# NethermindEth/latticefold

Hardware: AMD Instinct MI355X
Metric: folding-prover steps/sec (one NIFSProver::prove per step), GoldilocksRingNTT (higher is better)
Workload: dtype u64; 1 GPU; C4: GoldilocksRingNTT R1CS->CCS, m=N=2^20 rows, wit_len=262144, L=4, B=2^16, b=2, K=16, kappa=26, t=3; parallelism=replicas x1

## Files before the change

latticefold_amd/csrc/lf_capi.cpp:

```cpp
#include "lf_ring_host.h"

const char *lf_strerror(int code) {
    switch (code) {
        case LF_OK: return "ok";
        case LF_ERR_INVALID: return "invalid argument / wrong length";
        case LF_ERR_HIP: return "HIP runtime error (no GPU or out of device memory)";
        case LF_ERR_UNSUPPORTED: return "unsupported parameter";
        case LF_ERR_BAD_TABLES: return "ring tables are not a ring isomorphism";
        case LF_ERR_NORM: return "witness coefficient exceeds the decomposition bound";
        case LF_ERR_SIZE_BOUNDS: return "invalid size bounds (m must be >= wit_len*L, power of two)";
        case LF_ERR_STATE: return "call sequence misuse";
        case LF_ERR_REJECT: return "verifier rejected the proof";
    }
    return "unknown error";
}
const char *lf_phase_name(int i) { return (i >= 0 && i < LF_N_PHASES) ? PHASE_NAMES[i] : ""; }

static int install_tables(lf_ctx *c, u64 nonres, const u64 *y) {
    CrtTables T;
    if (build_crt_tables(nonres, y, T) != 0) return LF_ERR_BAD_TABLES;
    c->ring.T = T;
    c->dcrt = make_dev_crt(T);
    return ring_ops<GoldRing>::install_icrt(c, &T.icrt[0][0]);
}

int lf_ctx_create_ring(lf_ctx **out, int device, int ring) {
    if (ring == LF_RING_GOLDILOCKS) return lf_ctx_create(out, device);
    if (!out || ring != LF_RING_BABYBEAR) return LF_ERR_INVALID;
    lf_ctx *c = new lf_ctx();
    c->device = device;
    int rc = lfbb::BbCtx::create(&c->bb, c, device);
    if (rc != LF_OK) { delete c; return rc; }
    *out = c;
    return LF_OK;
}
int lf_ctx_device(const lf_ctx *c) { return c->device; }
int lf_ctx_ring(const lf_ctx *c) { return c && c->bb ? LF_RING_BABYBEAR : LF_RING_GOLDILOCKS; }
int lf_ring_words(int ring) { return ring == LF_RING_BABYBEAR ? 72 : (ring == LF_RING_GOLDILOCKS ? 24 : 0); }
int lf_ring_tau(int ring) { return ring == LF_RING_BABYBEAR ? 9 : (ring == LF_RING_GOLDILOCKS ? 3 : 0); }
uint64_t lf_ring_modulus(int ring) { return ring == LF_RING_BABYBEAR ? (uint64_t)lfbb::BB_P : (ring == LF_RING_GOLDILOCKS ? LF_P : 0); }

int lf_ctx_create(lf_ctx **out, int device) {
    if (!out) return LF_ERR_INVALID;
    int cnt = 0;
    if (hipGetDeviceCount(&cnt) != hipSuccess || cnt <= 0 || device < 0 || device >= cnt) return LF_ERR_HIP;
    HIPCHK(hipSetDevice(device));
    lf_ctx *c = new lf_ctx();
    c->device = device;
    int least = 0, greatest = 0;
    (void)hipDeviceGetStreamPriorityRange(&least, &greatest);
    if (c->create_lane_streams() != LF_OK || hipStreamCreateWithPriority(&c->st_io, hipStreamDefault, least) != hipSuccess) { delete c; return LF_ERR_HIP; }
    (void)hipEventCreateWithFlags(&c->ev_block, hipEventBlockingSync | hipEventDisableTiming);
    u64 nr, y[24];
    default_ring(&nr, y);
    int rc = install_tables(c, nr, y);
    if (rc != LF_OK) { delete c; return rc; }
    *out = c;
    return LF_OK;
}
static void planes_pool_drop(int device);
void lf_ctx_destroy(lf_ctx *c) {
    if (!c) return;
    while (c->io_jobs.load() > 0) std::this_thread::yield();
    (void)hipSetDevice(c->device);
    planes_pool_drop(c->device);
    if (c->bb) { c->bb->destroy(); delete c; return; }
    (void)c->sync_lanes();
    if (c->st_io) (void)hipStreamSynchronize(c->st_io);
    for (int l = 0; l < LF_NLANES; l++)
        if (c->stage[l]) (void)hipHostFree(c->stage[l]);
    if (c->h_pin2) { (void)hipHostFree(c->h_pin2); c->h_pin2 = nullptr; }
    if (c->ev_block) (void)hipEventDestroy(c->ev_block);
    c->comm[0].destroy();
    c->comm[1].destroy();
    if (c->tail_mail) (void)hipHostFree(c->tail_mail);
    if (c->tail_counters) (void)hipFree(c->tail_counters);
    if (c->d_poseidon) (void)hipFree(c->d_poseidon);
    if (c->ev_theta) (void)hipEventDestroy(c->ev_theta);
    if (c->ev_aux) (void)hipEventDestroy(c->ev_aux);
    if (c->st_aux) (void)hipStreamDestroy(c->st_aux);
    if (c->h_aux) (void)hipHostFree(c->h_aux);
    for (int i = 0; i < 2; i++)
        if (c->bits_ev[i]) (void)hipEventDestroy(c->bits_ev[i]);
    c->release_core();
    delete c;
}
int lf_set_ring_tables(lf_ctx *c, uint64_t nonres, const uint64_t *y) {
    if (!c || !y) return LF_ERR_INVALID;
    if (c->bb) return c->bb->set_ring_tables(nonres, y);
    std::lock_guard<std::mutex> g(c->mu);
    HIPCHK(hipSetDevice(c->device));
    return install_tables(c, nonres, y);
}
int lf_get_ring_tables(lf_ctx *c, uint64_t *nonres, uint64_t *y) {
    if (!c || !nonres || !y) return LF_ERR_INVALID;
    if (c->bb) return c->bb->get_ring_tables(nonres, y);
    *nonres = c->ring.T.nu;
    for (int k = 0; k < 8; k++)
        for (int q = 0; q < 3; q++) y[3 * k + q] = c->ring.T.y[k].c[q];
    return LF_OK;
}

int lf_set_digit_mode(lf_ctx *c, int mode) {
    if (!c || (mode != 0 && mode != 1)) return LF_ERR_INVALID;
    std::lock_guard<std::mutex> g(c->mu);
    c->core_any().digit_mode = mode;
    return LF_OK;
}
int lf_set_ext_basis(lf_ctx *c, const uint64_t *T) {
    if (!c || !T) return LF_ERR_INVALID;
    std::lock_guard<std::mutex> g(c->mu);
    const int ring = lf_ctx_ring(c);
    return c->xb.set(T, lf_ring_tau(ring), lf_ring_modulus(ring));
}
int lf_set_sharding(lf_ctx *c, int rank, int world, lf_exchange_fn cb, void *user) {
    if (!c || world < 1 || rank < 0 || rank >= world || (world & (world - 1)) != 0 || (world > 1 && !cb)) return LF_ERR_INVALID;
    if (c->bb) return c->bb->set_sharding(rank, world, cb, user);
    std::lock_guard<std::mutex> g(c->mu);
    if (c->A_loaded) return LF_ERR_STATE;
    for (int l = 0; l < 2; l++) {
        c->comm[l].destroy();
        c->comm[l].rank = rank; c->comm[l].world = world; c->comm[l].cb = cb; c->comm[l].user = user; c->comm[l].poisoned = false; c->comm[l].model = false;
    }
    c->sh_rank = rank; c->sh_world = world;
    c->two_lanes_ok = false;
    c->agreed_two_lanes = -1;
    return LF_OK;
}
int lf_set_sharding_model(lf_ctx *c, int rank, int world) {
    if (!c || world < 1 || rank < 0 || rank >= world || (world & (world - 1)) != 0) return LF_ERR_INVALID;
    if (c->bb) return LF_ERR_UNSUPPORTED;
    std::lock_guard<std::mutex> g(c->mu);
    if (c->A_loaded) return LF_ERR_STATE;
    for (int l = 0; l < 2; l++) {
        c->comm[l].destroy();
        c->comm[l].rank = rank; c->comm[l].world = world; c->comm[l].cb = nullptr; c->comm[l].user = nullptr; c->comm[l].poisoned = false; c->comm[l].model = world > 1;
    }
    c->sh_rank = rank; c->sh_world = world;
    c->two_lanes_ok = world > 1;
    c->agreed_two_lanes = -1;
    return LF_OK;
}
int lf_dist_stats_words(lf_ctx *c, uint64_t *words_sent, int reset) {
    if (!c || !words_sent) return LF_ERR_INVALID;
    if (c->bb) { *words_sent = 0; return LF_OK; }
    *words_sent = c->comm[0].words_sent + c->comm[1].words_sent;
    if (reset) c->comm[0].words_sent = c->comm[1].words_sent = 0;
    return LF_OK;
}
int exchange_modsum_dev(lf_ctx *c, u64 *inout_dev, size_t words) {
    if (c->sh_world <= 1 && !(c->tn.force_exchange && c->cm().nccl)) return LF_OK;
    u64 *g;
    RET(c->tbuf("sh_gather", (size_t)c->sh_world * words, &g));
    RET(c->cm().allgather_dev(inout_dev, g, words, c->stream()));
    launch_modsum(g, (u32)c->sh_world, words, inout_dev, c->stream());
    return LF_OK;
}
int lf_dist_unique_id(uint8_t *id128) { return lfdist::rccl_unique_id(id128); }
static int dist_handshake(lf_ctx *c) {
    c->two_lanes_ok = false;
    if (getenv("LF_DIST_NO_HANDSHAKE")) return LF_OK;
    const int W = c->sh_world, R = c->sh_rank, ITER = 4;
    const size_t words = 64, per_it = words * (size_t)(W + 1);
    const long limit_ms = 20000;
    u64 *dbuf[2] = {nullptr, nullptr}, *hbuf[2] = {nullptr, nullptr};
    for (int l = 0; l < 2; l++) {
        if (lf_dev_malloc(&dbuf[l], per_it * ITER * 8) != hipSuccess || hipHostMalloc((void **)&hbuf[l], per_it * ITER * 8) != hipSuccess) {
            for (int q = 0; q < 2; q++) { if (dbuf[q]) (void)hipFree(dbuf[q]); if (hbuf[q]) (void)hipHostFree(hbuf[q]); }
            return LF_ERR_HIP;
        }
    }
    auto word = [](int g, int lane, int it, size_t w) { return ((u64)(g + 1) * 0x9E3779B97F4A7C15ull) ^ ((u64)lane << 40) ^ ((u64)it << 32) ^ (u64)w; };
    auto run = [&](int lane) -> int {
        const int keep = t_lane;
        t_lane = lane;
        int rc = hipSetDevice(c->device) == hipSuccess ? LF_OK : LF_ERR_HIP;
        for (int it = 0; it < ITER && rc == LF_OK; it++) {
            u64 *hs = hbuf[lane] + per_it * it, *ds = dbuf[lane] + per_it * it;
            for (size_t w = 0; w < words; w++) hs[w] = word(R, lane, it, w);
            if (hipMemcpyAsync(ds, hs, words * 8, hipMemcpyHostToDevice, c->stream()) != hipSuccess) { rc = LF_ERR_HIP; break; }
            rc = c->cm().allgather_dev(ds, ds + words, words, c->stream());
            if (rc == LF_OK && hipMemcpyAsync(hs + words, ds + words, words * W * 8, hipMemcpyDeviceToHost, c->stream()) != hipSuccess) rc = LF_ERR_HIP;
        }
        t_lane = keep;
        return rc;
    };
    c->lane1.submit([&]() -> int { return run(1); });
    int rc = run(0);
    const int rc1 = c->lane1.wait();
    if (rc == LF_OK) rc = rc1;
    bool timed_out = false;
    const auto deadline = std::chrono::steady_clock::now() + std::chrono::milliseconds(limit_ms);
    for (int l = 0; l < 2 && rc == LF_OK && !timed_out; l++)
        for (;;) {
            const hipError_t q = hipStreamQuery(c->st_lane[l]);
            if (q == hipSuccess) break;
            if (q != hipErrorNotReady) { rc = LF_ERR_HIP; break; }
            if (std::chrono::steady_clock::now() > deadline) { timed_out = true; break; }
            std::this_thread::sleep_for(std::chrono::microseconds(200));
        }
    if (timed_out || rc != LF_OK) {
        c->comm[0].abort_peers(); c->comm[1].abort_peers();
        return LF_ERR_STATE;
    }
    bool ok = true;
    for (int l = 0; l < 2 && ok; l++)
        for (int it = 0; it < ITER && ok; it++)
            for (int g2 = 0; g2 < W && ok; g2++)
                for (size_t w = 0; w < words && ok; w++) ok = hbuf[l][per_it * it + words + (size_t)g2 * words + w] == word(g2, l, it, w);
    {
        const char *e = getenv("LF_SHARD_TWO_LANES");
        const u64 mine = e ? (atoi(e) != 0 ? 2 : 0) : (ok ? 1 : 0);
        u64 *hs = hbuf[0], *ds = dbuf[0];
        hs[0] = mine;
        const int keep = t_lane;
        t_lane = 0;
        int rc2 = hipMemcpyAsync(ds, hs, 8, hipMemcpyHostToDevice, c->stream()) == hipSuccess ? LF_OK : LF_ERR_HIP;
        if (rc2 == LF_OK) rc2 = c->cm().allgather_dev(ds, ds + 1, 1, c->stream());
        if (rc2 == LF_OK && hipMemcpyAsync(hs + 1, ds + 1, (size_t)W * 8, hipMemcpyDeviceToHost, c->stream()) != hipSuccess) rc2 = LF_ERR_HIP;
        bool late = false;
        for (; rc2 == LF_OK;) {
            const hipError_t q = hipStreamQuery(c->stream());
            if (q == hipSuccess) break;
            if (q != hipErrorNotReady) { rc2 = LF_ERR_HIP; break; }
            if (std::chrono::steady_clock::now() > deadline) { late = true; break; }
            std::this_thread::sleep_for(std::chrono::microseconds(200));
        }
        t_lane = keep;
        if (late || rc2 != LF_OK) { c->comm[0].abort_peers(); c->comm[1].abort_peers(); return LF_ERR_STATE; }
        u64 mn = 2;
        for (int g2 = 0; g2 < W; g2++) mn = hs[1 + g2] < mn ? hs[1 + g2] : mn;
        ok = mn >= 1;
        c->agreed_two_lanes = ok ? 1 : 0;
    }
    for (int l = 0; l < 2; l++) { (void)hipFree(dbuf[l]); (void)hipHostFree(hbuf[l]); c->comm[l].n_exchanges = 0; c->comm[l].us_total = 0; c->comm[l].us_max = 0; }
    c->two_lanes_ok = ok;
// ... 380 lines not shown
    return c->bb ? ring_ops<BbRing>::witness_from_f(c->bb->p, f_ntt, out) : ring_ops<GoldRing>::witness_from_f(c, f_ntt, out);
}
int lf_witness_get_f_coeff(lf_ctx *c, const lf_witness *w, uint64_t *out) {
    if (!c || !w || !out || w->ctx != c) return LF_ERR_INVALID;
    return c->bb ? ring_ops<BbRing>::witness_get_f_coeff(c->bb->p, w, out) : ring_ops<GoldRing>::witness_get_f_coeff(c, w, out);
}
int lf_witness_get_f(lf_ctx *c, const lf_witness *w, uint64_t *out) {
    if (LF_XB(c) && w && out) { XB x(c); int rc = lf_witness_get_f(c, w, out); if (rc == LF_OK) x.ring_out(out, w->N); return rc; }
    if (!c || !w || !out || w->ctx != c) return LF_ERR_INVALID;
    return c->bb ? ring_ops<BbRing>::witness_get_f(c->bb->p, w, out) : ring_ops<GoldRing>::witness_get_f(c, w, out);
}
int lf_witness_get_w_ccs(lf_ctx *c, const lf_witness *w, uint64_t *out) {
    if (LF_XB(c) && w && out && c->have_ccs_any()) { XB x(c); int rc = lf_witness_get_w_ccs(c, w, out); if (rc == LF_OK) x.ring_out(out, c->params_any().wit_len); return rc; }
    if (!c || !w || !out || w->ctx != c) return LF_ERR_INVALID;
    return c->bb ? ring_ops<BbRing>::witness_get_w_ccs(c->bb->p, w, out) : ring_ops<GoldRing>::witness_get_w_ccs(c, w, out);
}
int lf_witness_commit(lf_ctx *c, const lf_witness *w, uint64_t *cm_out) {
    if (LF_XB(c) && w && cm_out) { XB x(c); int rc = lf_witness_commit(c, w, cm_out); if (rc == LF_OK) x.ring_out(cm_out, c->core_any().kappa); return rc; }
    if (!c || !w || !cm_out || w->ctx != c) return LF_ERR_INVALID;
    return c->bb ? ring_ops<BbRing>::witness_commit(c->bb->p, w, cm_out) : ring_ops<GoldRing>::witness_commit(c, w, cm_out);
}
namespace {
struct PoolEnt { int device; size_t bytes; int32_t *p; };
std::mutex g_pool_mu;
std::vector<PoolEnt> g_pool;
}
int lf_planes_alloc(lf_ctx *c, size_t bytes, int32_t **out) {
    {
        std::lock_guard<std::mutex> g(g_pool_mu);
        for (size_t i = 0; i < g_pool.size(); i++)
            if (g_pool[i].device == c->device && g_pool[i].bytes == bytes) {
                *out = g_pool[i].p;
                g_pool.erase(g_pool.begin() + (long)i);
                return LF_OK;
            }
    }
    return lf_dev_malloc(out, bytes) == hipSuccess ? LF_OK : LF_ERR_HIP;
}
static void planes_release_dev(int device, size_t bytes, int32_t *p) {
    if (!p) return;
    {
        std::lock_guard<std::mutex> g(g_pool_mu);
        if (g_pool.size() < 9) { g_pool.push_back({device, bytes, p}); return; }
    }
    (void)hipFree(p);
}
void lf_planes_release(lf_ctx *c, size_t bytes, int32_t *p) { planes_release_dev(c->device, bytes, p); }
static void planes_pool_drop(int device) {
    std::lock_guard<std::mutex> g(g_pool_mu);
    for (size_t i = 0; i < g_pool.size();)
        if (g_pool[i].device == device) { (void)hipFree(g_pool[i].p); g_pool.erase(g_pool.begin() + (long)i); }
        else i++;
}
void lf_witness_free(lf_witness *w) {
    if (!w) return;
    (void)hipSetDevice(w->device);
    planes_release_dev(w->device, w->plane_bytes, w->planes);
    planes_release_dev(w->device, w->f_bytes, (int32_t *)w->f_ntt);
    planes_release_dev(w->device, w->w_bytes, (int32_t *)w->w_ccs);
    delete w;
}

lf_transcript *lf_transcript_new(void) { return new lf_transcript(); }
lf_transcript *lf_transcript_new_ring(int ring) {
    if (ring == LF_RING_GOLDILOCKS) return new lf_transcript();
    if (ring != LF_RING_BABYBEAR) return nullptr;
    lf_transcript *t = new lf_transcript();
    t->bb = new lfbb::BbTranscript();
    return t;
}
lf_transcript *lf_transcript_clone(const lf_transcript *t) { return t ? new lf_transcript(*t) : nullptr; }
void lf_transcript_free(lf_transcript *t) { delete t; }
void lf_transcript_absorb_fq(lf_transcript *t, const uint64_t *x, size_t n) {
    if (t->bb) t->bb->absorb_fq(x, n);
    else t->t.absorb_fq(x, n);
}
void lf_transcript_absorb_ring(lf_transcript *t, const uint64_t *e, size_t n) {
    if (t->bb) t->bb->absorb_ring(e, n);
    else t->t.absorb_ring(e, n);
}
void lf_transcript_get_challenge(lf_transcript *t, uint64_t *o) {
    if (t->bb) {
        lfbb::H9 c = t->bb->get_challenge();
        memcpy(o, c.c, sizeof(c.c));
        return;
    }
    Fq3 c = t->t.get_challenge();
    o[0] = c.c[0]; o[1] = c.c[1]; o[2] = c.c[2];
}
void lf_transcript_get_short_challenge(lf_transcript *t, uint64_t *o) {
    if (t->bb) t->bb->get_short_challenge(o);
    else t->t.get_short_challenge(o);
}
void lf_transcript_squeeze_bytes(lf_transcript *t, uint8_t *out, size_t n) {
    if (!t || !out || !n) return;
    const size_t usable = t->bb ? 3 : 7, ne = (n + usable - 1) / usable;
    std::vector<u64> e(ne);
    if (t->bb) t->bb->squeeze(e.data(), ne);
    else t->t.squeeze(e.data(), ne);
    for (size_t i = 0, o = 0; i < ne && o < n; i++)
        for (size_t j = 0; j < usable && o < n; j++) out[o++] = (uint8_t)(e[i] >> (8 * j));
}
void lf_poseidon_permute(uint64_t *state, int plain) {
    if (plain == 2) Transcript::permute_scalar(state);
    else if (plain) Transcript::permute_plain(state);
    else Transcript::permute(state);
}
void lf_poseidon_permute_ring(uint64_t *state, int plain, int ring) {
    if (ring == LF_RING_BABYBEAR) {
        if (plain == 2) lfbb::BbTranscript::permute_scalar(state);
        else if (plain) lfbb::BbTranscript::permute_plain(state);
        else lfbb::BbTranscript::permute(state);
    } else lf_poseidon_permute(state, plain);
}
void lf_poseidon_params(uint64_t *ark, uint64_t *mds) {
    const u64 *a, *m;
    Transcript::params(&a, &m);
    memcpy(ark, a, 720 * 8);
    memcpy(mds, m, 576 * 8);
}
void lf_poseidon_params_ring(uint64_t *ark, uint64_t *mds, int ring) {
    const u64 *a, *m;
    if (ring == LF_RING_BABYBEAR) lfbb::BbTranscript::params(&a, &m);
    else Transcript::params(&a, &m);
    memcpy(ark, a, 720 * 8);
    memcpy(mds, m, 576 * 8);
}

int lf_last_phase_ms(lf_ctx *c, float *out) {
    if (!c || !out) return LF_ERR_INVALID;
    for (int i = 0; i < LF_N_PHASES; i++) out[i] = c->core_any().phase_ms[i];
    return LF_OK;
}
int lf_last_timeline(lf_ctx *c, char *names, double *ms, int max_marks) {
    if (!c || !names || !ms || max_marks < 0) return LF_ERR_INVALID;
    if (c->bb) return 0;
    int n = 0;
    for (auto &m : c->tl_marks) {
        if (n >= max_marks) break;
        const char *w = m.first;
        while (*w == ' ') w++;
        snprintf(names + 32 * n, 32, "%s", w);
        ms[n++] = m.second;
    }
    return n;
}
int lf_abi_version(void) { return LFHIP_ABI_VERSION; }
int lf_debug_i8_prof(uint64_t *out64) {
    if (!out64) return LF_ERR_INVALID;
    return getenv("LF_I8G_PROF") ? ajtai_i8g_read_prof((unsigned long long *)out64) : ajtai_i8_read_prof((unsigned long long *)out64);
}
extern "C" int lfdbg_i8g_wg(unsigned int *out512) { return out512 ? ajtai_i8g_read_wg(out512) : -1; }
extern "C" unsigned lfdbg_i8g_planes_base(int ring, uint64_t base) { return ajtai_i8g_planes_base(ring == LF_RING_BABYBEAR ? ajtai_i8_babybear() : ajtai_i8_goldilocks(), base); }
int lf_last_fold_paths(lf_ctx *c, unsigned *sv_round_mask) {
    if (!c || !sv_round_mask) return LF_ERR_INVALID;
    *sv_round_mask = c->core_any().sv_round_mask;
    return LF_OK;
}
int lf_last_fold_split_rounds(lf_ctx *c, unsigned *round_mask) {
    if (!c || !round_mask) return LF_ERR_INVALID;
    *round_mask = c->core_any().fold_split_mask;
    return LF_OK;
}
int lf_last_lin_split_rounds(lf_ctx *c, unsigned *rounds) {
    if (!c || !rounds) return LF_ERR_INVALID;
    *rounds = c->bb ? 0u : c->lin_split_rounds;
    return LF_OK;
}
int lf_last_kernel_stats(lf_ctx *c, float *fold_ms, int *fold_n, float *aj_ms, int *aj_n) {
    if (!c) return LF_ERR_INVALID;
    const CtxCoreBase &k = c->core_any();
    if (fold_ms) *fold_ms = k.k_fold_ms;
    if (fold_n) *fold_n = k.k_fold_n;
    if (aj_ms) *aj_ms = k.k_ajtai_ms;
    if (aj_n) *aj_n = k.k_ajtai_n;
    return LF_OK;
}

namespace {
struct GoldV {
    static constexpr int RE = 24, TAU = 3;
    static u64 modulus() { return LF_P; }
    typedef Fq3 Ext;
    typedef Transcript Tr;
    HostRing ring;
    void mul(const u64 *a, const u64 *b, u64 *o) const { ring.mul_ntt(a, b, o); }
    void mul_ext(const u64 *a, Ext s, u64 *o) const { ring.mul_fq3(a, s, o); }
    static void add(const u64 *a, const u64 *b, u64 *o) { HostRing::add(a, b, o); }
    static void sub(const u64 *a, const u64 *b, u64 *o) { HostRing::sub(a, b, o); }
    static void from_u64(u64 v, u64 *o) { HostRing::from_u64(v, o); }
    static void from_ext(Ext e, u64 *o) { HostRing::from_fq3(e, o); }
    static Ext ext_of(const u64 *e) { return fq3_make(e[0], e[1], e[2]); }
    static Ext ext_from_u64(u64 v) { return fq3_make(v % LF_P, 0, 0); }
    Ext ext_mul(Ext a, Ext b) const { return ring.mul3(a, b); }
    static Ext ext_add(Ext a, Ext b) { return fq3_add(a, b); }
    static Ext ext_sub(Ext a, Ext b) { return fq3_sub(a, b); }
    Ext ext_inv(Ext a) const { return ring.inv3(a); }
    static void absorb_ext(Tr &tr, Ext e) { tr.absorb_fq3_as_ring(e); }
    void crt(const u64 *c, u64 *o) const { ring.crt(c, o); }
    static u64 fmul(u64 a, u64 b) { return fq_mul(a % LF_P, b % LF_P); }
    static u64 fadd(u64 a, u64 b) { return fq_add(a, b); }
    static void rot_x(u64 *a) {
        u64 top = a[23];
        for (int j = 23; j > 0; j--) a[j] = a[j - 1];
        a[0] = fq_neg(top);
        a[12] = fq_add(a[12], top);
    }
};
}

int lf_verify_host(int ring, const lf_params *p, const uint32_t *S_off, const uint32_t *S_idx, const uint64_t *c, lf_transcript *t,
                   const uint64_t *acc, const uint64_t *cm_i, const uint64_t *proof, uint64_t *lcccs_out, int *failed_stage) {
    if (!p || !S_off || !S_idx || !c || !t || !acc || !cm_i || !proof || !lcccs_out) return LF_ERR_INVALID;
    if (p->s == 0 || p->s > 40 || p->K == 0 || p->K > 32 || p->q == 0 || p->q > 8 || p->t == 0 || p->t > 16) return LF_ERR_UNSUPPORTED;
    if (((size_t)1 << p->s) < (size_t)p->wit_len * p->L) return LF_ERR_SIZE_BOUNDS;
    if (failed_stage) *failed_stage = 0;
    if (ring == LF_RING_BABYBEAR) return t->bb ? lfbb::bb_verify_host(p, S_off, S_idx, c, *t->bb, acc, cm_i, proof, lcccs_out, failed_stage) : LF_ERR_INVALID;
    if (ring != LF_RING_GOLDILOCKS || t->bb) return LF_ERR_INVALID;
    static const GoldV *gv = [] {
        GoldV *g = new GoldV();
        u64 nr, y[24];
        default_ring(&nr, y);
        build_crt_tables(nr, y, g->ring.T);
        return g;
    }();
    lfv::Verifier<GoldV> V(*gv, *p, S_off, S_idx, c);
    int rc = V.verify(t->t, acc, cm_i, proof, lcccs_out);
    if (failed_stage) *failed_stage = V.stage;
    return rc;
}
```

latticefold_amd/csrc/lf_ctx.h:

```cpp
#pragma once
#include <hip/hip_runtime.h>
#include <assert.h>
#include <string.h>

#include <atomic>
#include <chrono>
#include <condition_variable>
#include <functional>
#include <future>
#include <thread>
#include <map>
#include <memory>
#include <mutex>
#include <string>
#include <vector>

#include "../../include/lfhip.h"
#include "bb_capi.h"
#include "lf_ctx_core.h"
#include "lf_common.h"
#include "lf_dist.h"
#include "lf_kernels.h"
#include "lf_sb.h"
#include "lf_verify.h"

using namespace lf;

namespace lf {
void launch_fix_many(const DevCrt &t, const u64 *in, size_t ld_in, u64 *out, size_t ld_out, size_t n_in, u32 rows3, Fq3Const r, hipStream_t s);
}

#include <stdio.h>
#include <stdlib.h>
static bool lf_trace_on() { static int v = -1; if (v < 0) v = getenv("LF_TRACE") ? 1 : 0; return v == 1; }
#define LF_TRACE(c, msg)                                                              \
    do {                                                                              \
        if (lf_trace_on()) {                                                          \
            hipError_t e_ = hipStreamSynchronize((c)->stream());                            \
            fprintf(stderr, "[lf] %s:%d %s -> %s\n", __func__, __LINE__, msg, hipGetErrorString(e_)); \
            fflush(stderr);                                                           \
        }                                                                             \
    } while (0)

inline thread_local int t_lane = 0;

struct lf_transcript {
    Transcript t;
    lfbb::BbTranscript *bb = nullptr;
    lf_transcript() {}
    lf_transcript(const lf_transcript &o) : t(o.t), bb(o.bb ? new lfbb::BbTranscript(*o.bb) : nullptr) {}
    ~lf_transcript() { delete bb; }
};

struct Timeline {
    bool on;
    std::chrono::steady_clock::time_point t0;
    std::vector<std::pair<const char *, double>> marks, marks1;
    Timeline() : on(getenv("LF_TIMELINE") != nullptr), t0(std::chrono::steady_clock::now()) { marks1.reserve(32); }
    void mark(const char *what) {
        marks.push_back({what, std::chrono::duration<double, std::milli>(std::chrono::steady_clock::now() - t0).count()});
    }
    void mark1(const char *what) { marks1.push_back({what, std::chrono::duration<double, std::milli>(std::chrono::steady_clock::now() - t0).count()}); }
    void merge() {
        marks.insert(marks.end(), marks1.begin(), marks1.end());
        marks1.clear();
        std::stable_sort(marks.begin(), marks.end(), [](const std::pair<const char *, double> &a, const std::pair<const char *, double> &b) { return a.second < b.second; });
    }
    void dump() {
        if (!on) return;
        double prev = 0;
        for (auto &m : marks) { fprintf(stderr, "[timeline] %-28s at %8.3f ms  (+%7.3f)\n", m.first, m.second, m.second - prev); prev = m.second; }
    }
};
inline thread_local Timeline *t_tl = nullptr;
#define TL_MARK(x) do { if (t_tl) t_tl->mark(x); } while (0)

static const char *PHASE_NAMES[LF_N_PHASES] = {"linearization", "decomp_crt_commit", "decomp_evals", "fold_prepare",
                                                "fold_sumcheck", "fold_finish", "host_transcript", "total"};

struct LaneWorker {
    std::thread th;
    std::mutex m;
    std::condition_variable cv;
    std::function<int()> job;
    bool has_job = false, done = false, stop = false;
    int rc = 0;
    void loop() {
        std::unique_lock<std::mutex> lk(m);
        for (;;) {
            cv.wait(lk, [&] { return has_job || stop; });
            if (stop) return;
            std::function<int()> j = std::move(job);
            has_job = false;
            lk.unlock();
            int r = j();
            lk.lock();
            rc = r;
            done = true;
            cv.notify_all();
        }
    }
    void submit(std::function<int()> j) {
        std::unique_lock<std::mutex> lk(m);
        if (!th.joinable()) th = std::thread([this] { loop(); });
        job = std::move(j);
        has_job = true;
        done = false;
        cv.notify_all();
    }
    int wait() {
        std::unique_lock<std::mutex> lk(m);
        cv.wait(lk, [&] { return done; });
        return rc;
    }
    ~LaneWorker() {
        {
            std::unique_lock<std::mutex> lk(m);
            stop = true;
            cv.notify_all();
        }
        if (th.joinable()) th.join();
    }
};

struct lf_ctx : CtxCore<u64> {
    lf_ctx() : CtxCore<u64>(8192, 2 * 9 * 24 * sizeof(u64)) {}
    int lane() const override { return t_lane; }
    lfbb::BbCtx *bb = nullptr;
    ExtBasis xb;
    hipStream_t &st_io = st_lane[2];
    std::mutex io_mu;
    std::atomic<int> io_jobs{0};
    inline CtxCoreBase &core_any();
    bool have_ccs_any() { return core_any().have_ccs; }
    const lf_params &params_any() { return core_any().P; }
    size_t n_any() { return core_any().n; }
    size_t m_any() { return core_any().m; }
    size_t N_any() { return core_any().N; }
    HostRing ring;
    DevCrt dcrt;
    LaneWorker lane1;
    int agreed_two_lanes = -1;
    bool two_lanes_ok = false;
    lfdist::Comm comm[2];
    lfdist::Comm &cm() { assert(t_lane < 2); return comm[t_lane]; }
    bool ccs_general = false;
    size_t shc_r0 = (size_t)-1, shc_rcnt = 0, shc_lo = 0, shc_hi = 0;
    LinCombDesc desc{};
    std::vector<std::pair<const char *, double>> tl_marks;
    const lf_witness *bits_wit[2] = {nullptr, nullptr};
    u32 *bits_ptr[2] = {nullptr, nullptr};
    hipEvent_t bits_ev[2] = {nullptr, nullptr};
    hipEvent_t ev_yR = nullptr, ev_yL = nullptr;
    u64 *h_pin2 = nullptr;
    size_t h_pin2_words = 0;
    int pin2(size_t words) {
        if (words <= h_pin2_words) return LF_OK;
        if (h_pin2) (void)hipHostFree(h_pin2);
        h_pin2 = nullptr; h_pin2_words = 0;
        if (hipHostMalloc((void **)&h_pin2, words * 8) != hipSuccess) return LF_ERR_HIP;
        h_pin2_words = words;
        return LF_OK;
    }
    hipStream_t st_aux = nullptr;
    hipEvent_t ev_aux = nullptr;
    u64 *h_aux = nullptr;
    unsigned lin_split_rounds = 0;

    unsigned char *stage[LF_NLANES] = {nullptr, nullptr, nullptr};
    size_t stage_off[LF_NLANES] = {0, 0, 0};
    static constexpr size_t STAGE_BYTES = (size_t)1 << 20;
    int h2d_small(void *dst, const void *src, size_t bytes) {
        unsigned char *&ring = stage[t_lane];
        if (!ring && hipHostMalloc((void **)&ring, STAGE_BYTES, hipHostMallocDefault) != hipSuccess) { ring = nullptr; return LF_ERR_HIP; }
        const size_t need = (bytes + 63) & ~(size_t)63;
        if (need > STAGE_BYTES) {
            HIPCHK(hipMemcpyAsync(dst, src, bytes, hipMemcpyHostToDevice, stream()));
            HIPCHK(hipStreamSynchronize(stream()));
            return LF_OK;
        }
        if (stage_off[t_lane] + need > STAGE_BYTES) {
            HIPCHK(hipStreamSynchronize(stream()));
            stage_off[t_lane] = 0;
        }
        unsigned char *slot = ring + stage_off[t_lane];
        stage_off[t_lane] += need;
        memcpy(slot, src, bytes);
        HIPCHK(hipMemcpyAsync(dst, slot, bytes, hipMemcpyHostToDevice, stream()));
        return LF_OK;
    }
    TailMail *tail_mail = nullptr;
    u32 *tail_counters = nullptr;
    u64 *tail_dev_chal = nullptr;
    u32 tail_epoch = 0;
    int num_cus = 0;
    int tail_setup() {
        if (tail_mail) return LF_OK;
        hipDeviceProp_t pr;
        HIPCHK(hipGetDeviceProperties(&pr, device));
        num_cus = pr.multiProcessorCount;
        void *d = nullptr;
        HIPCHK(lf_dev_malloc(&d, 4096));
        HIPCHK(hipMemset(d, 0, 4096));
        tail_counters = (u32 *)d;
        tail_dev_chal = (u64 *)((char *)d + 1024);
        HIPCHK(hipHostMalloc((void **)&tail_mail, sizeof(TailMail), hipHostMallocMapped | hipHostMallocCoherent));
        memset(tail_mail, 0, sizeof(TailMail));
        return LF_OK;
    }
    u64 *d_poseidon = nullptr;
    int poseidon_setup() {
        if (d_poseidon) return LF_OK;
        const u64 *a, *m;
        Transcript::params(&a, &m);
        HIPCHK(lf_dev_malloc(&d_poseidon, (720 + 576) * 8));
        HIPCHK(hipMemcpy(d_poseidon, a, 720 * 8, hipMemcpyHostToDevice));
        HIPCHK(hipMemcpy(d_poseidon + 720, m, 576 * 8, hipMemcpyHostToDevice));
        return LF_OK;
    }
    hipEvent_t ev_theta = nullptr;
    hipEvent_t ev_block = nullptr;
    int lane_sync() {
        if (t_lane == 1 && ev_block) {
            HIPCHK(hipEventRecord(ev_block, st_lane[1]));
            HIPCHK(hipEventSynchronize(ev_block));
            return LF_OK;
        }
        HIPCHK(hipStreamSynchronize(stream()));
        return LF_OK;
    }
};
inline CtxCoreBase &lf_ctx::core_any() { return bb ? bb->core() : *this; }


#pragma GCC visibility push(hidden)
Fq3Const f3c(Fq3 a);
bool shard_keep(const lf_ctx *c, int kind, size_t n);
int build_eq_dev(lf_ctx *c, const Fq3 *pt, u32 nv, u64 *eq_dev);
int exchange_modsum_dev(lf_ctx *c, u64 *inout_dev, size_t words);
int down_small(lf_ctx *c, const u64 *dsrc, size_t words, u64 *host);
void shard_slice(const lf_ctx *c, size_t n, size_t *i0, size_t *cnt);
struct GatherPart { const u64 *src; size_t src_ld; u64 *dst; size_t planes; };
int shard_col_range(lf_ctx *c, size_t r0, size_t rcnt, size_t *lo, size_t *hi);
Fq3 sc_round_transcript(Transcript &tr, const u64 *evals, u32 npts);
void sc_prologue(Transcript &tr, u32 nv, u32 deg);
int gather_slices(lf_ctx *c, u64 *buf, size_t planes, size_t n);
struct SideState {
    const int32_t *planes = nullptr;
    u64 *z = nullptr;
    u64 *eq_r = nullptr;
    std::vector<u64> lcccs;
    std::atomic<int> z_state{0};
    hipEvent_t z_ev = nullptr;
    const unsigned char *D = nullptr;
    u32 *sv_bits = nullptr;
    ~SideState() { if (z_ev) (void)hipEventDestroy(z_ev); }
};
int gather_parts(lf_ctx *c, const GatherPart *parts, int np, size_t lcl);
inline thread_local bool t_xb_active = false;
struct XB {
    lf_ctx *c;
    size_t RE, TAU;
    std::vector<std::unique_ptr<std::vector<u64>>> keep;
    lf_transcript *tr = nullptr;
    explicit XB(lf_ctx *cc) : c(cc), RE((size_t)lf_ring_words(lf_ctx_ring(cc))), TAU((size_t)lf_ring_tau(lf_ctx_ring(cc))) { t_xb_active = true; }
    ~XB() {
        t_xb_active = false;
        if (tr) { tr->t.set_basis(nullptr, nullptr); if (tr->bb) tr->bb->set_basis(nullptr, nullptr); }
    }
    const u64 *ring_in(const u64 *p, size_t elems) {
        if (!p) return p;
        keep.emplace_back(new std::vector<u64>(p, p + elems * RE));
        c->xb.to_int(keep.back()->data(), elems * 8);
        return keep.back()->data();
    }
    const u64 *ext_in(const u64 *p, size_t n) {
        if (!p) return p;
        keep.emplace_back(new std::vector<u64>(p, p + n * TAU));
        c->xb.to_int(keep.back()->data(), n);
        return keep.back()->data();
    }
    void ring_out(u64 *p, size_t elems) { if (p) c->xb.to_ext(p, elems * 8); }
    void ext_out(u64 *p, size_t n) { if (p) c->xb.to_ext(p, n); }
    void transcript(lf_transcript *t) {
        tr = t;
        if (t->bb) t->bb->set_basis(c->xb.T, c->xb.Ti);
        else t->t.set_basis(c->xb.T, c->xb.Ti);
    }
};
#define LF_XB(c) ((c) && (c)->xb.on && !t_xb_active)
int fold_impl(lf_ctx *c, Transcript &tr, SideState *S , u64 *lcccs_out, lf_witness **w_out, u64 *proof);
int commit_download(lf_ctx *c, const u64 *dev, size_t words, u64 *host);
int commit_parts_i8g(lf_ctx *c, const unsigned char *D, size_t ldn, u32 NP, u64 *out_dev);
int sb_cut_parts(lf_ctx *c, const lf_witness *wit, const char *name, const unsigned char **D);
void fold_draw_rho(lf_ctx *c, Transcript &tr, const u64 *eta, std::vector<u64> &rho_c, std::vector<u64> &rho, std::vector<int8_t> &rho8);
void fold_instance_host(lf_ctx *c, const std::vector<Fq3> &pt, const u64 *theta, const u64 *eta, const std::vector<u64> &rho_c, const std::vector<u64> &rho, SideState *S,
                        u64 *lcccs_out);
int fold_impl_sb(lf_ctx *c, Transcript &tr, SideState *S , u64 *lcccs_out, lf_witness **w_out, u64 *proof);
int sb_fold_round_abi(lf_ctx *c, const u64 *t5, const u64 *F, size_t n, const Fq3Const *d_mu, u64 *evals_out);
int dot_batch_dev(lf_ctx *c, const u64 *X, size_t ldx, u32 na, const u64 *Y, size_t ldy, u32 nb, size_t n, u64 *dpart, u64 *od, hipStream_t st = nullptr,
                         const char *tag = "", unsigned char *yb_pre = nullptr);
int coef_eval_dev(lf_ctx *c, const int32_t *planes, size_t n, const u64 *eq, size_t ldeq, u32 K, int mode_bits, u64 *partial, u64 *od, size_t ldp,
                         const lf_witness *wit = nullptr);
int lin_tail_rounds(lf_ctx *c, Transcript &tr, const u64 *cur, const u64 *cure, size_t n, u64 *tout, u64 *partial, u32 round, Fq3 *point,
                           u64 *msgs, u32 deg, const std::function<void(u32)> *after_round);
int build_z(lf_ctx *c, const int32_t *planes, u32 K, int mode_bits, const u64 *heads, u64 *z, size_t w0 = 0, size_t wcnt = (size_t)-1,
            const unsigned char *D = nullptr );
bool lcccs_point(const lf_params &P, const u64 *lcccs, std::vector<Fq3> &pt);
#pragma GCC visibility pop
```

latticefold_amd/csrc/lf_ctx_core.h:

```cpp
#pragma once
#include <hip/hip_runtime.h>

#include <chrono>
#include <map>
#include <mutex>
#include <string>
#include <vector>

#include "../../include/lfhip.h"
#include "lf_common.h"

struct lf_witness;

constexpr int LF_NLANES = 3;

struct EvPair { hipEvent_t a, b; };

struct CtxCoreBase {
    int device = 0;
    hipStream_t st_lane[LF_NLANES] = {nullptr, nullptr, nullptr};
    std::mutex mu, buf_mu, ev_mu;
    int digit_mode = 0;
    Tunables tn;
    uint32_t lin_blocks = 0;
    bool A_loaded = false;
    unsigned char *dAb = nullptr;
    uint32_t i8_nch = 0, i8_kc = 0;
    uint32_t kappa = 0;
    size_t nA = 0, nA_total = 0, A_col0 = 0;
    int sh_rank = 0, sh_world = 1;
    bool have_ccs = false;
    lf_params P{};
    size_t N = 0, m = 0, n = 0;
    std::vector<uint32_t *> d_rowptr, d_col, d_colptr, d_rowidx;
    int sc_round = -1, sc_cur = 0;
    size_t sc_n = 0;
    int sf_round = -1, sf_cur = 0;
    size_t sf_n = 0;
    const lf_witness *vs_wit = nullptr;
    bool vs_keep = false;
    uint64_t *vs_dev = nullptr;
    hipEvent_t ev_prep[2] = {nullptr, nullptr};
    unsigned sv_round_mask = 0;
    unsigned fold_split_mask = 0;
    float phase_ms[LF_N_PHASES] = {0};
    float k_fold_ms = 0, k_ajtai_ms = 0;
    int k_fold_n = 0, k_ajtai_n = 0;
    double host_tr_ms = 0;

    virtual int lane() const = 0;
    hipStream_t stream() const { return st_lane[lane()]; }

    std::map<std::string, DevBuf> bufs;
    std::string lane_name(const std::string &name) const {
        const int l = lane();
        return l ? (l == 1 ? "lane1:" : "lane2:") + name : name;
    }
    int buf(const std::string &name, size_t bytes, void **out) {
        DevBuf *b;
        {
            std::lock_guard<std::mutex> g(buf_mu);
            b = &bufs[lane_name(name)];
        }
        int rc = b->ensure(bytes);
        *out = b->p;
        return rc;
    }
    void drop_buf(const std::string &name) {
        std::lock_guard<std::mutex> g(buf_mu);
        auto it = bufs.find(lane_name(name));
        if (it != bufs.end()) { it->second.release(); bufs.erase(it); }
    }
    template <class T>
    int tbuf(const std::string &name, size_t count, T **out) {
        void *p;
        int rc = buf(name, count * sizeof(T), &p);
        *out = (T *)p;
        return rc;
    }
    uint64_t *h_pin_lane[LF_NLANES] = {nullptr, nullptr, nullptr};
    size_t h_pin_words_lane[LF_NLANES] = {0, 0, 0};
    uint64_t *h_round[LF_NLANES] = {nullptr, nullptr, nullptr};
    uint64_t *&h_pin_ref() { return h_pin_lane[lane()]; }
    int pin(size_t words) {
        uint64_t *&hp = h_pin_lane[lane()];
        size_t &hw = h_pin_words_lane[lane()];
        if (words <= hw) return LF_OK;
        if (hp) (void)hipHostFree(hp);
        hp = nullptr; hw = 0;
        if (words < pin_min_words) words = pin_min_words;
        if (hipHostMalloc((void **)&hp, words * 8) != hipSuccess) return LF_ERR_HIP;
        hw = words;
        return LF_OK;
    }
    uint64_t *round_out() {
        uint64_t *&p = h_round[lane()];
        if (!p && hipHostMalloc((void **)&p, round_out_bytes, hipHostMallocMapped) != hipSuccess) p = nullptr;
        return p;
    }
    std::vector<EvPair> ev_pool;
    size_t ev_used = 0;
    std::vector<std::pair<int, size_t>> ev_tags;
    size_t ev_begin(int tag) {
        std::lock_guard<std::mutex> g(ev_mu);
        if (ev_used == ev_pool.size()) {
            EvPair e;
            (void)hipEventCreate(&e.a);
            (void)hipEventCreate(&e.b);
            ev_pool.push_back(e);
        }
        size_t i = ev_used++;
        (void)hipEventRecord(ev_pool[i].a, stream());
        ev_tags.push_back({tag, i});
        return i;
    }
    void ev_end(size_t i) {
        if (i == (size_t)-1) return;
        std::lock_guard<std::mutex> g(ev_mu);
        (void)hipEventRecord(ev_pool[i].b, stream());
    }
    void ev_reset() {
        ev_used = 0;
        ev_tags.clear();
    }
    void ev_collect() {
        (void)hipStreamSynchronize(st_lane[0]);
        (void)hipStreamSynchronize(st_lane[1]);
        k_fold_ms = k_ajtai_ms = 0;
        k_fold_n = k_ajtai_n = 0;
        for (int i = 0; i < LF_N_PHASES; i++) phase_ms[i] = 0;
        for (auto &tg : ev_tags) {
            float ms = 0;
            (void)hipEventElapsedTime(&ms, ev_pool[tg.second].a, ev_pool[tg.second].b);
            if (tg.first == 0) { k_fold_ms += ms; k_fold_n++; }
            else if (tg.first == 1) { k_ajtai_ms += ms; k_ajtai_n++; }
            else if (tg.first >= 10 && tg.first < 10 + LF_N_PHASES) phase_ms[tg.first - 10] += ms;
        }
        phase_ms[6] = (float)host_tr_ms;
    }
    int shard_columns(size_t n_cols, size_t *col0, size_t *cnt) const {
        if (n_cols % (size_t)sh_world) return LF_ERR_UNSUPPORTED;
        *cnt = n_cols / sh_world;
        *col0 = *cnt * sh_rank;
        return LF_OK;
    }
    int create_lane_streams() {
        int least = 0, greatest = 0;
        (void)hipDeviceGetStreamPriorityRange(&least, &greatest);
        if (hipStreamCreateWithPriority(&st_lane[0], hipStreamDefault, least) != hipSuccess ||
            hipStreamCreateWithPriority(&st_lane[1], hipStreamDefault, greatest) != hipSuccess) return LF_ERR_HIP;
        return LF_OK;
    }
    int sync_lanes() {
        HIPCHK(hipStreamSynchronize(st_lane[0]));
        HIPCHK(hipStreamSynchronize(st_lane[1]));
        return LF_OK;
    }
    void drop_matrix() {
        if (dAb) (void)hipFree(dAb);
        dAb = nullptr;
        A_loaded = false;
        kappa = i8_nch = i8_kc = 0;
        nA = nA_total = A_col0 = 0;
    }
    virtual ~CtxCoreBase() {}

protected:
    CtxCoreBase(size_t pin_min, size_t round_bytes) : pin_min_words(pin_min), round_out_bytes(round_bytes) {}
    const size_t pin_min_words, round_out_bytes;
    void release_base() {
        for (auto &kv : bufs) kv.second.release();
        drop_matrix();
        for (int l = 0; l < LF_NLANES; l++) {
            if (h_pin_lane[l]) (void)hipHostFree(h_pin_lane[l]);
            if (h_round[l]) (void)hipHostFree(h_round[l]);
            h_pin_lane[l] = h_round[l] = nullptr;
        }
        for (auto &e : ev_pool) { (void)hipEventDestroy(e.a); (void)hipEventDestroy(e.b); }
        ev_pool.clear();
        for (int l = 0; l < 2; l++)
            if (ev_prep[l]) (void)hipEventDestroy(ev_prep[l]);
        for (int l = 0; l < LF_NLANES; l++)
            if (st_lane[l]) (void)hipStreamDestroy(st_lane[l]);
    }
};

template <class W>
struct CtxCore : CtxCoreBase {
    W *d_icrt = nullptr;
    W *d_icrt_sp_val = nullptr;
    uint32_t *d_icrt_sp_col = nullptr;
    std::vector<W *> d_val, d_valT;
    const W *vs_eq = nullptr;
    void free_ccs() {
        for (auto q : d_rowptr) (void)hipFree(q);
        for (auto q : d_col) (void)hipFree(q);
        for (auto q : d_val) (void)hipFree(q);
// ... 26 lines not shown
```

latticefold_amd/csrc/lf_fold.cpp:

```cpp
#include "lf_ring_host.h"

static int tail_host_rounds(lf_ctx *c, Transcript &tr, u32 epoch, u32 nr, u32 npts, bool dev_transcript, u64 *msgs, Fq3 *pt,
                            const std::function<void(u32)> *after_round = nullptr, u32 round0 = 0) {
    TailMail *mail = c->tail_mail;
    const auto t_start = std::chrono::steady_clock::now();
    double host_us = 0, wait_us = 0;
    auto t_mark = t_start;
    const bool tl_on = t_tl && t_tl->on;
    for (u32 i = 0; i < nr; i++) {
        u32 spins = 0;
        while (__atomic_load_n(&mail->msg_seq[i], __ATOMIC_ACQUIRE) != epoch) {
            __builtin_ia32_pause();
            if ((++spins & 0xfff) == 0) {
                if (__atomic_load_n(&mail->err, __ATOMIC_RELAXED) == epoch ||
                    std::chrono::duration<double>(std::chrono::steady_clock::now() - t_start).count() > 10.0) {
                    __atomic_store_n(&mail->abort_seq, epoch, __ATOMIC_RELEASE);
                    (void)hipStreamSynchronize(c->stream());
                    return LF_ERR_HIP;
                }
            }
        }
        if (tl_on) { auto nw = std::chrono::steady_clock::now(); wait_us += std::chrono::duration<double, std::micro>(nw - t_mark).count(); t_mark = nw; }
        u64 *evs = msgs + (size_t)i * npts * 24;
        memcpy(evs, (const void *)mail->msg[i], (size_t)npts * 24 * 8);
// ... 28 lines not shown
    RET(c->tail_setup());
    LinTailArgs A;
    A.T = cur; A.E = cure; A.Tout = tout; A.n0 = n; A.rounds = P.s - round + 1; A.deg = deg; A.partial = partial;
    RET(c->tbuf("lin_tail_priv", lin_tail_priv_words(n, P.t), &A.priv));
    A.counters = c->tail_counters; A.dev_chal = c->tail_dev_chal;
    HIPCHK(hipHostGetDevicePointer((void **)&A.mail, c->tail_mail, 0));
    if (++c->tail_epoch >= (1u << 30)) c->tail_epoch = 1;
    A.epoch = c->tail_epoch;
    A.r_first = f3c(point[round - 2]);
    A.dev_transcript = (c->tn.device_transcript && !c->xb.on) ? 1u : 0u;
    A.pos_ark = A.pos_mds = nullptr; A.sponge_state = nullptr;
    if (A.dev_transcript) {
        RET(tail_sponge_to_device(c, tr, &A.sponge_state));
        A.pos_ark = c->d_poseidon; A.pos_mds = c->d_poseidon + 720;
    }
    if (launch_lin_tail(c->dcrt, c->desc, A, c->stream()) == 0) return LF_ERR_UNSUPPORTED;
    if (hipGetLastError() != hipSuccess) return LF_ERR_HIP;
    return tail_host_rounds(c, tr, A.epoch, A.rounds, deg + 1, A.dev_transcript != 0, msgs + (size_t)(round - 1) * (deg + 1) * 24, &point[round - 1], after_round, round);
}
static int fold_tail_rounds(lf_ctx *c, Transcript &tr, const FoldRoundArgs &a, u64 *curF, u64 *const Fbuf[2], u64 *T_other, const Fq3Const *d_mu,
                            u64 *partial, u32 round, std::vector<Fq3> &pt, u64 *msgs, u32 deg) {
    const lf_params &P = c->P;
    RET(c->tail_setup());
    const u32 nr = P.s - round + 1;
    FoldTailArgs A;
    A.T[0] = (u64 *)a.eqL; A.T[1] = T_other;
    A.F[0] = curF; A.F[1] = curF == Fbuf[0] ? Fbuf[1] : Fbuf[0];
    A.n0 = a.n; A.rounds = nr; A.K = P.K; A.mu_pow = d_mu; A.partial = partial;
    A.counters = c->tail_counters; A.dev_chal = c->tail_dev_chal;
    RET(c->tbuf("tail_eqpriv", fold_tail_eqpriv_words(a.n, P.K), &A.eqpriv));
    HIPCHK(hipHostGetDevicePointer((void **)&A.mail, c->tail_mail, 0));
    if (++c->tail_epoch >= (1u << 30)) c->tail_epoch = 1;
    A.epoch = c->tail_epoch;
    A.r_first = f3c(pt[round - 2]);
    A.dev_transcript = (c->tn.device_transcript && !c->xb.on) ? 1u : 0u;
    A.pos_ark = A.pos_mds = nullptr; A.sponge_state = nullptr;
    if (A.dev_transcript) {
        RET(tail_sponge_to_device(c, tr, &A.sponge_state));
        A.pos_ark = c->d_poseidon; A.pos_mds = c->d_poseidon + 720;
    }
    if (launch_fold_tail(c->dcrt, A, c->num_cus, c->stream()) == 0) return LF_ERR_UNSUPPORTED;
    if (hipGetLastError() != hipSuccess) return LF_ERR_HIP;
    return tail_host_rounds(c, tr, A.epoch, nr, deg + 1, A.dev_transcript != 0, msgs + (size_t)(round - 1) * (deg + 1) * 24, &pt[round - 1]);
}

static void sv_build_coef(lf_ctx *c, int V, const Fq3 *W, std::vector<u64> &out) {
    const int NX = 2 * V, NPR = sv_num_pairs(V);
    std::vector<Fq3> C((size_t)NPR * 4, fq3_zero());
    std::vector<SvPair> prs(NPR);
    for (int i = 0; i < NPR; i++) prs[i] = sv_pair(V, i);
    auto find = [&](unsigned s, unsigned b) {
        for (int i = 0; i < NPR; i++)
            if (prs[i].s == s && prs[i].b == b) return i;
        return -1;
    };
    std::vector<Fq3> wa(NX), wb(NX);
    for (int x = 0; x < NX; x++) {
        if (x < V) { wa[x] = W[x]; wb[x] = fq3_neg(W[x]); }
        else { wa[x] = fq3_zero(); wb[x] = W[x - V]; }
    }
    for (int x = 0; x < NX; x++)
        for (int y = x; y < NX; y++) {
            const Fq3 p2[3] = {c->ring.mul3(wa[x], wa[y]), fq3_add(c->ring.mul3(wa[x], wb[y]), c->ring.mul3(wb[x], wa[y])), c->ring.mul3(wb[x], wb[y])};
            for (int z = y; z < NX; z++) {
                Fq3 p3[4];
                p3[0] = c->ring.mul3(p2[0], wa[z]);
                p3[1] = fq3_add(c->ring.mul3(p2[0], wb[z]), c->ring.mul3(p2[1], wa[z]));
                p3[2] = fq3_add(c->ring.mul3(p2[1], wb[z]), c->ring.mul3(p2[2], wa[z]));
                p3[3] = c->ring.mul3(p2[2], wb[z]);
                int mult, idx;
                if (x == y && y == z) { mult = 1; idx = find(1u << x, 1u << x); }
                else if (x == y) { mult = 3; idx = find(1u << z, (1u << x) | (1u << z)); }
                else if (y == z) { mult = 3; idx = find(1u << x, (1u << x) | (1u << y)); }
                else { mult = 6; const unsigned mk = (1u << x) | (1u << y) | (1u << z); idx = find(mk, mk); }
                for (int e = 0; e < 4; e++) {
                    Fq3 t = p3[e], acc = fq3_zero();
                    for (int i = 0; i < mult; i++) acc = fq3_add(acc, t);
                    C[(size_t)idx * 4 + e] = fq3_add(C[(size_t)idx * 4 + e], acc);
                }
            }
        }
    for (int x = 0; x < NX; x++) {
        const int idx = find(1u << x, 1u << x);
        C[(size_t)idx * 4] = fq3_sub(C[(size_t)idx * 4], wa[x]);
        C[(size_t)idx * 4 + 1] = fq3_sub(C[(size_t)idx * 4 + 1], wb[x]);
    }
    out.resize((size_t)NPR * 12);
    for (size_t i = 0; i < (size_t)NPR * 4; i++)
        for (int q = 0; q < 3; q++) out[i * 3 + q] = C[i].c[q];
}

void fold_draw_rho(lf_ctx *c, Transcript &tr, const u64 *eta, std::vector<u64> &rho_c, std::vector<u64> &rho, std::vector<int8_t> &rho8) {
    const lf_params &P = c->P;
    const u32 K2 = 2 * P.K;
    rho_c.assign((size_t)K2 * 24, 0); rho.assign((size_t)K2 * 24, 0); rho8.assign((size_t)K2 * 24, 0);
    {
        HostTimer ht(c);
        tr.absorb_ring(eta, (size_t)K2 * P.t);
        tr.absorb_label("rho_s");
        for (u32 i = 0; i + 1 < K2; i++) tr.get_short_challenge(&rho_c[(size_t)i * 24]);
        rho_c[(size_t)(K2 - 1) * 24] = 1;
        for (u32 i = 0; i < K2; i++) {
            c->ring.crt(&rho_c[(size_t)i * 24], &rho[(size_t)i * 24]);
            for (int q2 = 0; q2 < 24; q2++) {
                u64 v = rho_c[(size_t)i * 24 + q2];
                rho8[(size_t)i * 24 + q2] = (int8_t)(v > LF_P / 2 ? -(int64_t)(LF_P - v) : (int64_t)v);
            }
        }
    }
}
void fold_instance_host(lf_ctx *c, const std::vector<Fq3> &pt, const u64 *theta, const u64 *eta, const std::vector<u64> &rho_c, const std::vector<u64> &rho, SideState *S,
                        u64 *lcccs_out) {
    const lf_params &P = c->P;
    const u32 K = P.K, K2 = 2 * K;
    const size_t ll = lf_lcccs_len(&P);
    HostTimer ht(c);
    u64 *o = lcccs_out;
    for (u32 i = 0; i < P.s; i++, o += 24) HostRing::from_fq3(pt[i], o);
    {
        Fq3 res[24];
        for (int j = 0; j < 24; j++) res[j] = fq3_zero();
        for (u32 i = 0; i < K2; i++) {
            u64 rot[24];
            memcpy(rot, &rho_c[(size_t)i * 24], sizeof(rot));
            const u64 *th = theta + (size_t)i * 72;
            for (int bi = 0; bi < 24; bi++) {
                Fq3 b = fq3_make(th[3 * bi], th[3 * bi + 1], th[3 * bi + 2]);
                for (int j = 0; j < 24; j++)
                    if (rot[j]) res[j] = fq3_add(res[j], fq3_mul_fq(b, rot[j]));
                u64 top = rot[23];
                for (int j = 23; j > 0; j--) rot[j] = rot[j - 1];
                rot[0] = fq_neg(top);
                rot[12] = fq_add(rot[12], top);
            }
        }
        for (int j = 0; j < 24; j++) { o[3 * j] = res[j].c[0]; o[3 * j + 1] = res[j].c[1]; o[3 * j + 2] = res[j].c[2]; }
        o += 72;
    }
    u64 tmp[24];
    auto part = [&](u32 i) { return &S[i < K ? 0 : 1].lcccs[(size_t)(i % K) * ll * 24]; };
    for (u32 q2 = 0; q2 < P.kappa; q2++, o += 24) {
        memset(o, 0, 24 * 8);
        for (u32 i = 0; i < K2; i++) { c->ring.mul_ntt(part(i) + ((size_t)P.s + 3 + q2) * 24, &rho[(size_t)i * 24], tmp); HostRing::add(o, tmp, o); }
    }
    for (u32 j = 0; j < P.t; j++, o += 24) {
        memset(o, 0, 24 * 8);
        for (u32 i = 0; i < K2; i++) { c->ring.mul_ntt(&rho[(size_t)i * 24], eta + ((size_t)i * P.t + j) * 24, tmp); HostRing::add(o, tmp, o); }
    }
    for (u32 q2 = 0; q2 < P.l + 1; q2++, o += 24) {
        memset(o, 0, 24 * 8);
        for (u32 i = 0; i < K2; i++) { c->ring.mul_ntt(&rho[(size_t)i * 24], part(i) + ((size_t)P.s + 3 + P.kappa + P.t + q2) * 24, tmp); HostRing::add(o, tmp, o); }
    }
}
int fold_impl(lf_ctx *c, Transcript &tr, SideState *S , u64 *lcccs_out, lf_witness **w_out, u64 *proof) {
    if (c->P.b != 2) return fold_impl_sb(c, tr, S, lcccs_out, w_out, proof);
    const lf_params &P = c->P;
    size_t m = c->m, n = c->n, N = c->N;
    u32 K = P.K, K2 = 2 * K, deg = 2 * P.b;
    std::vector<Fq3> alpha(K2), zeta(K2), mu(K2), beta(P.s);
    {
        HostTimer ht(c);
        tr.absorb_label("alpha_s");
        for (u32 i = 0; i < K2; i++) alpha[i] = tr.get_challenge();
        tr.absorb_label("zeta_s");
        for (u32 i = 0; i < K2; i++) zeta[i] = tr.get_challenge();
    }
    size_t ph = c->ev_begin(13);
    std::vector<Fq3Const> mu_pow((size_t)K2 * 3), a_pow((size_t)K2 * 3), z_pow((size_t)K2 * P.t);
    for (u32 i = 0; i < K2; i++) {
        Fq3 pa = alpha[i], pz = zeta[i];
        for (u32 d = 0; d < 3; d++) { a_pow[(size_t)i * 3 + d] = f3c(pa); pa = c->ring.mul3(pa, alpha[i]); }
        for (u32 j = 0; j < P.t; j++) { z_pow[(size_t)i * P.t + j] = f3c(pz); pz = c->ring.mul3(pz, zeta[i]); }
    }
    Fq3Const *d_mu, *d_ap, *d_zp;
    RET(upload_consts(c, "c_ap", a_pow, &d_ap));
    RET(upload_consts(c, "c_zp", z_pow, &d_zp));
    u64 *G[2], *eqb, *zz, *partial, *od;
    RET(c->tbuf("fold_G1", 24 * m, &G[0]));
    RET(c->tbuf("fold_G2", 24 * m, &G[1]));
    RET(c->tbuf("fold_eqb", 3 * m, &eqb));
    RET(c->tbuf("fold_zz", (size_t)P.t * 24 * n, &zz));
    RET(c->tbuf("round_partial", round_partial_words(), &partial));
    od = c->round_out();
    if (!od) return LF_ERR_HIP;
    u64 *const od_host = od, *od_shard = nullptr;
    if (c->sh_world > 1) {
        RET(c->tbuf("fold_round_out", 5 * 24 + 8, &od_shard));
        od = od_shard;
    }
    const bool shard_tabs = shard_keep(c, 1, m);
    const size_t g_r0 = shard_tabs ? (size_t)c->sh_rank * (m / (size_t)c->sh_world) : 0, g_rcnt = shard_tabs ? m / (size_t)c->sh_world : (size_t)-1;
    size_t zc_lo = 0, zc_hi = n;
    if (shard_tabs) RET(shard_col_range(c, g_r0, g_rcnt, &zc_lo, &zc_hi));
    {
        hipStream_t s0 = c->stream(), s1 = (t_lane == 0) ? c->st_lane[1] : s0;
        u64 *zz1 = zz;
        if (s1 != s0) {
            RET(c->tbuf("fold_zz1", (size_t)P.t * 24 * n, &zz1));
            if (!c->ev_prep[0]) { HIPCHK(hipEventCreateWithFlags(&c->ev_prep[0], hipEventDisableTiming)); HIPCHK(hipEventCreateWithFlags(&c->ev_prep[1], hipEventDisableTiming)); }
            HIPCHK(hipEventRecord(c->ev_prep[0], s0));
            HIPCHK(hipStreamWaitEvent(s1, c->ev_prep[0], 0));
        }
        for (int sd = 0; sd < 2; sd++) {
            hipStream_t st = sd ? s1 : s0;
            u64 *zb = sd ? zz1 : zz;
            launch_lincomb_z(c->dcrt, S[sd].z + zc_lo, n, K, d_zp + (size_t)sd * K * P.t, P.t, zc_hi - zc_lo, zb + zc_lo, st);
            if (c->ccs_general) {
                u64 *zaos;
                RET(c->tbuf(sd ? "spmv_zaos_R" : "spmv_zaos_L", (size_t)P.t * n * 24, &zaos));
                launch_spmv_rows(c->dcrt, P.t, c->d_rowptr.data(), c->d_col.data(), c->d_val.data(), zb, (size_t)24 * n, n, zaos, G[sd], m, 0, st, g_r0, g_rcnt);
            } else
            launch_spmv_sum(c->dcrt, P.t, c->d_rowptr.data(), c->d_col.data(), c->d_val.data(), zb, (size_t)24 * n, n, G[sd], m, st, g_r0, g_rcnt);
            launch_add_fhat_comb(c->dcrt, S[sd].planes, N, K, d_ap + (size_t)sd * K * 3, G[sd], m, st, g_r0, g_rcnt);
        }
        if (s1 != s0) {
            HIPCHK(hipEventRecord(c->ev_prep[1], s1));
            HIPCHK(hipStreamWaitEvent(s0, c->ev_prep[1], 0));
        }
    }
    {
        HostTimer ht(c);
        tr.absorb_label("mu_s");
        for (u32 i = 0; i + 1 < K2; i++) mu[i] = tr.get_challenge();
        mu[K2 - 1] = fq3_one();
        tr.absorb_label("beta_s");
        for (u32 i = 0; i < P.s; i++) beta[i] = tr.get_challenge();
    }
    TL_MARK(" fold challenges");
    for (u32 i = 0; i < K2; i++) {
        Fq3 pm = mu[i];
        for (u32 d = 0; d < 3; d++) { mu_pow[(size_t)i * 3 + d] = f3c(pm); pm = c->ring.mul3(pm, mu[i]); }
    }
    RET(upload_consts(c, "c_mu", mu_pow, &d_mu));
    RET(build_eq_dev(c, beta.data(), P.s, eqb));
    u64 *svE[3] = {nullptr, nullptr, nullptr};
    const bool sv_split = !c->tn.fold_sv_no_split && P.s >= 4 && m >= 256;
    if (sv_split) {
        RET(c->tbuf("fold_svE1", 3 * (m / 2), &svE[0]));
        RET(c->tbuf("fold_svE2", 3 * (m / 4), &svE[1]));
        RET(c->tbuf("fold_svE3", 3 * (m / 8), &svE[2]));
        RET(build_eq_dev(c, beta.data() + 1, P.s - 1, svE[0]));
    }
    Fq3 sv_c = fq3_one();
    u32 svE_level = 1;
    const bool fr_split = sv_split && c->sh_world == 1 && c->dcrt.nu2p40 && !c->tn.fold_rounds_no_split;
    u64 *svE_rest = nullptr;
    if (fr_split) RET(c->tbuf("fold_svE_rest", 3 * (m / 8) + 64, &svE_rest));
    auto svE_ptr = [&](u32 l) -> u64 * {
        if (l <= 3) return svE[l - 1];
        size_t off = 0;
        for (u32 q = 4; q < l; q++) off += 3 * (m >> q);
        return svE_rest + off;
    };
    auto svE_ensure = [&](u32 l) {
        for (; svE_level < l; svE_level++)
            launch_eq_pairsum(svE_ptr(svE_level), m >> svE_level, m >> (svE_level + 1), svE_ptr(svE_level + 1), m >> (svE_level + 1), c->stream());
    };
    auto sv_c_at = [&](u32 round, const std::vector<Fq3> &ptv) {
        Fq3 cc = fq3_one();
        for (u32 k = 1; k < round; k++) {
            const Fq3 b = beta[k - 1], r = ptv[k - 1];
            cc = c->ring.mul3(cc, fq3_add(c->ring.mul3(fq3_sub(fq3_one(), b), fq3_sub(fq3_one(), r)), c->ring.mul3(b, r)));
        }
        return cc;
    };
    LF_TRACE(c, "fold prepare");
    c->ev_end(ph);
    if (t_tl && t_tl->on) { (void)hipStreamSynchronize(c->stream()); TL_MARK(" fold prepare (synced)"); }

    ph = c->ev_begin(14);
    u64 *msgs = proof;
    std::vector<Fq3> pt(P.s);
    { HostTimer ht(c); sc_prologue(tr, P.s, deg); }
    const size_t Gw = (size_t)c->sh_world, gr = (size_t)c->sh_rank;
    bool sharded = Gw > 1;
    const bool fused = !c->tn.fold_unfused && (Gw == 1 || !c->tn.shard_plain_rounds);
    const size_t fuse_min = c->tn.fuse_min;
    int fmode = 0;
    const u64 *prevF = nullptr;
    size_t prevld = 0;
    const size_t lut_min = c->tn.lut_min;
    const size_t tab_min = c->tn.tab_min;
    const bool use_lut = fused && P.s >= 4 && m / 4 >= lut_min && m / 4 >= 4 && !c->tn.fold_no_lut;
    const bool use_r4tab = use_lut && c->dcrt.nu2p40 && !c->tn.fold_no_r4tab;
    const bool use_r5 = use_r4tab && !c->tn.fold_no_r5tab && Gw == 1 && P.s >= 5 && (N & 3) == 0 && (c->tn.no_tail || m / 8 > c->tn.tail_n) && m / 32 >= c->tn.r5_min;
    u64 *F[2], *T5[2];
    size_t half = m / 2;
    const size_t f0_ent = use_lut ? m / 16 : m / 4, f1_ent = use_r5 ? m / 32 : m / 8;
    RET(c->tbuf("fold_F0", (size_t)K2 * 3 * 24 * (f0_ent ? f0_ent : 1), &F[0]));
    RET(c->tbuf("fold_F1", (size_t)K2 * 3 * 24 * (f1_ent ? f1_ent : 1), &F[1]));
    RET(c->tbuf("fold_T0", 57 * (half ? half : 1), &T5[0]));
    RET(c->tbuf("fold_T1", 57 * (half / 2 ? half / 2 : 1), &T5[1]));
    FoldRoundArgs a;
    a.eqL = S[0].eq_r; a.eqR = S[1].eq_r; a.eqB = eqb; a.G1 = G[0]; a.G2 = G[1]; a.ld = m; a.n = m;
    a.p0 = 0; a.pcnt = m / 2; a.pF0 = 0;
    const u64 *curF = nullptr;
    size_t ldF = 0;
    int flip = 0;
    u64 *d_lut = nullptr;
    c->sv_round_mask = 0;
    c->fold_split_mask = 0;
    u32 *sv_bits[2] = {nullptr, nullptr};
    const bool sv_two_streams = t_lane == 0 && Gw == 1;
    hipStream_t sv_g_stream = c->stream();
    const bool use_sv = !c->tn.force_exchange && !c->tn.fold_no_sv && (Gw == 1 || !c->tn.shard_plain_rounds) && N <= m && (N & 3) == 0 && !c->tn.fold_tab_r1;
    for (u32 round = 1; round <= P.s; round++) {
        fmode = 0;
        if (!sharded && !c->tn.no_tail && round >= 5 && fmode == 0 && curF && ldF == a.n && a.n <= c->tn.tail_n && a.n >= 4 &&
            P.s - round + 1 <= TAIL_MAX_ROUNDS) {
            int trc = fold_tail_rounds(c, tr, a, (u64 *)curF, F, T5[flip], d_mu, partial, round, pt, msgs, deg);
            if (trc == LF_OK) {
                curF = (u64 *)curF == F[0] ? F[1] : F[0];
                ldF = 2;
                break;
            }
            if (trc != LF_ERR_UNSUPPORTED) return trc;
        }
        if (round > 1) {
            Fq3Const r = f3c(pt[round - 2]);
            size_t nn = a.n / 2;
            u64 *dst = T5[flip];
            const bool handover = sharded && !shard_keep(c, 1, nn);
            hipStream_t sg = c->stream();
            if (use_sv && sv_two_streams && !sharded && (int)round <= c->tn.sv_rounds && round <= 3 && nn / 2 >= c->tn.sv_min && sv_shape_ok(1 << (round - 1), nn / 2, K))
                sg = c->st_lane[1];
            sv_g_stream = sg;
            if (sharded) {
                const size_t j0 = gr * (nn / Gw), jc = nn / Gw;
                if (round == 2) {
                    launch_fix_many(c->dcrt, a.eqL + 2 * j0, a.ld, dst + j0, nn, 2 * jc, 1, r, sg);
                    launch_fix_many(c->dcrt, a.eqR + 2 * j0, a.ld, dst + 3 * nn + j0, nn, 2 * jc, 1, r, sg);
                    launch_fix_many(c->dcrt, a.eqB + 2 * j0, a.ld, dst + 6 * nn + j0, nn, 2 * jc, 1, r, sg);
                    launch_fix_many(c->dcrt, a.G1 + 2 * j0, a.ld, dst + 9 * nn + j0, nn, 2 * jc, 8, r, sg);
                    launch_fix_many(c->dcrt, a.G2 + 2 * j0, a.ld, dst + 33 * nn + j0, nn, 2 * jc, 8, r, sg);
                } else {
                    launch_fix_many(c->dcrt, a.eqL + 2 * j0, a.ld, dst + j0, nn, 2 * jc, 19, r, sg);
                }
                if (handover && round <= 3) RET(gather_slices(c, dst, 57, nn));
            } else if (round == 2) {
                launch_fix_many(c->dcrt, a.eqL, a.ld, dst, nn, a.n, 1, r, sg);
                launch_fix_many(c->dcrt, a.eqR, a.ld, dst + 3 * nn, nn, a.n, 1, r, sg);
                launch_fix_many(c->dcrt, a.eqB, a.ld, dst + 6 * nn, nn, a.n, 1, r, c->stream());
                launch_fix_many(c->dcrt, a.G1, a.ld, dst + 9 * nn, nn, a.n, 8, r, sg);
                launch_fix_many(c->dcrt, a.G2, a.ld, dst + 33 * nn, nn, a.n, 8, r, sg);
            } else if (sg != c->stream()) {
                launch_fix_many(c->dcrt, a.eqL, a.ld, dst, nn, a.n, 2, r, sg);
                launch_fix_many(c->dcrt, a.eqB, a.ld, dst + 6 * nn, nn, a.n, 1, r, c->stream());
                launch_fix_many(c->dcrt, a.G1, a.ld, dst + 9 * nn, nn, a.n, 16, r, sg);
            } else {
                launch_fix_many(c->dcrt, a.eqL, a.ld, dst, nn, a.n, 19, r, c->stream());
            }
            if (handover) {
                if (round > 3) {
                    u64 *fd = F[(round & 1) ? 0 : 1];
                    size_t lcl = ldF / 2;
                    launch_fix_many(c->dcrt, curF, ldF, fd, lcl, ldF, K2 * 3 * 8, r, c->stream());
                    const GatherPart gp[2] = {{dst + gr * lcl, nn, dst, 57}, {fd, lcl, fd, (size_t)K2 * 3 * 24}};
                    RET(gather_parts(c, gp, 2, lcl));
                    curF = fd; ldF = nn;
                    sharded = false;
                    a.eqL = dst; a.eqR = dst + 3 * nn; a.eqB = dst + 6 * nn; a.G1 = dst + 9 * nn; a.G2 = dst + 33 * nn;
                    a.ld = nn; a.n = nn; a.p0 = 0; a.pcnt = nn / 2; a.pF0 = 0;
                    flip ^= 1;
                    goto tables_ready;
                }
                sharded = false;
            }
            if (round == 3) {
                Fq3 r1 = pt[0], r2 = pt[1], o1 = fq3_sub(fq3_one(), r1), o2 = fq3_sub(fq3_one(), r2);
                Fq3Const W[4] = {f3c(c->ring.mul3(o1, o2)), f3c(c->ring.mul3(r1, o2)), f3c(c->ring.mul3(o1, r2)), f3c(c->ring.mul3(r1, r2))};
                size_t q = sharded ? nn / Gw : nn, j0 = sharded ? gr * q : 0;
                if (use_lut) {
                    std::vector<u64> lut(2 * 81 * 3);
                    for (int code = 0; code < 81; code++) {
                        Fq3 v = fq3_zero();
                        int cc = code;
                        for (int b = 0; b < 4; b++, cc /= 3) {
                            Fq3 wb = fq3_make(W[b].c[0], W[b].c[1], W[b].c[2]);
                            if (cc % 3 == 2) v = fq3_add(v, wb);
                            else if (cc % 3 == 0) v = fq3_sub(v, wb);
                        }
                        lut[3 * code] = v.c[0]; lut[3 * code + 1] = v.c[1]; lut[3 * code + 2] = v.c[2];
                        Fq3 sq = c->ring.mul3(v, v);
                        lut[3 * (81 + code)] = sq.c[0]; lut[3 * (81 + code) + 1] = sq.c[1]; lut[3 * (81 + code) + 2] = sq.c[2];
                    }
                    RET(c->tbuf("fold_lut", 2 * 81 * 3 + 8, &d_lut));
                    RET(c->h2d_small(d_lut, lut.data(), lut.size() * 8));
                    fmode = 3;
                    curF = nullptr; ldF = q;
                } else {
                    launch_fold_materialize2(c->dcrt, S[0].planes, S[1].planes, N, j0, q, K, W, F[0], c->stream());
                    curF = F[0]; ldF = q;
                }
            } else if (round > 3) {
                u64 *fd = F[(round & 1) ? 0 : 1];
                if (use_lut && round == 4) fmode = 4;
                else if (use_r5 && round == 5) fmode = 7;
                else if (fused && ldF >= fuse_min && ldF >= 4) { prevF = curF; prevld = ldF; fmode = 1; }
                else launch_fix_many(c->dcrt, curF, ldF, fd, ldF / 2, ldF, K2 * 3 * 8, r, c->stream());
                curF = fd; ldF = ldF / 2;
            }
            a.eqL = dst; a.eqR = dst + 3 * nn; a.eqB = dst + 6 * nn; a.G1 = dst + 9 * nn; a.G2 = dst + 33 * nn;
            a.ld = nn; a.n = nn;
            flip ^= 1;
        }
        if (sharded && !shard_keep(c, 1, a.n)) sharded = false;
        if (sharded) { a.pcnt = a.n / 2 / Gw; a.p0 = gr * a.pcnt; a.pF0 = a.p0; }
        else { a.p0 = 0; a.pcnt = a.n / 2; a.pF0 = 0; }
    tables_ready:
        const u64 *Er = nullptr;
        size_t ldEr = 0;
        bool split_now = false;
        if (fr_split && round >= 2 && !sharded && (fmode == 7 || (fmode == 4 && use_r4tab)) && a.pcnt >= c->tn.fold_split_min) {
            sv_c = sv_c_at(round, pt);
            const Fq3 bi = beta[round - 1];
            if ((sv_c.c[0] | sv_c.c[1] | sv_c.c[2]) && (bi.c[0] | bi.c[1] | bi.c[2])) {
                svE_ensure(round);
                Er = svE_ptr(round); ldEr = m >> round;
                split_now = true;
                c->fold_split_mask |= 1u << (round - 1);
            }
        }
        size_t ev = c->ev_begin(0);
        const int svV = 1 << (round - 1);
        if (use_sv && (int)round <= c->tn.sv_rounds && round <= 3 && a.pcnt >= c->tn.sv_min && sv_shape_ok(svV, a.pcnt, K) && (a.p0 * (size_t)svV) % 256 == 0) {
            std::vector<Fq3> W((size_t)svV, fq3_one());
            for (int b = 0; b < svV; b++)
                for (u32 j = 0; j + 1 < round; j++) W[b] = c->ring.mul3(W[b], ((b >> j) & 1) ? pt[j] : fq3_sub(fq3_one(), pt[j]));
            std::vector<u64> coef;
            sv_build_coef(c, svV, W.data(), coef);
            u64 *d_coef, *gtmp, *svtp;
            unsigned char *sveb;
            int32_t *svpart, *svtot;
            RET(c->tbuf("sv_coef", coef.size() + 8, &d_coef));
            RET(c->tbuf("sv_gtmp", 128, &gtmp));
            RET(c->tbuf("sv_tp", sv_tp_words(K), &svtp));
            RET(c->tbuf("sv_eb", sv_eb_bytes(a.pcnt), &sveb));
            RET(c->tbuf("sv_part", sv_part_words(svV, a.pcnt, K), &svpart));
            RET(c->tbuf("sv_tot", sv_tot_words(svV, K), &svtot));
            RET(c->h2d_small(d_coef, coef.data(), coef.size() * 8));
            if (!sv_bits[0])
                for (int sd = 0; sd < 2; sd++) {
                    if (S[sd].sv_bits) { sv_bits[sd] = S[sd].sv_bits; continue; }
                    RET(c->tbuf(sd ? "sv_bits_R" : "sv_bits_L", sv_bits_words(N, K), &sv_bits[sd]));
                    launch_sv_bits(S[sd].planes, N, N, K, sv_bits[sd], c->stream());
                }
            hipStream_t sg = round == 1 ? (sv_two_streams && !sharded ? c->st_lane[1] : c->stream()) : sv_g_stream;
            hipEvent_t g_ready = nullptr;
            if (sg != c->stream()) {
                if (!c->ev_prep[0]) { HIPCHK(hipEventCreateWithFlags(&c->ev_prep[0], hipEventDisableTiming)); HIPCHK(hipEventCreateWithFlags(&c->ev_prep[1], hipEventDisableTiming)); }
                if (round == 1) {
                    HIPCHK(hipEventRecord(c->ev_prep[0], c->stream()));
                    HIPCHK(hipStreamWaitEvent(sg, c->ev_prep[0], 0));
                }
            }
            launch_fold_round_g(c->dcrt, a, partial, gtmp, sg);
            if (sg != c->stream()) {
                HIPCHK(hipEventRecord(c->ev_prep[1], sg));
                g_ready = c->ev_prep[1];
            }
            const u64 *Ei = nullptr;
            size_t ldE = 0;
            Fq3Const w01[2] = {};
            if (sv_split) {
                sv_c = sv_c_at(round, pt);
                const Fq3 bi = beta[round - 1];
                w01[0] = f3c(c->ring.mul3(sv_c, fq3_sub(fq3_one(), bi)));
                w01[1] = f3c(c->ring.mul3(sv_c, bi));
                svE_ensure(round);
                const size_t ne = m >> round;
                Ei = svE[round - 1]; ldE = ne;
            }
            if (launch_sv_round(c->dcrt, svV, sv_bits[0], sv_bits[1], N, a.eqB, a.ld, a.p0, a.pcnt, K, d_mu, d_coef, sveb, svpart, svtot, svtp, gtmp, od, c->stream(), g_ready,
                                Ei, ldE, w01) != 0)
                return LF_ERR_UNSUPPORTED;
            c->sv_round_mask |= 1u << (round - 1);
        } else
        if ((round == 2 || (round == 1 && c->tn.fold_tab_r1)) && a.pcnt >= tab_min) {
            const int nd = round == 1 ? 2 : 4, ncode = round == 1 ? 9 : 81;
            std::vector<u64> poly((size_t)ncode * 12);
            const Fq3 one = fq3_one(), r1v = round == 2 ? pt[0] : fq3_zero();
            auto small = [&](int v) { return v == 0 ? fq3_zero() : (v > 0 ? (v == 1 ? one : fq3_add(one, one)) : (v == -1 ? fq3_neg(one) : fq3_neg(fq3_add(one, one)))); };
            for (int code = 0; code < ncode; code++) {
                int dg[4] = {0, 0, 0, 0}, cc = code;
                for (int b = 0; b < nd; b++, cc /= 3) dg[b] = cc % 3 - 1;
                Fq3 f0, f1;
                if (round == 1) { f0 = small(dg[0]); f1 = small(dg[1]); }
                else {
                    f0 = fq3_add(small(dg[0]), c->ring.mul3(small(dg[1] - dg[0]), r1v));
                    f1 = fq3_add(small(dg[2]), c->ring.mul3(small(dg[3] - dg[2]), r1v));
                }
                Fq3 df = fq3_sub(f1, f0), f0s = c->ring.mul3(f0, f0), dfs = c->ring.mul3(df, df);
                Fq3 t1 = c->ring.mul3(f0s, df), t2 = c->ring.mul3(f0, dfs);
                Fq3 q[4] = {fq3_sub(c->ring.mul3(f0s, f0), f0), fq3_sub(fq3_add(fq3_add(t1, t1), t1), df), fq3_add(fq3_add(t2, t2), t2), c->ring.mul3(dfs, df)};
                for (int e = 0; e < 4; e++)
                    for (int w = 0; w < 3; w++) poly[(size_t)code * 12 + 3 * e + w] = q[e].c[w];
            }
            u64 *d_poly, *d_tp;
            RET(c->tbuf("fold_poly", 81 * 12 + 8, &d_poly));
            RET(c->tbuf("fold_tp", (size_t)K2 * 3 * 81 * 12, &d_tp));
            RET(c->h2d_small(d_poly, poly.data(), poly.size() * 8));
            launch_fold_round_tab(c->dcrt, (int)round, a, S[0].planes, S[1].planes, N, K, d_mu, d_poly, d_tp, partial, od, c->stream());
        } else if (round == 1) launch_fold_round1(c->dcrt, a, S[0].planes, S[1].planes, N, K, d_mu, partial, od, c->stream());
        else if (round == 2) launch_fold_round2(c->dcrt, a, S[0].planes, S[1].planes, N, K, d_mu, f3c(pt[0]), partial, od, c->stream());
        else if (fmode == 3 && c->dcrt.nu2p40) {
            u64 *mutab;
            RET(c->tbuf("fold_mutab", (size_t)3 * K2 * 3 * 81 * 4, &mutab));
            launch_fold_round_lut_mu(c->dcrt, a, S[0].planes, S[1].planes, N, d_lut, mutab, K, d_mu, partial, od, c->stream());
        } else if (fmode == 3) launch_fold_round_lut(c->dcrt, a, S[0].planes, S[1].planes, N, d_lut, K, d_mu, partial, od, c->stream());
        else if (fmode == 4 && use_r4tab) {
            u64 *r4sq, *r4mt;
            RET(c->tbuf("fold_r4sq", (size_t)6561 * 4, &r4sq));
            RET(c->tbuf("fold_r4mt", (size_t)K2 * 3 * 162 * 4, &r4mt));
            launch_fold_round_lut_fix_tab(c->dcrt, a, S[0].planes, S[1].planes, N, d_lut, f3c(pt[round - 2]), r4sq, r4mt, use_r5 ? nullptr : (u64 *)curF, ldF, K, d_mu, partial, od,
                                          c->stream(), Er, ldEr);
        } else if (fmode == 7) {
            u64 *r5xx, *r5yy, *r5mt;
            RET(c->tbuf("fold_r5xx", (size_t)6561 * 4, &r5xx));
            RET(c->tbuf("fold_r5yy", (size_t)6561 * 4, &r5yy));
            RET(c->tbuf("fold_r5mt", (size_t)K2 * 3 * 324 * 4, &r5mt));
            launch_fold_round_lut_fix5(c->dcrt, a, S[0].planes, S[1].planes, N, d_lut, f3c(pt[round - 3]), f3c(pt[round - 2]), r5xx, r5yy, r5mt, (u64 *)curF, ldF, K, d_mu, partial, od,
                                       c->stream(), Er, ldEr);
        } else if (fmode == 4) launch_fold_round_lut_fix(c->dcrt, a, S[0].planes, S[1].planes, N, d_lut, f3c(pt[round - 2]), (u64 *)curF, ldF, K, d_mu, partial, od, c->stream());
        else if (fmode == 1) launch_fold_round_fix(c->dcrt, a, prevF, prevld, f3c(pt[round - 2]), (u64 *)curF, ldF, K, d_mu, partial, od, c->stream(), Er, ldEr);
        else launch_fold_round(c->dcrt, a, curF, ldF, K, d_mu, partial, od, c->stream());
        if (split_now) {
            u64 *partial_g;
            RET(c->tbuf("round_partial_g", round_partial_words(), &partial_g));
            launch_fold_round_g(c->dcrt, a, partial_g, od + 120, c->stream());
        }
        c->ev_end(ev);
        LF_TRACE(c, "fold round");
        u64 *evs = msgs + (size_t)(round - 1) * (deg + 1) * 24;
        if (od == od_shard) {
            if (sharded) RET(exchange_modsum_dev(c, od, (size_t)(deg + 1) * 24));
            HIPCHK(hipMemcpyAsync(od_host, od, (size_t)(deg + 1) * 24 * 8, hipMemcpyDeviceToHost, c->stream()));
        }
        RET(c->lane_sync());
        if (split_now) {
            HostTimer ht2(c);
            const Fq3 bi = beta[round - 1], obi = fq3_sub(fq3_one(), bi), cinv = c->ring.inv3(sv_c), binv = c->ring.inv3(bi);
            const Fq3 x = pt[round - 2];
            Fq3 wS[5];
            for (u32 j = 0; j <= deg; j++) {
                Fq3 num = fq3_one();
                u64 den = 1;
                for (u32 k = 0; k <= deg; k++) {
                    if (k == j) continue;
                    num = c->ring.mul3(num, fq3_sub(x, fq3_make(k, 0, 0)));
                    den = fq_mul(den, j > k ? (u64)(j - k) : LF_P - (u64)(k - j));
                }
                const u64 di = fq_inv(den);
                wS[j] = fq3_make(fq_mul(num.c[0], di), fq_mul(num.c[1], di), fq_mul(num.c[2], di));
            }
            const u64 *pe = msgs + (size_t)(round - 2) * (deg + 1) * 24;
            auto ld = [&](const u64 *b, u32 e, u32 slot) { return fq3_make(b[e * 24 + 3 * slot], b[e * 24 + 3 * slot + 1], b[e * 24 + 3 * slot + 2]); };
            for (u32 slot = 0; slot < 8; slot++) {
                Fq3 S = fq3_zero();
                for (u32 j = 0; j <= deg; j++) S = fq3_add(S, c->ring.mul3(wS[j], ld(pe, j, slot)));
                const Fq3 A0 = ld(od_host, 0, slot), A1 = ld(od_host, 1, slot), A2 = ld(od_host, 2, slot);
                const u64 *gev = od_host + 120;
                const Fq3 Gsum = fq3_add(ld(gev, 0, slot), ld(gev, 1, slot));
                const Fq3 T1 = c->ring.mul3(fq3_sub(c->ring.mul3(fq3_sub(S, Gsum), cinv), c->ring.mul3(obi, A0)), binv);
                const Fq3 A3 = fq3_sub(fq3_sub(fq3_sub(T1, A0), A1), A2);
                Fq3 l = obi;
                const Fq3 dl = fq3_sub(bi, obi);
                for (u32 X = 0; X <= deg; X++) {
                    const Fq3 xs = fq3_make(X, 0, 0);
                    const Fq3 T = fq3_add(A0, c->ring.mul3(xs, fq3_add(A1, c->ring.mul3(xs, fq3_add(A2, c->ring.mul3(xs, A3))))));
                    const Fq3 g = fq3_add(c->ring.mul3(c->ring.mul3(sv_c, l), T), ld(gev, X, slot));
                    evs[X * 24 + 3 * slot] = g.c[0]; evs[X * 24 + 3 * slot + 1] = g.c[1]; evs[X * 24 + 3 * slot + 2] = g.c[2];
                    l = fq3_add(l, dl);
                }
            }
        } else
        memcpy(evs, od_host, (size_t)(deg + 1) * 24 * 8);
        HostTimer ht(c);
        pt[round - 1] = sc_round_transcript(tr, evs, deg + 1);
        if (round == 1) TL_MARK("  round 1");
        if (round == 2) TL_MARK("  round 2");
        if (round == 3) TL_MARK("  round 3");
        if (round == 6) TL_MARK("  round 6");
        if (round == 10) TL_MARK("  round 10");
    }
    TL_MARK(" fold sumcheck");
    c->ev_end(ph);

    ph = c->ev_begin(15);
    u64 *theta = proof + (size_t)P.s * (deg + 1) * 24, *eta = theta + (size_t)K2 * 72;
    u64 *eq0, *q, *red, *sm, *dpart;
    RET(c->tbuf("fold_eq0", 3 * m, &eq0));
    RET(c->tbuf("dec_q", (size_t)P.t * 24 * n, &q));
    RET(c->tbuf("red_partial", 256 * 4096, &red));
    RET(c->tbuf("dec_small", 32 * 72 + 32 * 8 * 24 + 64, &sm));
    RET(c->tbuf("dot_partial", dot_partial_words(K, P.t), &dpart));
    RET(build_eq_dev(c, pt.data(), P.s, eq0));
    hipStream_t s1f = (t_lane == 0 && c->sh_world == 1 && c->st_lane[1]) ? c->st_lane[1] : c->stream();
    if (s1f != c->stream() && !c->ev_prep[0]) { HIPCHK(hipEventCreateWithFlags(&c->ev_prep[0], hipEventDisableTiming)); HIPCHK(hipEventCreateWithFlags(&c->ev_prep[1], hipEventDisableTiming)); }
    {
        size_t c0, cnt;
        shard_slice(c, n, &c0, &cnt);
        if (s1f != c->stream() && P.t > 1) {
            HIPCHK(hipEventRecord(c->ev_prep[0], c->stream()));
            HIPCHK(hipStreamWaitEvent(s1f, c->ev_prep[0], 0));
        }
        for (u32 j = 0; j < P.t; j++)
            launch_spmv_t_eq(c->dcrt, c->d_colptr[j], c->d_rowidx[j], c->d_valT[j], eq0, m, q + (size_t)j * 24 * n, n, (j & 1) ? s1f : c->stream(), c0, cnt);
        if (s1f != c->stream() && P.t > 1) {
            HIPCHK(hipEventRecord(c->ev_prep[1], s1f));
            HIPCHK(hipStreamWaitEvent(c->stream(), c->ev_prep[1], 0));
        }
    }
    u64 *fsm;
    RET(c->tbuf("fold_small", (size_t)K2 * 72 + (size_t)K2 * P.t * 24 + 64, &fsm));
    RET(c->pin((size_t)K2 * 72 + (size_t)K2 * P.t * 24));
    u64 *hp = c->h_pin_ref();
    u64 *d_theta = fsm, *d_eta = fsm + (size_t)K2 * 72;
    if (P.s >= 4 && curF && ldF == 2 && !c->tn.theta_eval) launch_fix_final(c->dcrt, curF, K2 * 3 * 8, f3c(pt[P.s - 1]), d_theta, c->stream());
    else
    {
        size_t i0, cnt;
        shard_slice(c, N, &i0, &cnt);
        for (int sd = 0; sd < 2; sd++) RET(coef_eval_dev(c, S[sd].planes + i0, cnt, eq0 + i0, m, K, 1, red, d_theta + (size_t)sd * K * 72, N));
        RET(exchange_modsum_dev(c, d_theta, (size_t)K2 * 72));
    }
    HIPCHK(hipMemcpyAsync(hp, d_theta, (size_t)K2 * 72 * 8, hipMemcpyDeviceToHost, c->stream()));
    if (!c->ev_theta) HIPCHK(hipEventCreateWithFlags(&c->ev_theta, hipEventDisableTiming));
    HIPCHK(hipEventRecord(c->ev_theta, c->stream()));
    {
        size_t c0, cnt;
        shard_slice(c, n, &c0, &cnt);
        hipStream_t s1 = (t_lane == 0 && c->sh_world == 1 && c->st_lane[1]) ? c->st_lane[1] : c->stream();
        if (s1 != c->stream()) {
            if (!c->ev_prep[0]) { HIPCHK(hipEventCreateWithFlags(&c->ev_prep[0], hipEventDisableTiming)); HIPCHK(hipEventCreateWithFlags(&c->ev_prep[1], hipEventDisableTiming)); }
            unsigned char *ybq = nullptr;
            if (!c->tn.dot_valu && cnt >= c->tn.dot_min && P.t <= 3 && K <= 16 && ((((size_t)(S[0].z + c0)) ^ ((size_t)(S[1].z + c0))) & 15) == 0) {
                RET(c->tbuf("dot_yb", dot_i8_yb_bytes(n + 1), &ybq));
                if (launch_dot_pack_y(S[0].z + c0, q + c0, n, P.t, cnt, ybq, c->stream()) != 0) ybq = nullptr;
            }
            HIPCHK(hipEventRecord(c->ev_prep[0], c->stream()));
            HIPCHK(hipStreamWaitEvent(s1, c->ev_prep[0], 0));
            u64 *dpart1;
            RET(c->tbuf("dot_partial1", dot_partial_words(K, P.t), &dpart1));
            RET(dot_batch_dev(c, S[1].z + c0, n, K, q + c0, n, P.t, cnt, dpart1, d_eta + (size_t)K * P.t * 24, s1, "_1", ybq));
            HIPCHK(hipEventRecord(c->ev_prep[1], s1));
            RET(dot_batch_dev(c, S[0].z + c0, n, K, q + c0, n, P.t, cnt, dpart, d_eta, nullptr, "", ybq));
            HIPCHK(hipStreamWaitEvent(c->stream(), c->ev_prep[1], 0));
        } else
            for (int sd = 0; sd < 2; sd++) RET(dot_batch_dev(c, S[sd].z + c0, n, K, q + c0, n, P.t, cnt, dpart, d_eta + (size_t)sd * K * P.t * 24));
        RET(exchange_modsum_dev(c, d_eta, (size_t)K2 * P.t * 24));
    }
    HIPCHK(hipMemcpyAsync(hp + (size_t)K2 * 72, d_eta, (size_t)K2 * P.t * 24 * 8, hipMemcpyDeviceToHost, c->stream()));
    HIPCHK(hipEventSynchronize(c->ev_theta));
    memcpy(theta, hp, (size_t)K2 * 72 * 8);
    {
        HostTimer ht(c);
        tr.absorb_ring(theta, (size_t)K2 * 3);
    }
    HIPCHK(hipStreamSynchronize(c->stream()));
    memcpy(eta, hp + (size_t)K2 * 72, (size_t)K2 * P.t * 24 * 8);
    TL_MARK(" theta/eta");
    std::vector<u64> rho_c, rho;
    std::vector<int8_t> rho8;
    fold_draw_rho(c, tr, eta, rho_c, rho, rho8);
    int8_t *d_rho;
    RET(c->tbuf("c_rho", (size_t)K2 * 24 + 64, &d_rho));
    HIPCHK(hipMemcpyAsync(d_rho, rho8.data(), rho8.size(), hipMemcpyHostToDevice, c->stream()));
    int32_t *npl;
    RET(lf_planes_alloc(c, N * 24 * 4, &npl));
    LF_TRACE(c, "theta/eta");
    launch_fold_witness(S[0].planes, S[1].planes, N, K, d_rho, npl, c->stream());
    u64 *nf = nullptr, *nw = nullptr;
    const size_t nf_bytes = N * 24 * 8, nw_bytes = (size_t)P.wit_len * 24 * 8;
    RET(lf_planes_alloc(c, nf_bytes, (int32_t **)&nf));
    RET(lf_planes_alloc(c, nw_bytes, (int32_t **)&nw));
// ... 89 lines not shown
```

latticefold_amd/csrc/lf_kernels.h:

```cpp
#pragma once
#include "lf_ajtai_i8.h"
#include "lf_sv_rounds.h"
#include <hip/hip_runtime.h>

#include "lf_host.h"

namespace lf {

struct DevCrt {
    u64 nu;
    int nu2p40;
    u64 w4, w2, w10, w1, w7, w5, w11;
    int slot_of_pos[8], pos1[8], pos2[8];
    u64 tw1[8], tw2[8];
};
DevCrt make_dev_crt(const CrtTables &T);

struct Fq3Const { u64 c[3]; };

void launch_aos_to_soa(const u64 *aos, u64 *soa, size_t n, hipStream_t s);
void launch_soa_to_aos(const u64 *soa, u64 *aos, size_t n, hipStream_t s);
void launch_fill_uniform(u64 *dst, size_t words, u64 seed, size_t start, hipStream_t s);
void launch_fill_ajtai(u64 *A, u32 kappa, size_t n, size_t n_total, size_t col0, u64 seed, hipStream_t s, u32 row0 = 0);

void launch_modsum(const u64 *parts, u32 nparts, size_t words, u64 *out, hipStream_t s);
void launch_gather_relayout(const u64 *all, u32 nranks, size_t planes, size_t lcl, u64 *full, hipStream_t s);
void launch_gather_relayout_part(const u64 *all, u32 nranks, size_t planes_tot, size_t p0, size_t planes, size_t lcl, u64 *full, hipStream_t s);

void launch_selftest_field(u64 seed, u32 n, u64 *mism_dev, hipStream_t s);

void launch_crt_fwd(const DevCrt &t, const u64 *coef, u64 *ntt, size_t n, hipStream_t s);
void launch_icrt_dense(const u64 *icrt_mat , const u64 *ntt, u64 *coef, size_t n, hipStream_t s);


void launch_decompose(const u64 *coef, size_t n, u64 base, u32 digits, int layout, u64 *out, hipStream_t s, int mode = 0);
void launch_recompose(const u64 *in, size_t n_out, u64 base, u32 digits, u64 *out, hipStream_t s);
void launch_coef_to_i32(const u64 *coef, int32_t *planes, size_t n, u32 bound, int *viol, hipStream_t s);
void launch_i32_to_coef(const int32_t *planes, u64 *coef, size_t n, hipStream_t s);
void launch_recompose_crt(const DevCrt &t, const int32_t *planes, size_t n_planes, u32 wit_len, u32 L, u64 B, u32 K,
                          int mode_bits, u64 *out, size_t ldz, size_t off, hipStream_t s);
void launch_linf(const u64 *coef, size_t n, u64 *out_max, hipStream_t s);


void launch_build_eq(const DevCrt &t, const Fq3Const *r_dev , u32 nv, u64 *eq , hipStream_t s);
size_t build_eq_scratch_words(u32 nv);
void launch_build_eq2(const DevCrt &t, const Fq3Const *r_dev, u32 nv, u64 *scratch, u64 *eq, hipStream_t s);
void launch_spmv(const DevCrt &t, const u32 *rowptr, const u32 *col, const u64 *val , const u64 *z,
                 size_t ldz, u64 *out, size_t m, int accumulate, hipStream_t s, size_t r0 = 0, size_t rcnt = (size_t)-1 );
void launch_spmv_sum(const DevCrt &t, u32 nm, const u32 *const *rowptr, const u32 *const *col, const u64 *const *val, const u64 *z,
                     size_t z_stride, size_t ldz, u64 *out, size_t m, hipStream_t s, size_t r0 = 0, size_t rcnt = (size_t)-1 );
void launch_spmv_rows(const DevCrt &t, u32 nm, const u32 *const *rowptr, const u32 *const *col, const u64 *const *val, const u64 *z, size_t z_stride, size_t n,
                      u64 *zaos, u64 *out, size_t m, int accumulate, hipStream_t s, size_t r0 = 0, size_t rcnt = (size_t)-1);
void launch_spmv_t_eq(const DevCrt &t, const u32 *colptr, const u32 *rowidx, const u64 *val, const u64 *eq, size_t m,
                      u64 *q, size_t n, hipStream_t s, size_t c0 = 0, size_t ccnt = (size_t)-1 );
void launch_dot_batch(const DevCrt &t, const u64 *X, size_t ldx, u32 na, const u64 *Y, size_t ldy, u32 nb, size_t n,
                      u64 *partial, u64 *out, hipStream_t s);
size_t dot_partial_words(u32 na, u32 nb);
void launch_dot_eq(const DevCrt &t, const u64 *X, size_t ldx, u32 na, const u64 *eq, size_t ldeq, size_t n, u64 *partial,
                   u64 *out, hipStream_t s);
void launch_coef_eval(const DevCrt &t, const int32_t *planes, size_t n, const u64 *eq, size_t ldeq, u32 K, int mode_bits,
                      u64 *partial, u64 *out, hipStream_t s, size_t ldp = 0);
size_t coef_eval_partial_words(u32 K);
void launch_lincomb_z(const DevCrt &t, const u64 *z, size_t ldz, u32 K, const Fq3Const *coef_dev , u32 tt, size_t n,
                      u64 *out, hipStream_t s, u32 per_slot = 0);
void launch_add_fhat_comb(const DevCrt &t, const int32_t *planes, size_t n_planes, u32 K, const Fq3Const *apow_dev ,
                          u64 *G, size_t m, hipStream_t s, size_t r0 = 0, size_t rcnt = (size_t)-1 );

void launch_fix_ring(const DevCrt &t, const u64 *in, u64 *out, size_t n_in, Fq3Const r, hipStream_t s);
void launch_fix_fq3(const DevCrt &t, const u64 *in, u64 *out, size_t n_in, Fq3Const r, hipStream_t s);
size_t dot_i8_yb_bytes(size_t n);
size_t dot_i8_part_words(size_t n);
size_t dot_i8_tot_words();
int launch_dot_batch_i8(const DevCrt &t, const u64 *X, size_t ldx, u32 na, const u64 *Y, size_t ldy, u32 nb, size_t n, unsigned char *YB, int32_t *part,
                        long long *tot, u64 *out, hipStream_t s, bool y_packed = false, u32 nb_out = 0, u32 b0 = 0);
int launch_dot_pack_y(const u64 *X, const u64 *Y, size_t ldy, u32 nb, size_t n, unsigned char *YB, hipStream_t s);
void launch_vs_combine(const u64 *vs , u32 K, u64 *v , hipStream_t s);
void launch_fix_final(const DevCrt &t, const u64 *in , u32 rows3, Fq3Const r, u64 *out , hipStream_t s);

struct LinCombDesc {
    u32 t, q;
    u32 S_off[9];
    u32 S_idx[16];
    u64 c[8][24];
    int c_unit[8];
    u32 first[8];
    u32 ms[8];
};
void launch_lin_round(const DevCrt &t, const LinCombDesc &desc, const u64 *mz, size_t ld, const u64 *eq, size_t ldeq, size_t n,
                      u32 deg, u64 *partial, u64 *out, hipStream_t s, u32 max_blocks = 0, u32 split_xmask = 0 );
void launch_lin_round_fused(const DevCrt &t, const LinCombDesc &desc, const u64 *mz_prev, size_t ld_prev, const u64 *eq_prev, size_t ldeq_prev, Fq3Const r, u64 *mz_out,
                            size_t ld_out, u64 *eq_out, size_t ldeq_out, size_t n, u32 deg, u64 *partial, u64 *out, hipStream_t s, u32 max_blocks = 0,
                            u32 split_xmask = 0 );
struct LinFix;
void launch_lin_round_wide(const DevCrt &t, const LinCombDesc &desc, const u64 *mz, size_t ld, const u64 *eq, size_t ldeq, size_t n, u32 deg, u64 *partial, u64 *out,
                           hipStream_t s, u32 max_blocks, u32 split_xmask, const LinFix *fx);
void launch_eq_pairsum(const u64 *in, size_t ld_in, size_t n_out, u64 *out, size_t ld_out, hipStream_t s);
void launch_eq_expand(const DevCrt &t, const u64 *E, size_t lde, size_t pairs, Fq3Const w0, Fq3Const w1, u64 *out, size_t ldo, hipStream_t s);

struct FoldRoundArgs {
    const u64 *eqL, *eqR, *eqB;
    const u64 *G1, *G2;
    size_t ld;
    size_t n;
    size_t p0, pcnt;
    size_t pF0;
};
void launch_fold_round1(const DevCrt &t, const FoldRoundArgs &a, const int32_t *planesL, const int32_t *planesR, size_t n_planes,
                        u32 K, const Fq3Const *mu_pow_dev , u64 *partial, u64 *out, hipStream_t s);
void launch_fold_round_g(const DevCrt &t, const FoldRoundArgs &a, u64 *partial, u64 *out, hipStream_t s);
void launch_fold_materialize(const DevCrt &t, const int32_t *planesL, const int32_t *planesR, size_t n_planes, size_t m, u32 K,
                             Fq3Const r1, u64 *F, hipStream_t s);
void launch_fold_round2(const DevCrt &t, const FoldRoundArgs &a, const int32_t *planesL, const int32_t *planesR, size_t n_planes, u32 K,
                        const Fq3Const *mu_pow_dev, Fq3Const r1, u64 *partial, u64 *out, hipStream_t s);
void launch_fold_round_tab(const DevCrt &t, int round, const FoldRoundArgs &a, const int32_t *planesL, const int32_t *planesR, size_t n_planes, u32 K,
                           const Fq3Const *mu_pow_dev, const u64 *poly_dev, u64 *tp_dev, u64 *partial, u64 *out, hipStream_t s);
void launch_fold_materialize2(const DevCrt &t, const int32_t *planesL, const int32_t *planesR, size_t n_planes, size_t j0, size_t q, u32 K,
                              const Fq3Const W[4], u64 *F, hipStream_t s);
void launch_fold_round(const DevCrt &t, const FoldRoundArgs &a, const u64 *F, size_t ldF, u32 K, const Fq3Const *mu_pow_dev,
                       u64 *partial, u64 *out, hipStream_t s);
void launch_fold_round_lut_fix_tab(const DevCrt &t, const FoldRoundArgs &a, const int32_t *planesL, const int32_t *planesR, size_t n_planes,
                                   const u64 *lut_dev, Fq3Const r, u64 *sq_dev, u64 *mt_dev, u64 *Fout, size_t ldout, u32 K, const Fq3Const *mu_pow_dev,
                                   u64 *partial, u64 *out, hipStream_t s, const u64 *E = nullptr, size_t ldE = 0 );
void launch_fold_round_lut_fix5(const DevCrt &t, const FoldRoundArgs &a, const int32_t *planesL, const int32_t *planesR, size_t n_planes,
                                const u64 *lut_dev, Fq3Const r3, Fq3Const r4, u64 *xx_dev, u64 *yy_dev, u64 *mt_dev, u64 *Fout, size_t ldout, u32 K,
                                const Fq3Const *mu_pow_dev, u64 *partial, u64 *out, hipStream_t s, const u64 *E = nullptr, size_t ldE = 0 );
void launch_fold_round_fix(const DevCrt &t, const FoldRoundArgs &a, const u64 *Fprev, size_t ldprev, Fq3Const r, u64 *Fout, size_t ldout, u32 K,
                           const Fq3Const *mu_pow_dev, u64 *partial, u64 *out, hipStream_t s, const u64 *E = nullptr, size_t ldE = 0 );
void launch_fold_round_lut(const DevCrt &t, const FoldRoundArgs &a, const int32_t *planesL, const int32_t *planesR, size_t n_planes,
                           const u64 *lut_dev, u32 K, const Fq3Const *mu_pow_dev, u64 *partial, u64 *out, hipStream_t s);
void launch_fold_round_lut_mu(const DevCrt &t, const FoldRoundArgs &a, const int32_t *planesL, const int32_t *planesR, size_t n_planes,
                              const u64 *lut_dev, u64 *mutab_dev, u32 K, const Fq3Const *mu_pow_dev, u64 *partial, u64 *out, hipStream_t s);
void launch_fold_round_lut_fix(const DevCrt &t, const FoldRoundArgs &a, const int32_t *planesL, const int32_t *planesR, size_t n_planes,
                               const u64 *lut_dev, Fq3Const r, u64 *Fout, size_t ldout, u32 K, const Fq3Const *mu_pow_dev, u64 *partial,
                               u64 *out, hipStream_t s);
size_t round_partial_words();

void launch_sponge_script(const u64 *ark, const u64 *mds, const u32 *ops, u32 nops, const u64 *words, u64 *out, u64 *state_out, hipStream_t s);

constexpr u32 TAIL_MAX_ROUNDS = 32;
struct TailMail {
    u64 msg[TAIL_MAX_ROUNDS][128];
    u32 msg_seq[TAIL_MAX_ROUNDS];
    u64 chal[TAIL_MAX_ROUNDS][4];
    u32 chal_seq[TAIL_MAX_ROUNDS];
    u32 abort_seq;
    u32 err;
    u64 chal_out[TAIL_MAX_ROUNDS][4];
    u64 sponge[32];
    u64 dbg[TAIL_MAX_ROUNDS][8];
};
struct FoldTailArgs {
    u64 *T[2];
    u64 *F[2];
    size_t n0;
    u32 rounds, K;
    const Fq3Const *mu_pow;
    u64 *partial;
    u64 *eqpriv;
    u32 *counters;
    u64 *dev_chal;
    TailMail *mail;
    u32 epoch;
    Fq3Const r_first;
    u32 dev_transcript;
    const u64 *pos_ark, *pos_mds;
    u64 *sponge_state;
};
struct LinTailArgs {
    const u64 *T;
    const u64 *E;
    u64 *Tout;
    size_t n0;
    u32 rounds, deg;
    u64 *partial;
    u64 *priv;
    u32 *counters;
    u64 *dev_chal;
    TailMail *mail;
    u32 epoch;
    Fq3Const r_first;
    u32 dev_transcript;
    const u64 *pos_ark, *pos_mds;
    u64 *sponge_state;
};
size_t lin_tail_priv_words(size_t n0, u32 t);
u32 launch_lin_tail(const DevCrt &t, const LinCombDesc &desc, const LinTailArgs &A, hipStream_t s);
constexpr u32 FOLD_TAIL_MAX_BLOCKS = 256;
size_t fold_tail_eqpriv_words(size_t n0, u32 K);
u32 launch_fold_tail(const DevCrt &t, const FoldTailArgs &A, int num_cus, hipStream_t s);

void launch_fold_witness(const int32_t *planesL, const int32_t *planesR, size_t n, u32 K, const int8_t *rho_dev, int32_t *out,
                         hipStream_t s);

}
```

latticefold_amd/csrc/lf_prove.cpp:

```cpp
#include "lf_ring_host.h"


void sc_prologue(Transcript &tr, u32 nv, u32 deg) {
    tr.absorb_u64_as_ring(nv);
    tr.absorb_u64_as_ring(deg);
}
Fq3 sc_round_transcript(Transcript &tr, const u64 *evals, u32 npts) {
    tr.absorb_ring(evals, npts);
    Fq3 r = tr.get_challenge();
    tr.absorb_fq3_as_ring(r);
    return r;
}

static int run_lin_sumcheck(lf_ctx *c, Transcript &tr, const u64 *mz, const u64 *eqb, u64 *msgs , Fq3 *point, u64 *u_dev = nullptr,
                            const std::function<void(u32)> *after_round = nullptr, const Fq3 *beta = nullptr) {
    const lf_params &P = c->P;
    u32 deg = P.d + 1;
    size_t m = c->m;
    u64 *fx[2], *fe[2], *partial, *od;
    RET(c->tbuf("lin_fix0", (size_t)P.t * 24 * (m / 2), &fx[0]));
    RET(c->tbuf("lin_fix1", (size_t)P.t * 24 * (m / 4 ? m / 4 : 1), &fx[1]));
    RET(c->tbuf("lin_efix0", 3 * (m / 2), &fe[0]));
    RET(c->tbuf("lin_efix1", 3 * (m / 4 ? m / 4 : 1), &fe[1]));
    RET(c->tbuf("round_partial", round_partial_words(), &partial));
// ... 619 lines not shown
    HIPCHK(hipSetDevice(c->device));
    std::vector<Fq3> rL;
    if (!lcccs_point(P, acc, rL)) return LF_ERR_UNSUPPORTED;
    c->tn = Tunables::read((size_t)1 << 14);
    Timeline tl;
    t_tl = &tl;
    c->ev_reset();
    c->host_tr_ms = 0;
    size_t tot = c->ev_begin(17);
    Transcript &tr = t->t;
    size_t ll = lf_lcccs_len(&P);
    u64 *lin_proof = proof, *decl = lin_proof + lin_proof_len(&P, 3) * 24, *decr = decl + dec_proof_len(&P, 3) * 24, *foldp = decr + dec_proof_len(&P, 3) * 24;
    std::vector<u64> lin(ll * 24);
    u64 *eq_r_R = nullptr;
    SideState S[2];
    std::promise<int> lin_done_p;
    std::shared_future<int> lin_done = lin_done_p.get_future().share();
    c->lin_blocks = 0;
    int rc;
    std::vector<Fq3> rR;
    const bool shard_threads = c->agreed_two_lanes >= 0 ? c->agreed_two_lanes == 1 : (c->tn.shard_two_lanes == 1 || (c->tn.shard_two_lanes < 0 && c->two_lanes_ok));
    if (P.b != 2) {
        u64 *ydL = nullptr, *ydR = nullptr;
        size_t evL = 0, evR = 0;
        rc = sb_cut_parts(c, w_acc, "sb_D_L", &S[0].D);
        if (rc == LF_OK) rc = sb_cut_parts(c, w_i, "sb_D_R", &S[1].D);
        if (rc == LF_OK) rc = decompose_commit_enqueue(c, w_acc, &ydL, &evL, "dec_y", S[0].D);
        if (rc == LF_OK) rc = decompose_commit_finish(c, acc + ((size_t)P.s + 3) * 24, ydL, evL, decl);
        if (rc == LF_OK) rc = decompose_evals(c, acc, rL, w_acc, "L", nullptr, S[0], decl);
        if (rc == LF_OK) rc = decompose_commit_enqueue(c, w_i, &ydR, &evR, "dec_y2", S[1].D);
        if (rc == LF_OK) {
            HostTimer ht(c);
            tr.absorb_label("acc");
            tr.absorb_ring(acc, ll);
            tr.absorb_label("cm_i");
            tr.absorb_ring(cm_i, lf_cccs_len(&P));
        }
        if (rc == LF_OK) rc = linearize_impl(c, tr, cm_i, w_i, lin.data(), lin_proof, &eq_r_R);
        if (rc == LF_OK) {
            lcccs_point(P, lin.data(), rR);
            rc = decompose_evals(c, lin.data(), rR, w_i, "R", eq_r_R, S[1], decr);
        }
        if (rc == LF_OK) c->host_tr_ms += absorb_decomposition(P, tr, acc, decl, S[0]);
        if (rc == LF_OK) rc = decompose_commit_finish(c, cm_i, ydR, evR, decr);
        if (rc == LF_OK) c->host_tr_ms += absorb_decomposition(P, tr, lin.data(), decr, S[1]);
    } else
    if (c->sh_world > 1 && !shard_threads) {
        auto on_lane1 = [&](auto &&fn) -> int { t_lane = 1; int r = fn(); t_lane = 0; return r; };
        u64 *ydL = nullptr, *ydR = nullptr;
        size_t evL = 0, evR = 0;
        rc = on_lane1([&]() -> int {
            RET(decompose_commit_enqueue(c, w_acc, &ydL, &evL));
            RET(decompose_commit_finish(c, acc + ((size_t)P.s + 3) * 24, ydL, evL, decl));
            RET(decompose_evals(c, acc, rL, w_acc, "L", nullptr, S[0], decl));
            return decompose_commit_enqueue(c, w_i, &ydR, &evR);
        });
        {
            HostTimer ht(c);
            tr.absorb_label("acc");
            tr.absorb_ring(acc, ll);
            tr.absorb_label("cm_i");
            tr.absorb_ring(cm_i, lf_cccs_len(&P));
        }
        if (rc == LF_OK) rc = linearize_impl(c, tr, cm_i, w_i, lin.data(), lin_proof, &eq_r_R);
        if (rc == LF_OK) {
            lcccs_point(P, lin.data(), rR);
            rc = decompose_evals(c, lin.data(), rR, w_i, "R", eq_r_R, S[1], decr);
        }
        if (rc == LF_OK) c->host_tr_ms += absorb_decomposition(P, tr, acc, decl, S[0]);
        if (rc == LF_OK) rc = on_lane1([&]() -> int { return decompose_commit_finish(c, cm_i, ydR, evR, decr); });
        c->lin_blocks = 0;
        if (rc == LF_OK) c->host_tr_ms += absorb_decomposition(P, tr, lin.data(), decr, S[1]);
    } else {
    c->bits_wit[0] = c->bits_wit[1] = nullptr;
    if (!c->tn.fold_no_sv && !c->tn.force_exchange && c->N <= c->m && (c->N & 3) == 0 && !c->tn.fold_tab_r1 && (c->m >> 1) >= c->tn.sv_min) {
        const lf_witness *ws[2] = {w_acc, w_i};
        for (int sd = 0; sd < 2; sd++) {
            u32 *bits;
            if (c->tbuf(sd ? "sv_bits_R" : "sv_bits_L", sv_bits_words(c->N, P.K), &bits) != LF_OK) break;
            if (!c->bits_ev[sd] && hipEventCreateWithFlags(&c->bits_ev[sd], hipEventDisableTiming) != hipSuccess) break;
            launch_sv_bits(ws[sd]->planes, c->N, c->N, P.K, bits, c->st_lane[1]);
            if (hipEventRecord(c->bits_ev[sd], c->st_lane[1]) != hipSuccess) break;
            c->bits_wit[sd] = ws[sd]; c->bits_ptr[sd] = bits;
            S[sd].sv_bits = bits;
        }
    }
    c->lane1.submit([&]() -> int {
        t_lane = 1;
        struct Publish {
            SideState &s;
            ~Publish() { int e = 0; s.z_state.compare_exchange_strong(e, -1, std::memory_order_release); }
        } publish{S[1]};
        if (hipSetDevice(c->device) != hipSuccess) return LF_ERR_HIP;
        Timeline *const tl1 = &tl;
        u64 *yd = nullptr, *ydL = nullptr;
        size_t ev = 0;
        bool yR_early = false;
        const u64 *yR_host = nullptr;
        size_t evL = 0;
        RET(decompose_evals(c, acc, rL, w_acc, "L", nullptr, S[0], decl));
        tl1->mark1("L1: left evals down");
        {
            std::vector<u64> xh((size_t)(P.l + 1) * 24);
            memcpy(xh.data(), cm_i + (size_t)P.kappa * 24, (size_t)P.l * 24 * 8);
            HostRing::from_u64(1, xh.data() + (size_t)P.l * 24);
            (void)decompose_prepare_z(c, xh.data(), w_i, "R", S[1], decr);
        }
        RET(decompose_commit_enqueue(c, w_acc, &ydL, &evL));
        const size_t ywords = (size_t)(P.K - 1) * P.kappa * 24;
        const bool early = c->sh_world == 1 && !c->tn.force_exchange && c->pin2(2 * ywords) == LF_OK &&
                           (c->ev_yL || hipEventCreateWithFlags(&c->ev_yL, hipEventDisableTiming) == hipSuccess) &&
                           (c->ev_yR || hipEventCreateWithFlags(&c->ev_yR, hipEventDisableTiming) == hipSuccess);
        bool yL_early = false;
        if (early && hipMemcpyAsync(c->h_pin2, ydL, ywords * 8, hipMemcpyDeviceToHost, c->stream()) == hipSuccess && hipEventRecord(c->ev_yL, c->stream()) == hipSuccess)
            yL_early = true;
        RET(decompose_commit_enqueue(c, w_i, &yd, &ev, "dec_y2"));
        if (early && hipMemcpyAsync(c->h_pin2 + ywords, yd, ywords * 8, hipMemcpyDeviceToHost, c->stream()) == hipSuccess && hipEventRecord(c->ev_yR, c->stream()) == hipSuccess) {
            yR_early = true;
            yR_host = c->h_pin2 + ywords;
        }
        tl1->mark1("L1: commits + z_R enqueued");
        RET(decompose_commit_finish(c, acc + ((size_t)P.s + 3) * 24, ydL, evL, decl, yL_early ? c->h_pin2 : nullptr, yL_early ? c->ev_yL : nullptr));
        tl1->mark1("L1: y_L down");
        if (lin_done.get() != LF_OK) return LF_OK;
        tl1->mark1("L1: left absorb starts");
        absorb_decomposition(P, tr, acc, decl, S[0]);
        tl1->mark1("L1: left absorb done");
        return decompose_commit_finish(c, cm_i, yd, ev, decr, yR_early ? yR_host : nullptr, yR_early ? c->ev_yR : nullptr);
    });
    {
        HostTimer ht(c);
        tr.absorb_label("acc");
        tr.absorb_ring(acc, ll);
        tr.absorb_label("cm_i");
        tr.absorb_ring(cm_i, lf_cccs_len(&P));
    }
    TL_MARK("public input absorbed");
    c->vs_keep = true;
    rc = linearize_impl(c, tr, cm_i, w_i, lin.data(), lin_proof, &eq_r_R);
    c->vs_keep = false;
    TL_MARK("linearization done");
    lin_done_p.set_value(rc);
    if (rc == LF_OK) {
        lcccs_point(P, lin.data(), rR);
        while (S[1].z_state.load(std::memory_order_acquire) == 0) std::this_thread::yield();
        rc = decompose_evals(c, lin.data(), rR, w_i, "R", eq_r_R, S[1], decr);
    }
    c->vs_wit = nullptr;
    TL_MARK("right evals done");
    int rc1 = c->lane1.wait();
    c->lin_blocks = 0;
    TL_MARK("lane 1 joined");
    if (rc == LF_OK) rc = rc1;
    if (rc == LF_OK) c->host_tr_ms += absorb_decomposition(P, tr, lin.data(), decr, S[1]);
    }
    TL_MARK("right absorb done");
    if (rc == LF_OK) rc = fold_impl(c, tr, S, lcccs_out, w_out, foldp);
    c->bits_wit[0] = c->bits_wit[1] = nullptr;
    TL_MARK("fold done");
    tl.merge();
    tl.dump();
    c->tl_marks = tl.marks;
    t_tl = nullptr;
    c->ev_end(tot);
    c->ev_collect();
    if (rc != LF_OK && c->sh_world > 1) { c->comm[0].abort_peers(); c->comm[1].abort_peers(); }
    return rc;
}

int lf_decomposition_prove(lf_ctx *c, lf_transcript *t, const uint64_t *lcccs, const lf_witness *wit, uint64_t *lcccs_s_out, uint64_t *dec_proof_out) {
    if (LF_XB(c) && t && lcccs && dec_proof_out && c->have_ccs_any()) {
        XB x(c);
        const lf_params &P = c->params_any();
        const int ring = lf_ctx_ring(c);
        const size_t ll = lf_lcccs_len_ring(&P, ring);
        x.transcript(t);
        int rc = lf_decomposition_prove(c, t, x.ring_in(lcccs, ll), wit, lcccs_s_out, dec_proof_out);
        if (rc == LF_OK) { x.ring_out(lcccs_s_out, (size_t)P.K * ll); x.ring_out(dec_proof_out, (size_t)P.K * (P.t + x.TAU + P.l + 1 + P.kappa)); }
        return rc;
    }
    if (!c || !t || !lcccs || !wit || !dec_proof_out || wit->ctx != c) return LF_ERR_INVALID;
    if (c->bb) return t->bb ? c->bb->decomposition_prove(*t->bb, lcccs, wit, lcccs_s_out, dec_proof_out) : LF_ERR_INVALID;
    if (t->bb) return LF_ERR_INVALID;
    std::lock_guard<std::mutex> g(c->mu);
    if (!c->have_ccs || !c->A_loaded) return LF_ERR_STATE;
    const lf_params &P = c->P;
    if (c->kappa != P.kappa || c->nA_total != c->N || wit->N != c->N) return LF_ERR_INVALID;
    HIPCHK(hipSetDevice(c->device));
    std::vector<Fq3> r;
    if (!lcccs_point(P, lcccs, r)) return LF_ERR_UNSUPPORTED;
    c->tn = Tunables::read((size_t)1 << 14);
    c->ev_reset();
    c->host_tr_ms = 0;
    u64 *yd = nullptr;
    size_t ev = 0;
    SideState S;
    if (P.b != 2) RET(sb_cut_parts(c, wit, "sb_D_L", &S.D));
    RET(decompose_commit_enqueue(c, wit, &yd, &ev, "dec_y", S.D));
    RET(decompose_commit_finish(c, lcccs + ((size_t)P.s + 3) * 24, yd, ev, dec_proof_out));
    RET(decompose_evals(c, lcccs, r, wit, "L", nullptr, S, dec_proof_out));
    c->host_tr_ms += absorb_decomposition(P, t->t, lcccs, dec_proof_out, S);
    if (lcccs_s_out) memcpy(lcccs_s_out, S.lcccs.data(), S.lcccs.size() * 8);
    c->ev_collect();
    return LF_OK;
}

int lf_folding_prove(lf_ctx *c, lf_transcript *t, const uint64_t *lcccs_s, const lf_witness *w_left, const lf_witness *w_right,
                     uint64_t *lcccs_out, lf_witness **w_out, uint64_t *fold_proof_out) {
    if (LF_XB(c) && t && lcccs_s && lcccs_out && fold_proof_out && c->have_ccs_any()) {
        XB x(c);
        const lf_params &P = c->params_any();
        const int ring = lf_ctx_ring(c);
        const size_t ll = lf_lcccs_len_ring(&P, ring);
        x.transcript(t);
        int rc = lf_folding_prove(c, t, x.ring_in(lcccs_s, 2 * (size_t)P.K * ll), w_left, w_right, lcccs_out, w_out, fold_proof_out);
        if (rc == LF_OK) { x.ring_out(lcccs_out, ll); x.ring_out(fold_proof_out, (size_t)P.s * (2 * P.b + 1) + 2 * (size_t)P.K * (x.TAU + P.t)); }
        return rc;
    }
    if (!c || !t || !lcccs_s || !w_left || !w_right || !lcccs_out || !w_out || !fold_proof_out) return LF_ERR_INVALID;
    if (w_left->ctx != c || w_right->ctx != c) return LF_ERR_INVALID;
    if (c->bb) return t->bb ? c->bb->folding_prove(*t->bb, lcccs_s, w_left, w_right, lcccs_out, w_out, fold_proof_out) : LF_ERR_INVALID;
    if (t->bb) return LF_ERR_INVALID;
    std::lock_guard<std::mutex> g(c->mu);
    if (!c->have_ccs) return LF_ERR_STATE;
    const lf_params &P = c->P;
    if (w_left->N != c->N || w_right->N != c->N) return LF_ERR_INVALID;
    HIPCHK(hipSetDevice(c->device));
    c->tn = Tunables::read((size_t)1 << 14);
    c->ev_reset();
    c->host_tr_ms = 0;
    const size_t ll = lf_lcccs_len(&P);
    const u32 K = P.K, hl = P.l + 1;
    SideState S[2];
    for (int sd = 0; sd < 2; sd++) {
        const u64 *base = lcccs_s + (size_t)sd * K * ll * 24;
        std::vector<Fq3> r;
        if (!lcccs_point(P, base, r)) return LF_ERR_UNSUPPORTED;
        for (u32 k = 1; k < K; k++)
            if (memcmp(base, base + (size_t)k * ll * 24, (size_t)P.s * 24 * 8) != 0) return LF_ERR_INVALID;
        const lf_witness *w = sd ? w_right : w_left;
        u64 *z, *eq_r;
        RET(c->tbuf(sd ? "z_R" : "z_L", (size_t)K * 24 * c->n, &z));
        RET(c->tbuf(sd ? "eq_r_R" : "eq_r_L", 3 * c->m, &eq_r));
        std::vector<u64> heads((size_t)K * hl * 24);
        for (u32 k = 0; k < K; k++)
            memcpy(&heads[(size_t)k * hl * 24], base + ((size_t)k * ll + P.s + 3 + P.kappa + P.t) * 24, (size_t)hl * 24 * 8);
        if (P.b != 2) RET(sb_cut_parts(c, w, sd ? "sb_D_R" : "sb_D_L", &S[sd].D));
        RET(build_z(c, w->planes, K, 1, heads.data(), z, 0, (size_t)-1, S[sd].D));
        RET(build_eq_dev(c, r.data(), P.s, eq_r));
        S[sd].planes = w->planes; S[sd].z = z; S[sd].eq_r = eq_r;
        S[sd].lcccs.assign(base, base + (size_t)K * ll * 24);
    }
    int rc = fold_impl(c, t->t, S, lcccs_out, w_out, fold_proof_out);
    c->ev_collect();
    return rc;
}
```

latticefold_amd/csrc/lf_rounds.hip:

```cpp
#include "lf_kernels.h"

#include <stdlib.h>

#include "lf_kernels_dev.cuh"

namespace lf {

template <int NP>
__device__ __forceinline__ void add_poly_evals(Fq3 (&acc)[NP], const Fq3 *co, int ncoef) {
#pragma unroll
    for (int X = 0; X < NP; X++) {
        Fq3 v = co[ncoef - 1];
        for (int e = ncoef - 2; e >= 0; e--) v = fq3_add(fq3_mul_small(v, X), co[e]);
        acc[X] = fq3_add(acc[X], v);
    }
}

template <bool NU, bool FUSED, bool SPLIT>
__global__ void __launch_bounds__(256) k_lin_round(DevCrt t, LinCombDesc desc, const u64 *mz, size_t ld, const u64 *eq, size_t ldeq, size_t n,
                                                   u32 deg, u64 *partial, LinFix fx, u32 xmask) {
    u32 slot = blockIdx.y;
    size_t pairs = n / 2;
    Fq3 acc[5];
#pragma unroll
// ... 404 lines not shown
#pragma unroll 1
            for (int pass = 0; pass < 2; pass++) {
                int64_t lo[2][4][3], hi[2][4][3];
                int32_t cs[2][4];
#pragma unroll
                for (int e = 0; e < 2; e++)
#pragma unroll
                    for (int j = 0; j < 4; j++) {
                        cs[e][j] = 0;
#pragma unroll
                        for (int c = 0; c < 3; c++) { lo[e][j][c] = 0; hi[e][j][c] = 0; }
                    }
                for (int side = 0; side < 2; side++) {
                    const int32_t *pl = side ? planesR : planesL;
                    for (int d = 0; d < 3; d++) {
                        const int32_t *src = pl + (size_t)(8 * d + slot) * n_planes + 4 * p;
                        int32_t w0 = src[0];
                        int32_t w1 = 4 * p + 1 < n_planes ? src[1] : 0, w2 = 4 * p + 2 < n_planes ? src[2] : 0, w3 = 4 * p + 3 < n_planes ? src[3] : 0;
                        for (u32 k = 0; k < K; k++) {
                            int d0 = digit2(w0, k), d1 = digit2(w1, k), d2 = digit2(w2, k), d3 = digit2(w3, k);
                            int u0 = d0, u1 = d2 - d0, v0 = d1 - d0, v1 = (d3 - d2) - v0;
                            int cf[2][4];
                            if (pass == 0) {
                                int u0s = u0 * u0;
                                cf[0][0] = u0s * u0 - u0; cf[0][1] = 3 * u0s * u1 - u1; cf[0][2] = 3 * u0 * u1 * u1; cf[0][3] = u1 * u1 * u1;
                                cf[1][0] = 3 * u0s * v0 - v0; cf[1][1] = 3 * (u0s * v1 + 2 * u0 * u1 * v0) - v1;
                                cf[1][2] = 3 * (2 * u0 * u1 * v1 + u1 * u1 * v0); cf[1][3] = 3 * u1 * u1 * v1;
                            } else {
                                int v0s = v0 * v0, v1s = v1 * v1;
                                cf[0][0] = 3 * u0 * v0s; cf[0][1] = 3 * (2 * u0 * v0 * v1 + u1 * v0s); cf[0][2] = 3 * (u0 * v1s + 2 * u1 * v0 * v1);
                                cf[0][3] = 3 * u1 * v1s;
                                cf[1][0] = v0s * v0; cf[1][1] = 3 * v0s * v1; cf[1][2] = 3 * v0 * v1s; cf[1][3] = v1s * v1;
                            }
                            Fq3Const m = mu_pow[(side * K + k) * 3 + d];
#pragma unroll
                            for (int e = 0; e < 2; e++)
#pragma unroll
                                for (int j = 0; j < 4; j++) cs[e][j] += cf[e][j];
#pragma unroll
                            for (int c = 0; c < 3; c++) {
                                int32_t ml = (int32_t)((u32)m.c[c] ^ 0x80000000u), mh = (int32_t)((u32)(m.c[c] >> 32) ^ 0x80000000u);
#pragma unroll
                                for (int e = 0; e < 2; e++)
#pragma unroll
                                    for (int j = 0; j < 4; j++) { lo[e][j][c] += (int64_t)ml * cf[e][j]; hi[e][j][c] += (int64_t)mh * cf[e][j]; }
                            }
                        }
                    }
                }
#pragma unroll
                for (int e = 0; e < 2; e++)
#pragma unroll
                    for (int j = 0; j < 4; j++) {
                        Fq3 T;
#pragma unroll
                        for (int c = 0; c < 3; c++) {
                            int64_t off = (int64_t)cs[e][j] << 31;
                            T.c[c] = fq_add(fq_from_i64(lo[e][j][c] + off), fq_mul(fq_from_i64(hi[e][j][c] + off), 1ULL << 32));
                        }
                        if (pass == 0 && e == 0) Q[j] = fq3_add(Q[j], T);
                        else Q[j] = fq3_add(Q[j], M3<NU>(T, pass == 0 ? r1 : (e == 0 ? r1s : r1c3), nu));
                    }
            }
        }
        fold_g2_finish<NU>(acc, Q, a, p, nu);
    }
    add_poly_evals<5>(acc, gco, 3);
    store_round_partial(acc, slot, partial);
}
void launch_fold_round2(const DevCrt &t, const FoldRoundArgs &a, const int32_t *planesL, const int32_t *planesR, size_t n_planes, u32 K,
                        const Fq3Const *mu_pow_dev, Fq3Const r1, u64 *partial, u64 *out, hipStream_t s) {
    u32 gb = (u32)((a.pcnt + 255) / 256);
    if (gb > RED_BLOCKS) gb = RED_BLOCKS;
    if (gb < 1) gb = 1;
    LF_LAUNCH(k_fold_round2, t.nu2p40, dim3(gb, 8), dim3(256), s, t, a, planesL, planesR, n_planes, K, mu_pow_dev, r1, partial);
    hipLaunchKernelGGL(k_reduce_rows, dim3(5 * 24), dim3(256), 0, s, partial, gb, 120, out);
}

__global__ void __launch_bounds__(256) k_fold_materialize2(const int32_t *planesL, const int32_t *planesR, size_t n_planes, size_t j0, size_t q, u32 K,
                                                           Fq3Const W0, Fq3Const W1, Fq3Const W2, Fq3Const W3, u64 *F) {
    size_t jl = (size_t)blockIdx.x * 256 + threadIdx.x;
    u32 cidx = blockIdx.y;
    if (jl >= q) return;
    size_t j = j0 + jl;
    u32 d = cidx / 8, slot = cidx % 8;
    const Fq3Const W[4] = {W0, W1, W2, W3};
    for (int side = 0; side < 2; side++) {
        const int32_t *pl = (side ? planesR : planesL) + (size_t)cidx * n_planes;
        int32_t v[4];
#pragma unroll
        for (int b = 0; b < 4; b++) v[b] = 4 * j + b < n_planes ? pl[4 * j + b] : 0;
        for (u32 k = 0; k < K; k++) {
            u64 acc[3] = {0, 0, 0};
#pragma unroll
            for (int b = 0; b < 4; b++) {
                int dg = digit2(v[b], k);
#pragma unroll
                for (int c = 0; c < 3; c++) {
                    u64 w = W[b].c[c];
                    acc[c] = dg > 0 ? fq_add(acc[c], w) : (dg < 0 ? fq_sub(acc[c], w) : acc[c]);
                }
            }
            u64 *dst = F + (((size_t)(side * K + k) * 3 + d) * 24 + 3 * slot) * q + jl;
            dst[0] = acc[0]; dst[q] = acc[1]; dst[2 * q] = acc[2];
        }
    }
}
void launch_fold_materialize2(const DevCrt &t, const int32_t *planesL, const int32_t *planesR, size_t n_planes, size_t j0, size_t q, u32 K,
                              const Fq3Const W[4], u64 *F, hipStream_t s) {
    hipLaunchKernelGGL(k_fold_materialize2, dim3(cdiv(q, 256), 24), dim3(256), 0, s, planesL, planesR, n_planes, j0, q, K, W[0], W[1], W[2], W[3], F);
}

__global__ void __launch_bounds__(256) k_fold_materialize(const int32_t *planesL, const int32_t *planesR, size_t n_planes, size_t m, u32 K,
                                                          Fq3Const r1, u64 *F) {
    size_t j = (size_t)blockIdx.x * 256 + threadIdx.x;
    u32 cidx = blockIdx.y;
    size_t half = m / 2;
    if (j >= half) return;
    u32 d = cidx / 8, slot = cidx % 8;
    u64 mul[5][3];
#pragma unroll
    for (int c = 0; c < 3; c++) {
        u64 r = r1.c[c], r2 = fq_add(r, r);
        mul[0][c] = fq_neg(r2); mul[1][c] = fq_neg(r); mul[2][c] = 0; mul[3][c] = r; mul[4][c] = r2;
    }
    for (int side = 0; side < 2; side++) {
        const int32_t *pl = (side ? planesR : planesL) + (size_t)cidx * n_planes;
        int32_t v0 = 2 * j < n_planes ? pl[2 * j] : 0, v1 = 2 * j + 1 < n_planes ? pl[2 * j + 1] : 0;
        for (u32 k = 0; k < K; k++) {
            int f0 = digit2(v0, k), df = digit2(v1, k) - f0;
            u64 *dst = F + (((size_t)(side * K + k) * 3 + d) * 24 + 3 * slot) * half + j;
            dst[0] = fq_add(fq_from_digit(f0), mul[df + 2][0]);
            dst[half] = mul[df + 2][1];
            dst[2 * half] = mul[df + 2][2];
        }
    }
}
void launch_fold_materialize(const DevCrt &t, const int32_t *planesL, const int32_t *planesR, size_t n_planes, size_t m, u32 K, Fq3Const r1,
                             u64 *F, hipStream_t s) {
    hipLaunchKernelGGL(k_fold_materialize, dim3(cdiv(m / 2, 256), 24), dim3(256), 0, s, planesL, planesR, n_planes, m, K, r1, F);
}

struct FoldSrc {
    u64 *out; size_t ldo;
    Fq3Const r;
    const int32_t *planesL, *planesR;
    size_t n_planes;
    const u64 *lut;
    const u64 *mutab;
    Fq3Const r_prev;
    const u64 *xx5, *yy5, *mt5;
    const u64 *sq4, *mt4;
    const u64 *E; size_t ldE;
};
template <bool NU>
__global__ void __launch_bounds__(128) k_fold_mutab(DevCrt t, const u64 *lut, const Fq3Const *mu_pow, u32 nkd, u64 *mutab) {
    u32 kd = blockIdx.x, code = threadIdx.x;
    if (code >= 81) return;
    Fq3 L = fq3_make(lut[3 * code], lut[3 * code + 1], lut[3 * code + 2]);
    Fq3Const mc = mu_pow[kd];
    Fq3 m1 = M3<NU>(fq3_make(mc.c[0], mc.c[1], mc.c[2]), L, t.nu), m2 = M3<NU>(m1, L, t.nu), m3 = M3<NU>(m2, L, t.nu);
    const Fq3 v[3] = {m1, m2, m3};
#pragma unroll
    for (int q = 0; q < 3; q++) {
        u64 *o = mutab + (((size_t)q * nkd + kd) * 81 + code) * 4;
        o[0] = v[q].c[0]; o[1] = v[q].c[1]; o[2] = v[q].c[2]; o[3] = 0;
    }
}
template <bool NU>
__global__ void __launch_bounds__(256) k_fold_r4tab(DevCrt t, const u64 *lut, Fq3Const r, const Fq3Const *mu_pow, u32 nkd, u64 *sq, u64 *mt) {
    const u32 i = blockIdx.x * 256 + threadIdx.x;
    const Fq3 rr = fq3_make(r.c[0], r.c[1], r.c[2]);
    auto L = [&](u32 c) { return fq3_make(lut[3 * c], lut[3 * c + 1], lut[3 * c + 2]); };
    if (i < 6561) {
        const u32 c0 = i / 81, c1 = i % 81;
        const Fq3 l0 = L(c0), f = fq3_add(l0, M3<NU>(fq3_sub(L(c1), l0), rr, t.nu)), sv = M3<NU>(f, f, t.nu);
        u64 *o = sq + (size_t)i * 4;
        o[0] = sv.c[0]; o[1] = sv.c[1]; o[2] = sv.c[2]; o[3] = 0;
    } else if (i < 6561 + nkd * 162) {
        const u32 j = i - 6561, kd = j / 162, w = (j % 162) / 81, c = j % 81;
        const Fq3 l = L(c), rl = M3<NU>(l, rr, t.nu);
        const Fq3Const mc = mu_pow[kd];
        const Fq3 m = M3<NU>(fq3_make(mc.c[0], mc.c[1], mc.c[2]), w ? rl : fq3_sub(l, rl), t.nu);
        u64 *o = mt + (((size_t)kd * 2 + w) * 81 + c) * 4;
        o[0] = m.c[0]; o[1] = m.c[1]; o[2] = m.c[2]; o[3] = 0;
    }
}
template <bool NU>
__device__ __forceinline__ Fq3 r5_entry(const u64 *lut, u32 w, u32 c, Fq3 r3, Fq3 r4, u64 nu) {
    const Fq3 l = fq3_make(lut[3 * c], lut[3 * c + 1], lut[3 * c + 2]), rl = M3<NU>(l, r3, nu), a = (w & 1) ? rl : fq3_sub(l, rl), ra = M3<NU>(a, r4, nu);
    return (w & 2) ? ra : fq3_sub(a, ra);
}
template <bool NU>
__global__ void __launch_bounds__(256) k_fold_r5tab(DevCrt t, const u64 *lut, Fq3Const r3c, Fq3Const r4c, const Fq3Const *mu_pow, u32 nkd, u64 *xx, u64 *yy, u64 *mt) {
    const u32 i = blockIdx.x * 256 + threadIdx.x;
    const Fq3 r3 = fq3_make(r3c.c[0], r3c.c[1], r3c.c[2]), r4 = fq3_make(r4c.c[0], r4c.c[1], r4c.c[2]);
    if (i < 2 * 6561) {
        const u32 hi = i / 6561, j = i % 6561, c0 = j / 81, c1 = j % 81;
        const Fq3 f = fq3_add(r5_entry<NU>(lut, 2 * hi, c0, r3, r4, t.nu), r5_entry<NU>(lut, 2 * hi + 1, c1, r3, r4, t.nu)), sv = M3<NU>(f, f, t.nu);
        u64 *o = (hi ? yy : xx) + (size_t)j * 4;
        o[0] = sv.c[0]; o[1] = sv.c[1]; o[2] = sv.c[2]; o[3] = 0;
    } else if (i < 2 * 6561 + nkd * 324) {
        const u32 j = i - 2 * 6561, kd = j / 324, w = (j % 324) / 81, c = j % 81;
        const Fq3Const mc = mu_pow[kd];
        const Fq3 m = M3<NU>(fq3_make(mc.c[0], mc.c[1], mc.c[2]), r5_entry<NU>(lut, w, c, r3, r4, t.nu), t.nu);
        u64 *o = mt + (((size_t)kd * 4 + w) * 81 + c) * 4;
        o[0] = m.c[0]; o[1] = m.c[1]; o[2] = m.c[2]; o[3] = 0;
    }
}
__device__ __forceinline__ u32 digit_code4(const int32_t *v, u32 k) {
    int code = 40;
    const int w[4] = {1, 3, 9, 27};
#pragma unroll
    for (int b = 0; b < 4; b++) {
        int32_t x = v[b], mg = x < 0 ? -x : x;
        int bit = (mg >> k) & 1;
        code += x < 0 ? -bit * w[b] : bit * w[b];
    }
    return (u32)code;
}
template <bool NU, int MODE, bool SPLIT = false>
__global__ void __launch_bounds__(256) k_fold_round(DevCrt t, FoldRoundArgs a, const u64 *F, size_t ldF, u32 K, const Fq3Const *mu_pow,
                                                    FoldSrc src, u64 *partial) {
    static_assert(!SPLIT || (NU && (MODE == 1 || MODE == 6 || MODE == 7)), "split form: the large-round modes of the 2^40 non-residue path");
    constexpr int NA = SPLIT ? 3 : 5;
    u32 slot = blockIdx.y;
    const size_t pend = a.p0 + a.pcnt;
    const u64 nu = t.nu;
    const u32 nkd = 2 * K * 3, per = (nkd + gridDim.z - 1) / gridDim.z;
    const u32 kd0 = blockIdx.z * per, kd1 = kd0 + per < nkd ? kd0 + per : nkd;
    if (MODE == 0) F -= 2 * a.pF0;
    if (MODE == 1) { F -= 4 * a.pF0; src.out -= 2 * a.pF0; }
    if ((MODE == 4 || MODE == 6 || MODE == 7) && src.out) src.out -= 2 * a.pF0;
    const Fq3 rfix = fq3_make(src.r.c[0], src.r.c[1], src.r.c[2]);
    __shared__ u64 slut[MODE == 7 ? 4 * 81 * 3 : (MODE >= 3 ? 3 * 81 * 3 : 1)];
    if (MODE == 7) {
        for (u32 i = threadIdx.x; i < 4 * 81; i += 256) {
            const Fq3 e = r5_entry<NU>(src.lut, i / 81, i % 81, fq3_make(src.r_prev.c[0], src.r_prev.c[1], src.r_prev.c[2]), rfix, nu);
            slut[3 * i] = e.c[0]; slut[3 * i + 1] = e.c[1]; slut[3 * i + 2] = e.c[2];
        }
        __syncthreads();
    } else
    if (MODE >= 3) {
        for (u32 i = threadIdx.x; i < 2 * 81 * 3; i += 256) slut[i] = src.lut[i];
        __syncthreads();
        if (MODE == 4 || MODE == 6) {
            if (threadIdx.x < 81) {
                Fq3 rv = M3<NU>(fq3_make(slut[3 * threadIdx.x], slut[3 * threadIdx.x + 1], slut[3 * threadIdx.x + 2]), rfix, nu);
                slut[3 * (162 + threadIdx.x)] = rv.c[0]; slut[3 * (162 + threadIdx.x) + 1] = rv.c[1]; slut[3 * (162 + threadIdx.x) + 2] = rv.c[2];
            }
            __syncthreads();
        }
    }
    auto lut3 = [&](u32 code) { return fq3_make(slut[3 * code], slut[3 * code + 1], slut[3 * code + 2]); };
    Fq3 acc[NA];
#pragma unroll
    for (int i = 0; i < NA; i++) acc[i] = fq3_zero();
    for (size_t p = a.p0 + (size_t)blockIdx.x * 256 + threadIdx.x; p < pend; p += (size_t)gridDim.x * 256) {
        if constexpr (!SPLIT)
        if (blockIdx.z == 0) fold_g13_evals<NU>(acc, a, slot, p, nu);
        auto load_pair = [&](u32 kd, Fq3 &f0, Fq3 &df) {
            if (MODE == 0) {
                const u64 *fp = F + ((size_t)kd * 24 + 3 * slot) * ldF;
                ulonglong2 x0 = *(const ulonglong2 *)(fp + 2 * p), x1 = *(const ulonglong2 *)(fp + ldF + 2 * p), x2 = *(const ulonglong2 *)(fp + 2 * ldF + 2 * p);
                f0 = fq3_make(x0.x, x1.x, x2.x);
                df = fq3_sub(fq3_make(x0.y, x1.y, x2.y), f0);
            } else if (MODE == 1) {
                const u64 *fp = F + ((size_t)kd * 24 + 3 * slot) * ldF + 4 * p;
                ulonglong2 a0 = *(const ulonglong2 *)(fp), a1 = *(const ulonglong2 *)(fp + ldF), a2 = *(const ulonglong2 *)(fp + 2 * ldF);
                ulonglong2 b0 = *(const ulonglong2 *)(fp + 2), b1 = *(const ulonglong2 *)(fp + ldF + 2), b2 = *(const ulonglong2 *)(fp + 2 * ldF + 2);
                Fq3 lo = fq3_make(a0.x, a1.x, a2.x), hi = fq3_make(b0.x, b1.x, b2.x);
                f0 = fq3_add(lo, M3<NU>(fq3_sub(fq3_make(a0.y, a1.y, a2.y), lo), rfix, nu));
                Fq3 f1 = fq3_add(hi, M3<NU>(fq3_sub(fq3_make(b0.y, b1.y, b2.y), hi), rfix, nu));
                u64 *op = src.out + ((size_t)kd * 24 + 3 * slot) * src.ldo + 2 * p;
                *(ulonglong2 *)(op) = make_ulonglong2(f0.c[0], f1.c[0]);
                *(ulonglong2 *)(op + src.ldo) = make_ulonglong2(f0.c[1], f1.c[1]);
                *(ulonglong2 *)(op + 2 * src.ldo) = make_ulonglong2(f0.c[2], f1.c[2]);
                df = fq3_sub(f1, f0);
            } else {
                constexpr int NE = MODE == 4 ? 16 : 8;
                const u32 side = kd / (3 * K), k = (kd / 3) % K, d = kd % 3;
                const int32_t *pl = (side ? src.planesR : src.planesL) + (size_t)(d * 8 + slot) * src.n_planes + (size_t)NE * p;
                int32_t v[NE];
                if ((size_t)NE * p + NE <= src.n_planes && (src.n_planes & 3) == 0) {
#pragma unroll
                    for (int q = 0; q < NE / 4; q++) {
                        int4 w = *(const int4 *)(pl + 4 * q);
                        v[4 * q] = w.x; v[4 * q + 1] = w.y; v[4 * q + 2] = w.z; v[4 * q + 3] = w.w;
                    }
                } else {
#pragma unroll
                    for (int q = 0; q < NE; q++) v[q] = (size_t)NE * p + q < src.n_planes ? pl[q] : 0;
                }
                if (MODE != 4) {
                    f0 = lut3(digit_code4(v, k));
                    df = fq3_sub(lut3(digit_code4(v + 4, k)), f0);
                } else {
                    const u32 c0 = digit_code4(v, k), c1 = digit_code4(v + 4, k), c2 = digit_code4(v + 8, k), c3 = digit_code4(v + 12, k);
                    f0 = fq3_add(lut3(c0), fq3_sub(lut3(162 + c1), lut3(162 + c0)));
                    Fq3 f1 = fq3_add(lut3(c2), fq3_sub(lut3(162 + c3), lut3(162 + c2)));
                    u64 *op = src.out + ((size_t)kd * 24 + 3 * slot) * src.ldo + 2 * p;
                    *(ulonglong2 *)(op) = make_ulonglong2(f0.c[0], f1.c[0]);
                    *(ulonglong2 *)(op + src.ldo) = make_ulonglong2(f0.c[1], f1.c[1]);
                    *(ulonglong2 *)(op + 2 * src.ldo) = make_ulonglong2(f0.c[2], f1.c[2]);
                    df = fq3_sub(f1, f0);
                }
            }
        };
        Fq3 Q[4];
        if (NU && MODE == 5) {
            LH5 A1, A2;
            lh5_zero(A1); lh5_zero(A2);
            u64 s64[12];
            u32 scy[12];
#pragma unroll
            for (int i = 0; i < 12; i++) { s64[i] = 0; scy[i] = 0; }
            auto ladd = [&](int base, const ulonglong2 &a, u64 b) {
                const u64 w[3] = {a.x, a.y, b};
#pragma unroll
                for (int q = 0; q < 3; q++) { u64 sm = s64[base + q] + w[q]; scy[base + q] += sm < w[q]; s64[base + q] = sm; }
            };
            const u32 nkd_all = 2 * K * 3;
            for (u32 kd = kd0; kd < kd1; kd++) {
                const u32 side = kd / (3 * K), k = (kd / 3) % K, d = kd % 3;
                const int32_t *pl = (side ? src.planesR : src.planesL) + (size_t)(d * 8 + slot) * src.n_planes + (size_t)8 * p;
                int32_t v[8];
                if ((size_t)8 * p + 8 <= src.n_planes && (src.n_planes & 3) == 0) {
                    int4 w0 = *(const int4 *)pl, w1 = *(const int4 *)(pl + 4);
                    v[0] = w0.x; v[1] = w0.y; v[2] = w0.z; v[3] = w0.w; v[4] = w1.x; v[5] = w1.y; v[6] = w1.z; v[7] = w1.w;
                } else {
#pragma unroll
                    for (int q = 0; q < 8; q++) v[q] = (size_t)8 * p + q < src.n_planes ? pl[q] : 0;
                }
                const u32 c0 = digit_code4(v, k), c1 = digit_code4(v + 4, k);
                const u64 *t1 = src.mutab + ((size_t)kd * 81) * 4, *t2 = t1 + (size_t)nkd_all * 81 * 4, *t3 = t2 + (size_t)nkd_all * 81 * 4;
                ulonglong2 m10 = *(const ulonglong2 *)(t1 + 4 * c0), m11 = *(const ulonglong2 *)(t1 + 4 * c1);
                ulonglong2 m20 = *(const ulonglong2 *)(t2 + 4 * c0), m21 = *(const ulonglong2 *)(t2 + 4 * c1);
                ulonglong2 m30 = *(const ulonglong2 *)(t3 + 4 * c0), m31 = *(const ulonglong2 *)(t3 + 4 * c1);
                u64 m10c = t1[4 * c0 + 2], m11c = t1[4 * c1 + 2], m20c = t2[4 * c0 + 2], m21c = t2[4 * c1 + 2], m30c = t3[4 * c0 + 2], m31c = t3[4 * c1 + 2];
                ladd(0, m30, m30c); ladd(3, m31, m31c); ladd(6, m10, m10c); ladd(9, m11, m11c);
                lh5_mac(A1, fq3_make(m20.x, m20.y, m20c), lut3(c1));
                lh5_mac(A2, fq3_make(m21.x, m21.y, m21c), lut3(c0));
            }
            auto lfin = [&](int base) {
                return fq3_make(fq_canon(fq_reduce128_loose(s64[base], (u64)scy[base])), fq_canon(fq_reduce128_loose(s64[base + 1], (u64)scy[base + 1])),
                                fq_canon(fq_reduce128_loose(s64[base + 2], (u64)scy[base + 2])));
            };
            Fq3 P0 = lfin(0), P3 = lfin(3), sp = lfin(6), su = lfin(9), P1 = lh5_finish(A1), P2 = lh5_finish(A2);
            Fq3 a1 = fq3_sub(P1, P0);
            Fq3 a2 = fq3_add(fq3_sub(P2, fq3_add(P1, P1)), P0);
            Fq3 p12 = fq3_sub(P1, P2);
            Fq3 a3 = fq3_add(fq3_sub(P3, P0), fq3_add(fq3_add(p12, p12), p12));
            Q[0] = fq3_sub(P0, sp);
            Q[1] = fq3_sub(fq3_add(fq3_add(a1, a1), a1), fq3_sub(su, sp));
            Q[2] = fq3_add(fq3_add(a2, a2), a2);
            Q[3] = a3;
        } else if (NU && MODE == 7) {
            LH5 A0, A1, A2, A3;
            lh5_zero(A0); lh5_zero(A1); lh5_zero(A2); lh5_zero(A3);
            Fq3 sp = fq3_zero(), su = fq3_zero();
            for (u32 kd = kd0; kd < kd1; kd++) {
                const u32 side = kd / (3 * K), k = (kd / 3) % K, d = kd % 3;
                const int32_t *pl = (side ? src.planesR : src.planesL) + (size_t)(d * 8 + slot) * src.n_planes + (size_t)32 * p;
                const u64 *mt = src.mt5 + (size_t)kd * 4 * 81 * 4;
                Fq3 fv[2], sq[2], mf[2];
#pragma unroll
                for (int e = 0; e < 2; e++) {
                    int32_t v[16];
                    if ((size_t)32 * p + 16 * e + 16 <= src.n_planes && (src.n_planes & 3) == 0) {
#pragma unroll
                        for (int q = 0; q < 4; q++) {
                            int4 w = *(const int4 *)(pl + 16 * e + 4 * q);
                            v[4 * q] = w.x; v[4 * q + 1] = w.y; v[4 * q + 2] = w.z; v[4 * q + 3] = w.w;
                        }
                    } else {
#pragma unroll
                        for (int q = 0; q < 16; q++) v[q] = (size_t)32 * p + 16 * e + q < src.n_planes ? pl[16 * e + q] : 0;
                    }
                    const u32 c0 = digit_code4(v, k), c1 = digit_code4(v + 4, k), c2 = digit_code4(v + 8, k), c3 = digit_code4(v + 12, k);
                    const u64 *qx = src.xx5 + (size_t)(c0 * 81 + c1) * 4, *qy = src.yy5 + (size_t)(c2 * 81 + c3) * 4;
                    const ulonglong2 xa = *(const ulonglong2 *)qx, ya = *(const ulonglong2 *)qy;
                    const u64 xc = qx[2], yc = qy[2];
                    const ulonglong2 m0 = *(const ulonglong2 *)(mt + 4 * c0), m1 = *(const ulonglong2 *)(mt + 4 * (81 + c1));
                    const ulonglong2 m2 = *(const ulonglong2 *)(mt + 4 * (162 + c2)), m3 = *(const ulonglong2 *)(mt + 4 * (243 + c3));
                    const u64 m0c = mt[4 * c0 + 2], m1c = mt[4 * (81 + c1) + 2], m2c = mt[4 * (162 + c2) + 2], m3c = mt[4 * (243 + c3) + 2];
                    const Fq3 X = fq3_add(lut3(c0), lut3(81 + c1)), Y = fq3_add(lut3(162 + c2), lut3(243 + c3));
                    const Fq3 xy = fq3_mul_2p40(X, Y);
                    fv[e] = fq3_add(X, Y);
                    sq[e] = fq3_add(fq3_add(fq3_make(xa.x, xa.y, xc), fq3_make(ya.x, ya.y, yc)), fq3_add(xy, xy));
                    mf[e] = fq3_add(fq3_add(fq3_make(m0.x, m0.y, m0c), fq3_make(m1.x, m1.y, m1c)), fq3_add(fq3_make(m2.x, m2.y, m2c), fq3_make(m3.x, m3.y, m3c)));
                }
                u64 *op = src.out + ((size_t)kd * 24 + 3 * slot) * src.ldo + 2 * p;
                *(ulonglong2 *)(op) = make_ulonglong2(fv[0].c[0], fv[1].c[0]);
                *(ulonglong2 *)(op + src.ldo) = make_ulonglong2(fv[0].c[1], fv[1].c[1]);
                *(ulonglong2 *)(op + 2 * src.ldo) = make_ulonglong2(fv[0].c[2], fv[1].c[2]);
                lh5_mac(A0, mf[0], sq[0]); lh5_mac(A1, mf[1], sq[0]); lh5_mac(A2, mf[0], sq[1]);
                if constexpr (!SPLIT) lh5_mac(A3, mf[1], sq[1]);
                sp = fq3_add(sp, mf[0]); su = fq3_add(su, mf[1]);
            }
            Fq3 P0 = lh5_finish(A0), P1 = lh5_finish(A1), P2 = lh5_finish(A2);
            Fq3 a1 = fq3_sub(P1, P0);
            Fq3 a2 = fq3_add(fq3_sub(P2, fq3_add(P1, P1)), P0);
            Q[0] = fq3_sub(P0, sp);
            Q[1] = fq3_sub(fq3_add(fq3_add(a1, a1), a1), fq3_sub(su, sp));
            Q[2] = fq3_add(fq3_add(a2, a2), a2);
            if constexpr (!SPLIT) {
                Fq3 P3 = lh5_finish(A3), p12 = fq3_sub(P1, P2);
                Q[3] = fq3_add(fq3_sub(P3, P0), fq3_add(fq3_add(p12, p12), p12));
            } else Q[3] = fq3_zero();
        } else if (NU && MODE == 6) {
            LH5 A0, A1, A2, A3;
            lh5_zero(A0); lh5_zero(A1); lh5_zero(A2); lh5_zero(A3);
            Fq3 sp = fq3_zero(), su = fq3_zero();
            auto gen = [&](u32 kd, Fq3 &tt, Fq3 &uu, Fq3 &s0, Fq3 &s1) {
                const u32 side = kd / (3 * K), k = (kd / 3) % K, d = kd % 3;
                const int32_t *pl = (side ? src.planesR : src.planesL) + (size_t)(d * 8 + slot) * src.n_planes + (size_t)16 * p;
                int32_t v[16];
                if ((size_t)16 * p + 16 <= src.n_planes && (src.n_planes & 3) == 0) {
#pragma unroll
                    for (int q = 0; q < 4; q++) {
                        int4 w = *(const int4 *)(pl + 4 * q);
                        v[4 * q] = w.x; v[4 * q + 1] = w.y; v[4 * q + 2] = w.z; v[4 * q + 3] = w.w;
                    }
                } else {
#pragma unroll
                    for (int q = 0; q < 16; q++) v[q] = (size_t)16 * p + q < src.n_planes ? pl[q] : 0;
                }
                const u32 c0 = digit_code4(v, k), c1 = digit_code4(v + 4, k), c2 = digit_code4(v + 8, k), c3 = digit_code4(v + 12, k);
                const u64 *q0 = src.sq4 + (size_t)(c0 * 81 + c1) * 4, *q1 = src.sq4 + (size_t)(c2 * 81 + c3) * 4;
                const u64 *ma = src.mt4 + (size_t)kd * 2 * 81 * 4, *mb = ma + 81 * 4;
                const ulonglong2 s0a = *(const ulonglong2 *)q0, s1a = *(const ulonglong2 *)q1;
                const u64 s0c = q0[2], s1c = q1[2];
                const ulonglong2 a0 = *(const ulonglong2 *)(ma + 4 * c0), b1 = *(const ulonglong2 *)(mb + 4 * c1);
                const ulonglong2 a2 = *(const ulonglong2 *)(ma + 4 * c2), b3 = *(const ulonglong2 *)(mb + 4 * c3);
                const u64 a0c = ma[4 * c0 + 2], b1c = mb[4 * c1 + 2], a2c = ma[4 * c2 + 2], b3c = mb[4 * c3 + 2];
                if (src.out) {
                    const Fq3 f0 = fq3_add(lut3(c0), fq3_sub(lut3(162 + c1), lut3(162 + c0)));
                    const Fq3 f1 = fq3_add(lut3(c2), fq3_sub(lut3(162 + c3), lut3(162 + c2)));
                    u64 *op = src.out + ((size_t)kd * 24 + 3 * slot) * src.ldo + 2 * p;
                    *(ulonglong2 *)(op) = make_ulonglong2(f0.c[0], f1.c[0]);
                    *(ulonglong2 *)(op + src.ldo) = make_ulonglong2(f0.c[1], f1.c[1]);
                    *(ulonglong2 *)(op + 2 * src.ldo) = make_ulonglong2(f0.c[2], f1.c[2]);
                }
                tt = fq3_add(fq3_make(a0.x, a0.y, a0c), fq3_make(b1.x, b1.y, b1c));
                uu = fq3_add(fq3_make(a2.x, a2.y, a2c), fq3_make(b3.x, b3.y, b3c));
                s0 = fq3_make(s0a.x, s0a.y, s0c);
                s1 = fq3_make(s1a.x, s1a.y, s1c);
                sp = fq3_add(sp, tt); su = fq3_add(su, uu);
            };
            u32 kd = kd0;
            for (; kd + 1 < kd1; kd += 2) {
                Fq3 tA, uA, xA, yA, tB, uB, xB, yB;
                gen(kd, tA, uA, xA, yA);
                gen(kd + 1, tB, uB, xB, yB);
                lh5_mac2(A0, tA, xA, tB, xB); lh5_mac2(A1, uA, xA, uB, xB); lh5_mac2(A2, tA, yA, tB, yB);
                if constexpr (!SPLIT) lh5_mac2(A3, uA, yA, uB, yB);
            }
            if (kd < kd1) {
                Fq3 tA, uA, xA, yA;
                gen(kd, tA, uA, xA, yA);
                lh5_mac(A0, tA, xA); lh5_mac(A1, uA, xA); lh5_mac(A2, tA, yA);
                if constexpr (!SPLIT) lh5_mac(A3, uA, yA);
            }
            Fq3 P0 = lh5_finish(A0), P1 = lh5_finish(A1), P2 = lh5_finish(A2);
            Fq3 a1 = fq3_sub(P1, P0);
            Fq3 a2 = fq3_add(fq3_sub(P2, fq3_add(P1, P1)), P0);
            Q[0] = fq3_sub(P0, sp);
            Q[1] = fq3_sub(fq3_add(fq3_add(a1, a1), a1), fq3_sub(su, sp));
            Q[2] = fq3_add(fq3_add(a2, a2), a2);
            if constexpr (!SPLIT) {
                Fq3 P3 = lh5_finish(A3), p12 = fq3_sub(P1, P2);
                Q[3] = fq3_add(fq3_sub(P3, P0), fq3_add(fq3_add(p12, p12), p12));
            } else Q[3] = fq3_zero();
        } else if (NU && MODE == 3) {
            LH5 A0, A1, A2, A3;
            lh5_zero(A0); lh5_zero(A1); lh5_zero(A2); lh5_zero(A3);
            Fq3 sp = fq3_zero(), su = fq3_zero();
            for (u32 kd = kd0; kd < kd1; kd++) {
                const u32 side = kd / (3 * K), k = (kd / 3) % K, d = kd % 3;
                const int32_t *pl = (side ? src.planesR : src.planesL) + (size_t)(d * 8 + slot) * src.n_planes + (size_t)8 * p;
                int32_t v[8];
                if ((size_t)8 * p + 8 <= src.n_planes && (src.n_planes & 3) == 0) {
                    int4 w0 = *(const int4 *)pl, w1 = *(const int4 *)(pl + 4);
                    v[0] = w0.x; v[1] = w0.y; v[2] = w0.z; v[3] = w0.w; v[4] = w1.x; v[5] = w1.y; v[6] = w1.z; v[7] = w1.w;
                } else {
#pragma unroll
                    for (int q = 0; q < 8; q++) v[q] = (size_t)8 * p + q < src.n_planes ? pl[q] : 0;
                }
                const u32 c0 = digit_code4(v, k), c1 = digit_code4(v + 4, k);
                Fq3 f0 = lut3(c0), f1 = lut3(c1), s0 = lut3(81 + c0), s1 = lut3(81 + c1);
                Fq3Const mc = mu_pow[kd];
                Fq3 mu = fq3_make(mc.c[0], mc.c[1], mc.c[2]);
                Fq3 tt = fq3_mul_2p40(mu, f0), uu = fq3_mul_2p40(mu, f1);
                lh5_mac(A0, tt, s0); lh5_mac(A1, uu, s0); lh5_mac(A2, tt, s1); lh5_mac(A3, uu, s1);
                sp = fq3_add(sp, tt); su = fq3_add(su, uu);
            }
            Fq3 P0 = lh5_finish(A0), P1 = lh5_finish(A1), P2 = lh5_finish(A2), P3 = lh5_finish(A3);
            Fq3 a1 = fq3_sub(P1, P0);
            Fq3 a2 = fq3_add(fq3_sub(P2, fq3_add(P1, P1)), P0);
            Fq3 p12 = fq3_sub(P1, P2);
            Fq3 a3 = fq3_add(fq3_sub(P3, P0), fq3_add(fq3_add(p12, p12), p12));
            Q[0] = fq3_sub(P0, sp);
            Q[1] = fq3_sub(fq3_add(fq3_add(a1, a1), a1), fq3_sub(su, sp));
            Q[2] = fq3_add(fq3_add(a2, a2), a2);
            Q[3] = a3;
        } else if (NU) {
            LH5 A0, A1, A2, A3;
            lh5_zero(A0); lh5_zero(A1); lh5_zero(A2); lh5_zero(A3);
            Fq3 sp = fq3_zero(), sq = fq3_zero();
            for (u32 kd = kd0; kd < kd1; kd++) {
                Fq3 f0, df;
                load_pair(kd, f0, df);
                Fq3Const mc = mu_pow[kd];
                Fq3 mu = fq3_make(mc.c[0], mc.c[1], mc.c[2]);
                Fq3 f0s = fq3_mul_2p40(f0, f0), dfs = fq3_mul_2p40(df, df);
                Fq3 pp = fq3_mul_2p40(mu, f0), qq = fq3_mul_2p40(mu, df);
                lh5_mac(A0, pp, f0s); lh5_mac(A1, qq, f0s); lh5_mac(A2, pp, dfs);
                if constexpr (!SPLIT) lh5_mac(A3, qq, dfs);
                sp = fq3_add(sp, pp); sq = fq3_add(sq, qq);
            }
            Fq3 t1 = lh5_finish(A1), t2 = lh5_finish(A2);
            Q[0] = fq3_sub(lh5_finish(A0), sp);
            Q[1] = fq3_sub(fq3_add(fq3_add(t1, t1), t1), sq);
            Q[2] = fq3_add(fq3_add(t2, t2), t2);
            if constexpr (!SPLIT) Q[3] = lh5_finish(A3);
            else Q[3] = fq3_zero();
        } else {
            Q[0] = Q[1] = Q[2] = Q[3] = fq3_zero();
            for (u32 kd = kd0; kd < kd1; kd++) {
                Fq3 f0, df;
                load_pair(kd, f0, df);
                Fq3 f0s = S3<NU>(f0, nu), dfs = S3<NU>(df, nu);
                Fq3 c0 = fq3_sub(M3<NU>(f0s, f0, nu), f0);
                Fq3 c3 = M3<NU>(dfs, df, nu);
                Fq3 t1 = M3<NU>(f0s, df, nu), t2 = M3<NU>(dfs, f0, nu);
                Fq3 c1 = fq3_sub(fq3_add(fq3_add(t1, t1), t1), df);
                Fq3 c2 = fq3_add(fq3_add(t2, t2), t2);
                Fq3Const mc = mu_pow[kd];
                Fq3 mu = fq3_make(mc.c[0], mc.c[1], mc.c[2]);
                Q[0] = fq3_add(Q[0], M3<NU>(c0, mu, nu));
                Q[1] = fq3_add(Q[1], M3<NU>(c1, mu, nu));
                Q[2] = fq3_add(Q[2], M3<NU>(c2, mu, nu));
                Q[3] = fq3_add(Q[3], M3<NU>(c3, mu, nu));
            }
        }
        if constexpr (SPLIT) {
            const Fq3 E = fq3_make(src.E[p], src.E[src.ldE + p], src.E[2 * src.ldE + p]);
#pragma unroll
            for (int e = 0; e < 3; e++) acc[e] = fq3_add(acc[e], M3<NU>(Q[e], E, nu));
        } else fold_g2_finish<NU>(acc, Q, a, p, nu);
    }
    u64 vv[3 * NA];
#pragma unroll
    for (int i = 0; i < NA; i++) { vv[3 * i] = acc[i].c[0]; vv[3 * i + 1] = acc[i].c[1]; vv[3 * i + 2] = acc[i].c[2]; }
    __shared__ u64 red[3 * NA];
    block_sum_store<3 * NA>(vv, red);
    __syncthreads();
    size_t row = (size_t)blockIdx.x + (size_t)gridDim.x * blockIdx.z;
    if (threadIdx.x < 3 * NA) partial[row * (24 * NA) + (threadIdx.x / 3) * 24 + 3 * slot + threadIdx.x % 3] = red[threadIdx.x];
}
static size_t fold_chunk_threads() {
    constexpr size_t v = 131072;
    return v;
}
template <int MODE>
static void launch_fold_round_mode(const DevCrt &t, const FoldRoundArgs &a, const u64 *F, size_t ldF, u32 K, const Fq3Const *mu_pow_dev,
                                   const FoldSrc &src, u64 *partial, u64 *out, hipStream_t s) {
    size_t pairs = a.pcnt;
    u32 gb = (u32)((pairs + 255) / 256);
    if (gb > RED_BLOCKS) gb = RED_BLOCKS;
    if (gb < 1) gb = 1;
    u32 nkd = 2 * K * 3, chunks = 1;
    static const u32 cand[] = {1, 2, 3, 4, 6, 8, 12, 16, 24, 32, 48, 96};
    for (u32 cc : cand) {
        if (cc > nkd) break;
        chunks = cc;
        if (pairs * 8 * cc >= fold_chunk_threads()) break;
    }
    while (gb * chunks > RED_BLOCKS && chunks > 1) chunks--;
    if (MODE >= 3) chunks = 1;
    if constexpr (MODE == 1 || MODE == 6 || MODE == 7) {
        if (src.E && t.nu2p40) {
            hipLaunchKernelGGL((k_fold_round<true, MODE, true>), dim3(gb, 8, chunks), dim3(256), 0, s, t, a, F, ldF, K, mu_pow_dev, src, partial);
            hipLaunchKernelGGL(k_reduce_rows, dim3(3 * 24), dim3(256), 0, s, partial, gb * chunks, 72, out);
            return;
        }
    }
    if (t.nu2p40) hipLaunchKernelGGL((k_fold_round<true, MODE>), dim3(gb, 8, chunks), dim3(256), 0, s, t, a, F, ldF, K, mu_pow_dev, src, partial);
    else hipLaunchKernelGGL((k_fold_round<false, MODE>), dim3(gb, 8, chunks), dim3(256), 0, s, t, a, F, ldF, K, mu_pow_dev, src, partial);
    hipLaunchKernelGGL(k_reduce_rows, dim3(5 * 24), dim3(256), 0, s, partial, gb * chunks, 120, out);
}
void launch_fold_round(const DevCrt &t, const FoldRoundArgs &a, const u64 *F, size_t ldF, u32 K, const Fq3Const *mu_pow_dev, u64 *partial,
                       u64 *out, hipStream_t s) {
    FoldSrc src = {};
    launch_fold_round_mode<0>(t, a, F, ldF, K, mu_pow_dev, src, partial, out, s);
}
struct SpongeDev {
    int idx;
    int squeezing;
};
__device__ __forceinline__ void wave_lds_sync() { __builtin_amdgcn_fence(__ATOMIC_ACQ_REL, "workgroup"); __builtin_amdgcn_wave_barrier(); }
__device__ void poseidon_permute_wave(u64 *st , u64 *tmp , const u64 *ark, const u64 *mds) {
    const int lane = threadIdx.x & 63;
    for (int r = 0; r < 30; r++) {
        const bool full = r < 4 || r >= 26;
        if (lane < 24) {
            u64 x = fq_add(st[lane], ark[r * 24 + lane]);
            if (full || lane == 0) {
                u64 x2 = fq_mul(x, x), x4 = fq_mul(x2, x2), x6 = fq_mul(x4, x2);
                x = fq_mul(x6, x);
            }
            tmp[lane] = fq_canon(x);
        }
        wave_lds_sync();
        if (lane < 24) {
            const u64 *row = mds + lane * 24;
            Acc a;
            acc_set(a, row[0], tmp[0]);
#pragma unroll 4
            for (int j = 1; j < 24; j++) acc_mad(a, row[j], tmp[j]);
            st[lane] = fq_canon(acc_reduce(a));
        }
        wave_lds_sync();
    }
}
__device__ void sponge_absorb_wave(SpongeDev &sp, u64 *st, u64 *tmp, const u64 *ark, const u64 *mds, const u64 *x , int n) {
    const int lane = threadIdx.x & 63;
    if (n <= 0) return;
    int idx;
    if (!sp.squeezing) {
        idx = sp.idx;
        if (idx == 20) { poseidon_permute_wave(st, tmp, ark, mds); idx = 0; }
    } else {
        poseidon_permute_wave(st, tmp, ark, mds);
        idx = 0;
    }
    for (;;) {
        const int take = idx + n <= 20 ? n : 20 - idx;
        if (lane < take) st[4 + idx + lane] = fq_add(st[4 + idx + lane], fq_canon(x[lane]));
        wave_lds_sync();
        if (take == n) { sp.squeezing = 0; sp.idx = idx + n; return; }
        poseidon_permute_wave(st, tmp, ark, mds);
        x += take; n -= take; idx = 0;
    }
}
__device__ void sponge_squeeze_wave(SpongeDev &sp, u64 *st, u64 *tmp, const u64 *ark, const u64 *mds, u64 *out , int n) {
    const int lane = threadIdx.x & 63;
    int idx;
    if (!sp.squeezing) { poseidon_permute_wave(st, tmp, ark, mds); idx = 0; }
    else {
        idx = sp.idx;
        if (idx == 20) { poseidon_permute_wave(st, tmp, ark, mds); idx = 0; }
    }
    for (;;) {
        const int take = idx + n <= 20 ? n : 20 - idx;
        if (lane < take) out[lane] = st[4 + idx + lane];
        wave_lds_sync();
        if (take == n) { sp.squeezing = 1; sp.idx = idx + n; return; }
        if (n != 20) poseidon_permute_wave(st, tmp, ark, mds);
        out += take; n -= take; idx = 0;
    }
}
__global__ void __launch_bounds__(64) k_sponge_script(const u64 *ark, const u64 *mds, const u32 *ops, u32 nops, const u64 *words, u64 *out, u64 *state_out) {
    __shared__ u64 st[24], tmp[24];
    const int lane = threadIdx.x;
    if (lane < 24) st[lane] = 0;
    wave_lds_sync();
    SpongeDev sp;
    sp.idx = 0; sp.squeezing = 0;
    for (u32 i = 0; i < nops; i++) {
        const u32 kind = ops[i] >> 24;
        const int cnt = (int)(ops[i] & 0xffffff);
        if (kind == 0) { sponge_absorb_wave(sp, st, tmp, ark, mds, words, cnt); words += cnt; }
        else { sponge_squeeze_wave(sp, st, tmp, ark, mds, out, cnt); out += cnt; }
    }
    if (lane < 24) state_out[lane] = st[lane];
    if (lane == 0) { state_out[24] = (u64)sp.idx; state_out[25] = (u64)sp.squeezing; }
}
void launch_sponge_script(const u64 *ark, const u64 *mds, const u32 *ops, u32 nops, const u64 *words, u64 *out, u64 *state_out, hipStream_t s) {
    hipLaunchKernelGGL(k_sponge_script, dim3(1), dim3(64), 0, s, ark, mds, ops, nops, words, out, state_out);
}

__device__ __forceinline__ u32 ld_sys_u32(const u32 *p) { return __hip_atomic_load(p, __ATOMIC_RELAXED, __HIP_MEMORY_SCOPE_SYSTEM); }
__device__ __forceinline__ u64 ld_sys_u64(const u64 *p) { return __hip_atomic_load(p, __ATOMIC_RELAXED, __HIP_MEMORY_SCOPE_SYSTEM); }
__device__ __forceinline__ u64 ld_dev_u64(const u64 *p) { return __hip_atomic_load(p, __ATOMIC_RELAXED, __HIP_MEMORY_SCOPE_AGENT); }
__device__ __forceinline__ void st_dev_u64(u64 *p, u64 v) { __hip_atomic_store(p, v, __ATOMIC_RELAXED, __HIP_MEMORY_SCOPE_AGENT); }
__device__ __forceinline__ void wait_mem() { asm volatile("s_waitcnt vmcnt(0) lgkmcnt(0)" ::: "memory"); }
constexpr u64 TAIL_TIMEOUT_TICKS = 400000000ull;
constexpr u64 TAIL_ABORT_BIT = 1ull << 40;
#ifdef LF_TAIL_DEBUG
#define TAIL_STAMP(mail, rd, k) __hip_atomic_store((u64 *)&(mail)->dbg[rd][k], (u64)wall_clock64(), __ATOMIC_RELAXED, __HIP_MEMORY_SCOPE_SYSTEM)
#else
#define TAIL_STAMP(mail, rd, k) do { } while (0)
#endif

__device__ bool tail_wait_challenge(TailMail *mail, u64 *dev_chal, u32 idx, u32 epoch, bool leader, u64 *r_out) {
    u64 *slot = dev_chal + (size_t)idx * 4;
    const u64 t0 = wall_clock64();
    if (leader) {
        u32 st = 0;
        for (u32 it = 0;; it++) {
            if (ld_sys_u32((const u32 *)&mail->chal_seq[idx]) == epoch) { st = 1; TAIL_STAMP(mail, idx + 1, 0); break; }
            if ((it & 63) == 63) {
                if (ld_sys_u32((const u32 *)&mail->abort_seq) == epoch) break;
                if (wall_clock64() - t0 > TAIL_TIMEOUT_TICKS) { __hip_atomic_store((u32 *)&mail->err, epoch, __ATOMIC_RELAXED, __HIP_MEMORY_SCOPE_SYSTEM); break; }
            }
        }
        if (st) {
            u64 v[3];
            for (int q = 0; q < 3; q++) v[q] = ld_sys_u64((const u64 *)&mail->chal[idx][q]);
            for (int q = 0; q < 3; q++) st_dev_u64(slot + q, v[q]);
        }
        wait_mem();
        st_dev_u64(slot + 3, st ? (u64)epoch : ((u64)epoch | TAIL_ABORT_BIT));
        TAIL_STAMP(mail, idx + 1, 1);
    }
    for (u32 it = 0;; it++) {
        u64 v = ld_dev_u64(slot + 3);
        if (v == (u64)epoch) break;
        if (v == ((u64)epoch | TAIL_ABORT_BIT)) return false;
        if ((it & 255) == 255 && wall_clock64() - t0 > 2 * TAIL_TIMEOUT_TICKS) return false;
        __builtin_amdgcn_s_sleep(1);
    }
    for (int q = 0; q < 3; q++) r_out[q] = ld_dev_u64(slot + q);
    return true;
}

template <bool NU>
__global__ void __launch_bounds__(256) k_fold_tail(DevCrt t, FoldTailArgs A) {
    const u32 slot = blockIdx.y;
    const u64 nu = t.nu;
    const u32 nkd = 2 * A.K * 3, per = (nkd + gridDim.z - 1) / gridDim.z;
    const u32 kd0 = blockIdx.z * per, kd1 = kd0 + per < nkd ? kd0 + per : nkd;
// ... 263 lines not shown
                    Fq3 res = fq3_zero(), term = fq3_zero();
                    int sgn = 0;
#pragma unroll
                    for (int j = 0; j < 4; j++) {
                        if ((u32)j < nt) {
                            if (desc.first[j]) {
                                if (sgn) res = sgn < 0 ? fq3_sub(res, term) : fq3_add(res, term);
                                u32 i = desc.ms[j];
                                if (desc.c_unit[i]) { term = v[j]; sgn = desc.c_unit[i]; }
                                else { term = M3<NU>(fq3_make(desc.c[i][3 * slot], desc.c[i][3 * slot + 1], desc.c[i][3 * slot + 2]), v[j], nu); sgn = 1; }
                            } else term = M3<NU>(term, v[j], nu);
                        }
                    }
                    if (sgn) res = sgn < 0 ? fq3_sub(res, term) : fq3_add(res, term);
                    const Fq3 gx = M3<NU>(res, ev, nu);
                    if (X == 0) acc[0] = fq3_add(acc[0], gx);
                    else if (X == 1) acc[1] = fq3_add(acc[1], gx);
                    else if (X == 2) acc[2] = fq3_add(acc[2], gx);
                    else if (X == 3) acc[3] = fq3_add(acc[3], gx);
                    else acc[4] = fq3_add(acc[4], gx);
#pragma unroll
                    for (int j = 0; j < 4; j++) v[j] = fq3_add(v[j], st[j]);
                    ev = fq3_add(ev, es);
                }
            }
        }
        u64 vv[15];
#pragma unroll
        for (int i = 0; i < 5; i++) { vv[3 * i] = acc[i].c[0]; vv[3 * i + 1] = acc[i].c[1]; vv[3 * i + 2] = acc[i].c[2]; }
        __syncthreads();
        block_sum_store<15>(vv, red);
        __syncthreads();
        if (threadIdx.x < 15) st_dev_u64(A.partial + (threadIdx.x / 3) * 24 + 3 * slot + threadIdx.x % 3, red[threadIdx.x]);
        wait_mem();
        __syncthreads();
        if (threadIdx.x == 0) s_flag = __hip_atomic_fetch_add(&A.counters[rd], 1u, __ATOMIC_RELAXED, __HIP_MEMORY_SCOPE_AGENT) == nblocks - 1 ? 1u : 0u;
        __syncthreads();
        if (s_flag) {
            __shared__ u64 s_msg[128];
            if (threadIdx.x < 120) {
                const u64 tot = threadIdx.x < npts * 24 ? fq_canon(ld_dev_u64(A.partial + threadIdx.x)) : 0;
                s_msg[threadIdx.x] = tot;
                __hip_atomic_store((u64 *)&A.mail->msg[rd][threadIdx.x], tot, __ATOMIC_RELAXED, __HIP_MEMORY_SCOPE_SYSTEM);
            }
            if (A.dev_transcript) {
                __shared__ u64 sp_st[24], sp_tmp[24], sp_c[24];
                __syncthreads();
                if (threadIdx.x < 64) {
                    const int lane = threadIdx.x;
                    if (lane < 24) sp_st[lane] = ld_dev_u64(A.sponge_state + lane);
                    SpongeDev sp;
                    sp.idx = (int)ld_dev_u64(A.sponge_state + 24);
                    sp.squeezing = (int)ld_dev_u64(A.sponge_state + 25);
                    wave_lds_sync();
                    for (u32 e = 0; e < npts; e++) sponge_absorb_wave(sp, sp_st, sp_tmp, A.pos_ark, A.pos_mds, s_msg + 24 * e, 24);
                    sponge_squeeze_wave(sp, sp_st, sp_tmp, A.pos_ark, A.pos_mds, sp_c, 3);
                    sponge_absorb_wave(sp, sp_st, sp_tmp, A.pos_ark, A.pos_mds, sp_c, 3);
                    const u64 c0 = sp_c[0], c1 = sp_c[1], c2 = sp_c[2];
                    wave_lds_sync();
                    if (lane < 24) sp_c[lane] = lane % 3 == 0 ? c0 : (lane % 3 == 1 ? c1 : c2);
                    wave_lds_sync();
                    sponge_absorb_wave(sp, sp_st, sp_tmp, A.pos_ark, A.pos_mds, sp_c, 24);
                    if (lane < 24) st_dev_u64(A.sponge_state + lane, sp_st[lane]);
                    if (lane == 0) { st_dev_u64(A.sponge_state + 24, (u64)sp.idx); st_dev_u64(A.sponge_state + 25, (u64)sp.squeezing); }
                    if (lane < 3) {
                        const u64 cv = lane == 0 ? c0 : (lane == 1 ? c1 : c2);
                        __hip_atomic_store((u64 *)&A.mail->chal_out[rd][lane], cv, __ATOMIC_RELAXED, __HIP_MEMORY_SCOPE_SYSTEM);
                        st_dev_u64(A.dev_chal + (size_t)rd * 4 + lane, cv);
                    }
                    if (rd + 1 == A.rounds) {
                        if (lane < 24) __hip_atomic_store((u64 *)&A.mail->sponge[lane], sp_st[lane], __ATOMIC_RELAXED, __HIP_MEMORY_SCOPE_SYSTEM);
                        if (lane == 0) {
                            __hip_atomic_store((u64 *)&A.mail->sponge[24], (u64)sp.idx, __ATOMIC_RELAXED, __HIP_MEMORY_SCOPE_SYSTEM);
                            __hip_atomic_store((u64 *)&A.mail->sponge[25], (u64)sp.squeezing, __ATOMIC_RELAXED, __HIP_MEMORY_SCOPE_SYSTEM);
                        }
                    }
                    wait_mem();
                    if (lane == 0) st_dev_u64(A.dev_chal + (size_t)rd * 4 + 3, (u64)A.epoch);
                }
            }
            wait_mem();
            __syncthreads();
            if (threadIdx.x == 0) {
                __hip_atomic_store(&A.counters[rd], 0u, __ATOMIC_RELAXED, __HIP_MEMORY_SCOPE_AGENT);
                __hip_atomic_store((u32 *)&A.mail->msg_seq[rd], A.epoch, __ATOMIC_RELAXED, __HIP_MEMORY_SCOPE_SYSTEM);
            }
        }
        n_prev = n;
    }
}
size_t lin_tail_priv_words(size_t n0, u32 t) { return (size_t)8 * 2 * ((((1 + (size_t)t) * 3 * (n0 / 2)) + 15) & ~(size_t)15) + 16; }
u32 launch_lin_tail(const DevCrt &t, const LinCombDesc &desc, const LinTailArgs &A, hipStream_t s) {
    if (A.n0 < 4 || A.rounds < 1 || A.rounds > TAIL_MAX_ROUNDS || A.deg + 1 > 5 || desc.t > 4) return 0;
    if (t.nu2p40) hipLaunchKernelGGL((k_lin_tail<true>), dim3(1, 8), dim3(256), 0, s, t, desc, A);
    else hipLaunchKernelGGL((k_lin_tail<false>), dim3(1, 8), dim3(256), 0, s, t, desc, A);
    return 8;
}

size_t fold_tail_eqpriv_words(size_t n0, u32 K) {
    size_t worst = 0;
    static const u32 cand[] = {1, 2, 3, 4, 6, 8, 12, 16, 24, 32, 48, 96};
    for (u32 cc : cand) {
        if (8 * cc > FOLD_TAIL_MAX_BLOCKS) break;
        size_t per = (2 * (size_t)K * 3 + cc - 1) / cc, buf = (((5 + per) * 3 * (n0 / 2)) + 15) & ~(size_t)15;
        size_t tot = (size_t)8 * cc * 2 * buf;
        if (tot > worst) worst = tot;
    }
    return worst + 16;
}
u32 launch_fold_tail(const DevCrt &t, const FoldTailArgs &A, int num_cus, hipStream_t s) {
    static int occ_nu = -1, occ_g = -1;
    if (occ_nu < 0) {
        if (hipOccupancyMaxActiveBlocksPerMultiprocessor(&occ_nu, (const void *)k_fold_tail<true>, 256, 0) != hipSuccess) occ_nu = 0;
        if (hipOccupancyMaxActiveBlocksPerMultiprocessor(&occ_g, (const void *)k_fold_tail<false>, 256, 0) != hipSuccess) occ_g = 0;
    }
    const int occ = t.nu2p40 ? occ_nu : occ_g;
    if (occ < 1 || num_cus < 1 || A.n0 < 4 || A.rounds < 1 || A.rounds > TAIL_MAX_ROUNDS) return 0;
    size_t max_blocks = (size_t)occ * (size_t)num_cus / 2;
    if (max_blocks > FOLD_TAIL_MAX_BLOCKS) max_blocks = FOLD_TAIL_MAX_BLOCKS;
    if (max_blocks < 8) return 0;
    const u32 nkd = 2 * A.K * 3;
    u32 chunks = 1;
    static const u32 cand[] = {1, 2, 3, 4, 6, 8, 12, 16, 24, 32, 48, 96};
    for (u32 cc : cand) {
        if (cc > nkd || (size_t)8 * cc > max_blocks) break;
        chunks = cc;
    }
    if (t.nu2p40) hipLaunchKernelGGL((k_fold_tail<true>), dim3(1, 8, chunks), dim3(256), 0, s, t, A);
    else hipLaunchKernelGGL((k_fold_tail<false>), dim3(1, 8, chunks), dim3(256), 0, s, t, A);
    return 8 * chunks;
}

void launch_fold_round_lut(const DevCrt &t, const FoldRoundArgs &a, const int32_t *planesL, const int32_t *planesR, size_t n_planes,
                           const u64 *lut_dev, u32 K, const Fq3Const *mu_pow_dev, u64 *partial, u64 *out, hipStream_t s) {
    FoldSrc src = {};
    src.planesL = planesL; src.planesR = planesR; src.n_planes = n_planes; src.lut = lut_dev;
    launch_fold_round_mode<3>(t, a, nullptr, 0, K, mu_pow_dev, src, partial, out, s);
}
void launch_fold_round_lut_mu(const DevCrt &t, const FoldRoundArgs &a, const int32_t *planesL, const int32_t *planesR, size_t n_planes,
                              const u64 *lut_dev, u64 *mutab_dev, u32 K, const Fq3Const *mu_pow_dev, u64 *partial, u64 *out, hipStream_t s) {
    LF_LAUNCH(k_fold_mutab, t.nu2p40, dim3(2 * K * 3), dim3(128), s, t, lut_dev, mu_pow_dev, 2 * K * 3, mutab_dev);
    FoldSrc src = {};
    src.planesL = planesL; src.planesR = planesR; src.n_planes = n_planes; src.lut = lut_dev; src.mutab = mutab_dev;
    launch_fold_round_mode<5>(t, a, nullptr, 0, K, mu_pow_dev, src, partial, out, s);
}
void launch_fold_round_lut_fix(const DevCrt &t, const FoldRoundArgs &a, const int32_t *planesL, const int32_t *planesR, size_t n_planes,
                               const u64 *lut_dev, Fq3Const r, u64 *Fout, size_t ldout, u32 K, const Fq3Const *mu_pow_dev, u64 *partial,
                               u64 *out, hipStream_t s) {
    FoldSrc src = {};
    src.planesL = planesL; src.planesR = planesR; src.n_planes = n_planes; src.lut = lut_dev;
    src.out = Fout; src.ldo = ldout; src.r = r;
    launch_fold_round_mode<4>(t, a, nullptr, 0, K, mu_pow_dev, src, partial, out, s);
}
void launch_fold_round_lut_fix_tab(const DevCrt &t, const FoldRoundArgs &a, const int32_t *planesL, const int32_t *planesR, size_t n_planes,
                                   const u64 *lut_dev, Fq3Const r, u64 *sq_dev, u64 *mt_dev, u64 *Fout, size_t ldout, u32 K, const Fq3Const *mu_pow_dev,
                                   u64 *partial, u64 *out, hipStream_t s, const u64 *E, size_t ldE) {
    const u32 nkd = 2 * K * 3;
    LF_LAUNCH(k_fold_r4tab, t.nu2p40, dim3((6561 + nkd * 162 + 255) / 256), dim3(256), s, t, lut_dev, r, mu_pow_dev, nkd, sq_dev, mt_dev);
    FoldSrc src = {};
    src.planesL = planesL; src.planesR = planesR; src.n_planes = n_planes; src.lut = lut_dev;
    src.out = Fout; src.ldo = ldout; src.r = r; src.sq4 = sq_dev; src.mt4 = mt_dev; src.E = E; src.ldE = ldE;
    launch_fold_round_mode<6>(t, a, nullptr, 0, K, mu_pow_dev, src, partial, out, s);
}
void launch_fold_round_lut_fix5(const DevCrt &t, const FoldRoundArgs &a, const int32_t *planesL, const int32_t *planesR, size_t n_planes,
                                const u64 *lut_dev, Fq3Const r3, Fq3Const r4, u64 *xx_dev, u64 *yy_dev, u64 *mt_dev, u64 *Fout, size_t ldout, u32 K,
                                const Fq3Const *mu_pow_dev, u64 *partial, u64 *out, hipStream_t s, const u64 *E, size_t ldE) {
    const u32 nkd = 2 * K * 3;
    LF_LAUNCH(k_fold_r5tab, t.nu2p40, dim3((2 * 6561 + nkd * 324 + 255) / 256), dim3(256), s, t, lut_dev, r3, r4, mu_pow_dev, nkd, xx_dev, yy_dev, mt_dev);
    FoldSrc src = {};
    src.planesL = planesL; src.planesR = planesR; src.n_planes = n_planes; src.lut = lut_dev;
    src.out = Fout; src.ldo = ldout; src.r = r4; src.r_prev = r3; src.xx5 = xx_dev; src.yy5 = yy_dev; src.mt5 = mt_dev; src.E = E; src.ldE = ldE;
    launch_fold_round_mode<7>(t, a, nullptr, 0, K, mu_pow_dev, src, partial, out, s);
}
void launch_fold_round_fix(const DevCrt &t, const FoldRoundArgs &a, const u64 *Fprev, size_t ldprev, Fq3Const r, u64 *Fout, size_t ldout, u32 K,
                           const Fq3Const *mu_pow_dev, u64 *partial, u64 *out, hipStream_t s, const u64 *E, size_t ldE) {
    FoldSrc src = {};
    src.out = Fout; src.ldo = ldout; src.r = r; src.E = E; src.ldE = ldE;
    launch_fold_round_mode<1>(t, a, Fprev, ldprev, K, mu_pow_dev, src, partial, out, s);
}

}
```

Baseline: 60.31 steps/s.

## Precompute byte digit codes for fold rounds 4/5 on lane streams

Adds a kernel that turns each witness's int32 digit planes into packed 8-bit per-group digit codes for all K digit levels. It runs on the lane streams after the decomposition joins, and an event hands the result to the fold stream. Fold modes 6 and 7 then read one code byte per group of four instead of loading sixteen int32 values and recomputing digit_code4 for every k. This cuts memory traffic and ALU work in the large fold rounds, at the cost of an extra kernel, K*24*N/4 bytes of buffer per side, and a cross-stream dependency.

After: 60.95 steps/s, median of 6. 1.01x the previous value.

```diff
diff --git a/latticefold_amd/csrc/lf_capi.cpp b/latticefold_amd/csrc/lf_capi.cpp
--- a/latticefold_amd/csrc/lf_capi.cpp
+++ b/latticefold_amd/csrc/lf_capi.cpp
@@ -82,6 +82,8 @@
     if (c->h_aux) (void)hipHostFree(c->h_aux);
     for (int i = 0; i < 2; i++)
         if (c->bits_ev[i]) (void)hipEventDestroy(c->bits_ev[i]);
+    for (int i = 0; i < 2; i++)
+        if (c->codes_ev[i]) (void)hipEventDestroy(c->codes_ev[i]);
     c->release_core();
     delete c;
 }
@@ -768,6 +770,28 @@
 }
 extern "C" int lfdbg_i8g_wg(unsigned int *out512) { return out512 ? ajtai_i8g_read_wg(out512) : -1; }
 extern "C" unsigned lfdbg_i8g_planes_base(int ring, uint64_t base) { return ajtai_i8g_planes_base(ring == LF_RING_BABYBEAR ? ajtai_i8_babybear() : ajtai_i8_goldilocks(), base); }
+extern "C" int lfdbg_fold_code_rounds(lf_ctx *c, unsigned *round_mask) {
+    if (!c || !round_mask) return LF_ERR_INVALID;
+    *round_mask = c->core_any().fold_code_mask;
+    return LF_OK;
+}
+extern "C" int lfdbg_digit_codes(const int32_t *planes, size_t n_planes, unsigned K, uint8_t *codes_out, size_t cap, size_t *ldc_out) {
+    if (!planes || !codes_out || !ldc_out || !n_planes || !K || K > 32) return LF_ERR_INVALID;
+    const size_t ldc = digit_codes_ld(n_planes), bytes = (size_t)K * 24 * ldc;
+    *ldc_out = ldc;
+    if (bytes > cap) return LF_ERR_INVALID;
+    int32_t *dp = nullptr;
+    uint8_t *dc = nullptr;
+    int rc = LF_ERR_HIP;
+    if (hipMalloc((void **)&dp, 24 * n_planes * 4) == hipSuccess && hipMalloc((void **)&dc, bytes) == hipSuccess &&
+        hipMemcpy(dp, planes, 24 * n_planes * 4, hipMemcpyHostToDevice) == hipSuccess) {
+        launch_digit_codes(dp, n_planes, K, dc, nullptr);
+        if (hipGetLastError() == hipSuccess && hipMemcpy(codes_out, dc, bytes, hipMemcpyDeviceToHost) == hipSuccess) rc = LF_OK;
+    }
+    if (dp) (void)hipFree(dp);
+    if (dc) (void)hipFree(dc);
+    return rc;
+}
 int lf_last_fold_paths(lf_ctx *c, unsigned *sv_round_mask) {
     if (!c || !sv_round_mask) return LF_ERR_INVALID;
     *sv_round_mask = c->core_any().sv_round_mask;
diff --git a/latticefold_amd/csrc/lf_ctx.h b/latticefold_amd/csrc/lf_ctx.h
--- a/latticefold_amd/csrc/lf_ctx.h
+++ b/latticefold_amd/csrc/lf_ctx.h
@@ -151,6 +151,7 @@
     const lf_witness *bits_wit[2] = {nullptr, nullptr};
     u32 *bits_ptr[2] = {nullptr, nullptr};
     hipEvent_t bits_ev[2] = {nullptr, nullptr};
+    hipEvent_t codes_ev[2] = {nullptr, nullptr};
     hipEvent_t ev_yR = nullptr, ev_yL = nullptr;
     u64 *h_pin2 = nullptr;
     size_t h_pin2_words = 0;
@@ -254,6 +255,8 @@
     hipEvent_t z_ev = nullptr;
     const unsigned char *D = nullptr;
     u32 *sv_bits = nullptr;
+    const uint8_t *codes = nullptr;
+    hipEvent_t codes_ev = nullptr;
     ~SideState() { if (z_ev) (void)hipEventDestroy(z_ev); }
 };
 int gather_parts(lf_ctx *c, const GatherPart *parts, int np, size_t lcl);
@@ -290,6 +293,9 @@
 };
 #define LF_XB(c) ((c) && (c)->xb.on && !t_xb_active)
 int fold_impl(lf_ctx *c, Transcript &tr, SideState *S , u64 *lcccs_out, lf_witness **w_out, u64 *proof);
+struct FoldTabPlan { bool use_lut, use_r4tab, use_r5, codes; };
+FoldTabPlan fold_tab_plan(const lf_ctx *c);
+int fold_digit_codes(lf_ctx *c, const int32_t *planes, int sd, hipStream_t s, const uint8_t **codes);
 int commit_download(lf_ctx *c, const u64 *dev, size_t words, u64 *host);
 int commit_parts_i8g(lf_ctx *c, const unsigned char *D, size_t ldn, u32 NP, u64 *out_dev);
 int sb_cut_parts(lf_ctx *c, const lf_witness *wit, const char *name, const unsigned char **D);
diff --git a/latticefold_amd/csrc/lf_ctx_core.h b/latticefold_amd/csrc/lf_ctx_core.h
--- a/latticefold_amd/csrc/lf_ctx_core.h
+++ b/latticefold_amd/csrc/lf_ctx_core.h
@@ -43,6 +43,7 @@
     hipEvent_t ev_prep[2] = {nullptr, nullptr};
     unsigned sv_round_mask = 0;
     unsigned fold_split_mask = 0;
+    unsigned fold_code_mask = 0;
     float phase_ms[LF_N_PHASES] = {0};
     float k_fold_ms = 0, k_ajtai_ms = 0;
     int k_fold_n = 0, k_ajtai_n = 0;
diff --git a/latticefold_amd/csrc/lf_fold.cpp b/latticefold_amd/csrc/lf_fold.cpp
--- a/latticefold_amd/csrc/lf_fold.cpp
+++ b/latticefold_amd/csrc/lf_fold.cpp
@@ -204,6 +204,25 @@
         for (u32 i = 0; i < K2; i++) { c->ring.mul_ntt(&rho[(size_t)i * 24], part(i) + ((size_t)P.s + 3 + P.kappa + P.t + q2) * 24, tmp); HostRing::add(o, tmp, o); }
     }
 }
+FoldTabPlan fold_tab_plan(const lf_ctx *c) {
+    const lf_params &P = c->P;
+    const size_t m = c->m, N = c->N, Gw = (size_t)c->sh_world;
+    FoldTabPlan pl = {false, false, false, false};
+    if (P.b != 2) return pl;
+    const bool fused = !c->tn.fold_unfused && (Gw == 1 || !c->tn.shard_plain_rounds);
+    pl.use_lut = fused && P.s >= 4 && m / 4 >= c->tn.lut_min && m / 4 >= 4 && !c->tn.fold_no_lut;
+    pl.use_r4tab = pl.use_lut && c->dcrt.nu2p40 && !c->tn.fold_no_r4tab;
+    pl.use_r5 = pl.use_r4tab && !c->tn.fold_no_r5tab && Gw == 1 && P.s >= 5 && (N & 3) == 0 && (c->tn.no_tail || m / 8 > c->tn.tail_n) && m / 32 >= c->tn.r5_min;
+    pl.codes = pl.use_r4tab && Gw == 1;
+    return pl;
+}
+int fold_digit_codes(lf_ctx *c, const int32_t *planes, int sd, hipStream_t s, const uint8_t **codes) {
+    uint8_t *buf;
+    RET(c->tbuf(sd ? "fold_codes_R" : "fold_codes_L", (size_t)c->P.K * 24 * digit_codes_ld(c->N), &buf));
+    launch_digit_codes(planes, c->N, c->P.K, buf, s);
+    *codes = buf;
+    return LF_OK;
+}
 int fold_impl(lf_ctx *c, Transcript &tr, SideState *S , u64 *lcccs_out, lf_witness **w_out, u64 *proof) {
     if (c->P.b != 2) return fold_impl_sb(c, tr, S, lcccs_out, w_out, proof);
     const lf_params &P = c->P;
@@ -331,11 +350,10 @@
     int fmode = 0;
     const u64 *prevF = nullptr;
     size_t prevld = 0;
-    const size_t lut_min = c->tn.lut_min;
     const size_t tab_min = c->tn.tab_min;
-    const bool use_lut = fused && P.s >= 4 && m / 4 >= lut_min && m / 4 >= 4 && !c->tn.fold_no_lut;
-    const bool use_r4tab = use_lut && c->dcrt.nu2p40 && !c->tn.fold_no_r4tab;
-    const bool use_r5 = use_r4tab && !c->tn.fold_no_r5tab && Gw == 1 && P.s >= 5 && (N & 3) == 0 && (c->tn.no_tail || m / 8 > c->tn.tail_n) && m / 32 >= c->tn.r5_min;
+    const FoldTabPlan tabs = fold_tab_plan(c);
+    const bool use_lut = tabs.use_lut, use_r4tab = tabs.use_r4tab, use_r5 = tabs.use_r5;
+    c->fold_code_mask = 0;
     u64 *F[2], *T5[2];
     size_t half = m / 2;
     const size_t f0_ent = use_lut ? m / 16 : m / 4, f1_ent = use_r5 ? m / 32 : m / 8;
@@ -564,15 +582,23 @@
             u64 *r4sq, *r4mt;
             RET(c->tbuf("fold_r4sq", (size_t)6561 * 4, &r4sq));
             RET(c->tbuf("fold_r4mt", (size_t)K2 * 3 * 162 * 4, &r4mt));
+            if (tabs.codes)
+                for (int sd = 0; sd < 2; sd++) {
+                    if (S[sd].codes) { if (S[sd].codes_ev) HIPCHK(hipStreamWaitEvent(c->stream(), S[sd].codes_ev, 0)); }
+                    else RET(fold_digit_codes(c, S[sd].planes, sd, c->stream(), &S[sd].codes));
+                    S[sd].codes_ev = nullptr;
+                }
+            if (S[0].codes && S[1].codes) c->fold_code_mask |= 1u << (round - 1);
             launch_fold_round_lut_fix_tab(c->dcrt, a, S[0].planes, S[1].planes, N, d_lut, f3c(pt[round - 2]), r4sq, r4mt, use_r5 ? nullptr : (u64 *)curF, ldF, K, d_mu, partial, od,
-                                          c->stream(), Er, ldEr);
+                                          c->stream(), Er, ldEr, S[0].codes, S[1].codes);
         } else if (fmode == 7) {
             u64 *r5xx, *r5yy, *r5mt;
             RET(c->tbuf("fold_r5xx", (size_t)6561 * 4, &r5xx));
             RET(c->tbuf("fold_r5yy", (size_t)6561 * 4, &r5yy));
             RET(c->tbuf("fold_r5mt", (size_t)K2 * 3 * 324 * 4, &r5mt));
+            if (S[0].codes && S[1].codes) c->fold_code_mask |= 1u << (round - 1);
             launch_fold_round_lut_fix5(c->dcrt, a, S[0].planes, S[1].planes, N, d_lut, f3c(pt[round - 3]), f3c(pt[round - 2]), r5xx, r5yy, r5mt, (u64 *)curF, ldF, K, d_mu, partial, od,
-                                       c->stream(), Er, ldEr);
+                                       c->stream(), Er, ldEr, S[0].codes, S[1].codes);
         } else if (fmode == 4) launch_fold_round_lut_fix(c->dcrt, a, S[0].planes, S[1].planes, N, d_lut, f3c(pt[round - 2]), (u64 *)curF, ldF, K, d_mu, partial, od, c->stream());
         else if (fmode == 1) launch_fold_round_fix(c->dcrt, a, prevF, prevld, f3c(pt[round - 2]), (u64 *)curF, ldF, K, d_mu, partial, od, c->stream(), Er, ldEr);
         else launch_fold_round(c->dcrt, a, curF, ldF, K, d_mu, partial, od, c->stream());
diff --git a/latticefold_amd/csrc/lf_kernels.h b/latticefold_amd/csrc/lf_kernels.h
--- a/latticefold_amd/csrc/lf_kernels.h
+++ b/latticefold_amd/csrc/lf_kernels.h
@@ -120,10 +120,14 @@
                        u64 *partial, u64 *out, hipStream_t s);
 void launch_fold_round_lut_fix_tab(const DevCrt &t, const FoldRoundArgs &a, const int32_t *planesL, const int32_t *planesR, size_t n_planes,
                                    const u64 *lut_dev, Fq3Const r, u64 *sq_dev, u64 *mt_dev, u64 *Fout, size_t ldout, u32 K, const Fq3Const *mu_pow_dev,
-                                   u64 *partial, u64 *out, hipStream_t s, const u64 *E = nullptr, size_t ldE = 0 );
+                                   u64 *partial, u64 *out, hipStream_t s, const u64 *E = nullptr, size_t ldE = 0 ,
+                                   const uint8_t *codesL = nullptr, const uint8_t *codesR = nullptr);
 void launch_fold_round_lut_fix5(const DevCrt &t, const FoldRoundArgs &a, const int32_t *planesL, const int32_t *planesR, size_t n_planes,
                                 const u64 *lut_dev, Fq3Const r3, Fq3Const r4, u64 *xx_dev, u64 *yy_dev, u64 *mt_dev, u64 *Fout, size_t ldout, u32 K,
-                                const Fq3Const *mu_pow_dev, u64 *partial, u64 *out, hipStream_t s, const u64 *E = nullptr, size_t ldE = 0 );
+                                const Fq3Const *mu_pow_dev, u64 *partial, u64 *out, hipStream_t s, const u64 *E = nullptr, size_t ldE = 0 ,
+                                const uint8_t *codesL = nullptr, const uint8_t *codesR = nullptr);
+size_t digit_codes_ld(size_t n_planes);
+void launch_digit_codes(const int32_t *planes, size_t n_planes, u32 K, uint8_t *codes, hipStream_t s);
 void launch_fold_round_fix(const DevCrt &t, const FoldRoundArgs &a, const u64 *Fprev, size_t ldprev, Fq3Const r, u64 *Fout, size_t ldout, u32 K,
                            const Fq3Const *mu_pow_dev, u64 *partial, u64 *out, hipStream_t s, const u64 *E = nullptr, size_t ldE = 0 );
 void launch_fold_round_lut(const DevCrt &t, const FoldRoundArgs &a, const int32_t *planesL, const int32_t *planesR, size_t n_planes,
diff --git a/latticefold_amd/csrc/lf_prove.cpp b/latticefold_amd/csrc/lf_prove.cpp
--- a/latticefold_amd/csrc/lf_prove.cpp
+++ b/latticefold_amd/csrc/lf_prove.cpp
@@ -795,6 +795,16 @@
     c->lin_blocks = 0;
     TL_MARK("lane 1 joined");
     if (rc == LF_OK) rc = rc1;
+    if (rc == LF_OK && fold_tab_plan(c).codes) {
+        const lf_witness *ws[2] = {w_acc, w_i};
+        for (int sd = 0; sd < 2; sd++) {
+            hipStream_t st = c->st_lane[sd];
+            if (!c->codes_ev[sd] && hipEventCreateWithFlags(&c->codes_ev[sd], hipEventDisableTiming) != hipSuccess) break;
+            if (fold_digit_codes(c, ws[sd]->planes, sd, st, &S[sd].codes) != LF_OK) { S[sd].codes = nullptr; break; }
+            if (hipEventRecord(c->codes_ev[sd], st) != hipSuccess) { (void)hipStreamSynchronize(st); S[sd].codes = nullptr; break; }
+            S[sd].codes_ev = c->codes_ev[sd];
+        }
+    }
     if (rc == LF_OK) c->host_tr_ms += absorb_decomposition(P, tr, lin.data(), decr, S[1]);
     }
     TL_MARK("right absorb done");
diff --git a/latticefold_amd/csrc/lf_rounds.hip b/latticefold_amd/csrc/lf_rounds.hip
--- a/latticefold_amd/csrc/lf_rounds.hip
+++ b/latticefold_amd/csrc/lf_rounds.hip
@@ -580,6 +580,8 @@
     const u64 *xx5, *yy5, *mt5;
     const u64 *sq4, *mt4;
     const u64 *E; size_t ldE;
+    const uint8_t *codesL, *codesR;
+    size_t ldc;
 };
 template <bool NU>
 __global__ void __launch_bounds__(128) k_fold_mutab(DevCrt t, const u64 *lut, const Fq3Const *mu_pow, u32 nkd, u64 *mutab) {
@@ -647,10 +649,35 @@
     }
     return (u32)code;
 }
-template <bool NU, int MODE, bool SPLIT = false>
+__global__ void __launch_bounds__(256) k_digit_codes(const int32_t *planes, size_t n_planes, u32 K, uint8_t *codes, size_t ldc) {
+    const size_t w = (size_t)blockIdx.x * 256 + threadIdx.x;
+    const u32 plane = blockIdx.y;
+    if (4 * w >= ldc) return;
+    const int32_t *pl = planes + (size_t)plane * n_planes + 16 * w;
+    int32_t v[16];
+    if (16 * w + 16 <= n_planes && (n_planes & 3) == 0) {
+#pragma unroll
+        for (int q = 0; q < 4; q++) {
+            int4 x = *(const int4 *)(pl + 4 * q);
+            v[4 * q] = x.x; v[4 * q + 1] = x.y; v[4 * q + 2] = x.z; v[4 * q + 3] = x.w;
+        }
+    } else {
+#pragma unroll
+        for (int q = 0; q < 16; q++) v[q] = 16 * w + q < n_planes ? pl[q] : 0;
+    }
+    u32 *out = (u32 *)(codes + (size_t)plane * ldc) + w;
+    for (u32 k = 0; k < K; k++, out += 6 * ldc) {
+        u32 word = 0;
+#pragma unroll
+        for (int g = 0; g < 4; g++) word |= digit_code4(v + 4 * g, k) << (8 * g);
+        *out = word;
+    }
+}
+template <bool NU, int MODE, bool SPLIT = false, bool CODES = false>
 __global__ void __launch_bounds__(256) k_fold_round(DevCrt t, FoldRoundArgs a, const u64 *F, size_t ldF, u32 K, const Fq3Const *mu_pow,
                                                     FoldSrc src, u64 *partial) {
     static_assert(!SPLIT || (NU && (MODE == 1 || MODE == 6 || MODE == 7)), "split form: the large-round modes of the 2^40 non-residue path");
+    static_assert(!CODES || (NU && (MODE == 6 || MODE == 7)), "digit-code tables: modes 6 and 7");
     constexpr int NA = SPLIT ? 3 : 5;
     u32 slot = blockIdx.y;
     const size_t pend = a.p0 + a.pcnt;
@@ -792,20 +819,29 @@
                 const int32_t *pl = (side ? src.planesR : src.planesL) + (size_t)(d * 8 + slot) * src.n_planes + (size_t)32 * p;
                 const u64 *mt = src.mt5 + (size_t)kd * 4 * 81 * 4;
                 Fq3 fv[2], sq[2], mf[2];
+                u64 cw = 0;
+                if constexpr (CODES)
+                    cw = (size_t)8 * p < src.ldc ? *(const u64 *)((side ? src.codesR : src.codesL) + ((size_t)k * 24 + d * 8 + slot) * src.ldc + (size_t)8 * p) : 0x2828282828282828ull;
 #pragma unroll
                 for (int e = 0; e < 2; e++) {
-                    int32_t v[16];
-                    if ((size_t)32 * p + 16 * e + 16 <= src.n_planes && (src.n_planes & 3) == 0) {
-#pragma unroll
-                        for (int q = 0; q < 4; q++) {
-                            int4 w = *(const int4 *)(pl + 16 * e + 4 * q);
-                            v[4 * q] = w.x; v[4 * q + 1] = w.y; v[4 * q + 2] = w.z; v[4 * q + 3] = w.w;
+                    u32 c0, c1, c2, c3;
+                    if constexpr (CODES) {
+                        const u32 w = (u32)(cw >> (32 * e));
+                        c0 = w & 255; c1 = (w >> 8) & 255; c2 = (w >> 16) & 255; c3 = w >> 24;
+                    } else {
+                        int32_t v[16];
+                        if ((size_t)32 * p + 16 * e + 16 <= src.n_planes && (src.n_planes & 3) == 0) {
+#pragma unroll
+                            for (int q = 0; q < 4; q++) {
+                                int4 w = *(const int4 *)(pl + 16 * e + 4 * q);
+                                v[4 * q] = w.x; v[4 * q + 1] = w.y; v[4 * q + 2] = w.z; v[4 * q + 3] = w.w;
+                            }
+                        } else {
+#pragma unroll
+                            for (int q = 0; q < 16; q++) v[q] = (size_t)32 * p + 16 * e + q < src.n_planes ? pl[16 * e + q] : 0;
                         }
-                    } else {
-#pragma unroll
-                        for (int q = 0; q < 16; q++) v[q] = (size_t)32 * p + 16 * e + q < src.n_planes ? pl[16 * e + q] : 0;
+                        c0 = digit_code4(v, k); c1 = digit_code4(v + 4, k); c2 = digit_code4(v + 8, k); c3 = digit_code4(v + 12, k);
                     }
-                    const u32 c0 = digit_code4(v, k), c1 = digit_code4(v + 4, k), c2 = digit_code4(v + 8, k), c3 = digit_code4(v + 12, k);
                     const u64 *qx = src.xx5 + (size_t)(c0 * 81 + c1) * 4, *qy = src.yy5 + (size_t)(c2 * 81 + c3) * 4;
                     const ulonglong2 xa = *(const ulonglong2 *)qx, ya = *(const ulonglong2 *)qy;
                     const u64 xc = qx[2], yc = qy[2];
@@ -842,19 +878,25 @@
             Fq3 sp = fq3_zero(), su = fq3_zero();
             auto gen = [&](u32 kd, Fq3 &tt, Fq3 &uu, Fq3 &s0, Fq3 &s1) {
                 const u32 side = kd / (3 * K), k = (kd / 3) % K, d = kd % 3;
-                const int32_t *pl = (side ? src.planesR : src.planesL) + (size_t)(d * 8 + slot) * src.n_planes + (size_t)16 * p;
-                int32_t v[16];
-                if ((size_t)16 * p + 16 <= src.n_planes && (src.n_planes & 3) == 0) {
-#pragma unroll
-                    for (int q = 0; q < 4; q++) {
-                        int4 w = *(const int4 *)(pl + 4 * q);
-                        v[4 * q] = w.x; v[4 * q + 1] = w.y; v[4 * q + 2] = w.z; v[4 * q + 3] = w.w;
+                u32 c0, c1, c2, c3;
+                if constexpr (CODES) {
+                    const u32 w = (size_t)4 * p < src.ldc ? *(const u32 *)((side ? src.codesR : src.codesL) + ((size_t)k * 24 + d * 8 + slot) * src.ldc + (size_t)4 * p) : 0x28282828u;
+                    c0 = w & 255; c1 = (w >> 8) & 255; c2 = (w >> 16) & 255; c3 = w >> 24;
+                } else {
+                    const int32_t *pl = (side ? src.planesR : src.planesL) + (size_t)(d * 8 + slot) * src.n_planes + (size_t)16 * p;
+                    int32_t v[16];
+                    if ((size_t)16 * p + 16 <= src.n_planes && (src.n_planes & 3) == 0) {
+#pragma unroll
+                        for (int q = 0; q < 4; q++) {
+                            int4 w = *(const int4 *)(pl + 4 * q);
+                            v[4 * q] = w.x; v[4 * q + 1] = w.y; v[4 * q + 2] = w.z; v[4 * q + 3] = w.w;
+                        }
+                    } else {
+#pragma unroll
+                        for (int q = 0; q < 16; q++) v[q] = (size_t)16 * p + q < src.n_planes ? pl[q] : 0;
                     }
-                } else {
-#pragma unroll
-                    for (int q = 0; q < 16; q++) v[q] = (size_t)16 * p + q < src.n_planes ? pl[q] : 0;
-                }
-                const u32 c0 = digit_code4(v, k), c1 = digit_code4(v + 4, k), c2 = digit_code4(v + 8, k), c3 = digit_code4(v + 12, k);
+                    c0 = digit_code4(v, k); c1 = digit_code4(v + 4, k); c2 = digit_code4(v + 8, k); c3 = digit_code4(v + 12, k);
+                }
                 const u64 *q0 = src.sq4 + (size_t)(c0 * 81 + c1) * 4, *q1 = src.sq4 + (size_t)(c2 * 81 + c3) * 4;
                 const u64 *ma = src.mt4 + (size_t)kd * 2 * 81 * 4, *mb = ma + 81 * 4;
                 const ulonglong2 s0a = *(const ulonglong2 *)q0, s1a = *(const ulonglong2 *)q1;
@@ -1007,6 +1049,14 @@
     }
     while (gb * chunks > RED_BLOCKS && chunks > 1) chunks--;
     if (MODE >= 3) chunks = 1;
+    if constexpr (MODE == 6 || MODE == 7) {
+        if (src.codesL && src.codesR && t.nu2p40) {
+            if (src.E) hipLaunchKernelGGL((k_fold_round<true, MODE, true, true>), dim3(gb, 8, chunks), dim3(256), 0, s, t, a, F, ldF, K, mu_pow_dev, src, partial);
+            else hipLaunchKernelGGL((k_fold_round<true, MODE, false, true>), dim3(gb, 8, chunks), dim3(256), 0, s, t, a, F, ldF, K, mu_pow_dev, src, partial);
+            hipLaunchKernelGGL(k_reduce_rows, dim3((src.E ? 3 : 5) * 24), dim3(256), 0, s, partial, gb * chunks, src.E ? 72 : 120, out);
+            return;
+        }
+    }
     if constexpr (MODE == 1 || MODE == 6 || MODE == 7) {
         if (src.E && t.nu2p40) {
             hipLaunchKernelGGL((k_fold_round<true, MODE, true>), dim3(gb, 8, chunks), dim3(256), 0, s, t, a, F, ldF, K, mu_pow_dev, src, partial);
@@ -1576,24 +1626,34 @@
     src.out = Fout; src.ldo = ldout; src.r = r;
     launch_fold_round_mode<4>(t, a, nullptr, 0, K, mu_pow_dev, src, partial, out, s);
 }
+size_t digit_codes_ld(size_t n_planes) {
+    const size_t ld = ((n_planes + 3) / 4 + 7) / 8 * 8;
+    return ld ? ld : 8;
+}
+void launch_digit_codes(const int32_t *planes, size_t n_planes, u32 K, uint8_t *codes, hipStream_t s) {
+    const size_t ldc = digit_codes_ld(n_planes);
+    hipLaunchKernelGGL(k_digit_codes, dim3((unsigned)((ldc / 4 + 255) / 256), 24), dim3(256), 0, s, planes, n_planes, K, codes, ldc);
+}
 void launch_fold_round_lut_fix_tab(const DevCrt &t, const FoldRoundArgs &a, const int32_t *planesL, const int32_t *planesR, size_t n_planes,
                                    const u64 *lut_dev, Fq3Const r, u64 *sq_dev, u64 *mt_dev, u64 *Fout, size_t ldout, u32 K, const Fq3Const *mu_pow_dev,
-                                   u64 *partial, u64 *out, hipStream_t s, const u64 *E, size_t ldE) {
+                                   u64 *partial, u64 *out, hipStream_t s, const u64 *E, size_t ldE, const uint8_t *codesL, const uint8_t *codesR) {
     const u32 nkd = 2 * K * 3;
     LF_LAUNCH(k_fold_r4tab, t.nu2p40, dim3((6561 + nkd * 162 + 255) / 256), dim3(256), s, t, lut_dev, r, mu_pow_dev, nkd, sq_dev, mt_dev);
     FoldSrc src = {};
     src.planesL = planesL; src.planesR = planesR; src.n_planes = n_planes; src.lut = lut_dev;
     src.out = Fout; src.ldo = ldout; src.r = r; src.sq4 = sq_dev; src.mt4 = mt_dev; src.E = E; src.ldE = ldE;
+    src.codesL = codesL; src.codesR = codesR; src.ldc = digit_codes_ld(n_planes);
     launch_fold_round_mode<6>(t, a, nullptr, 0, K, mu_pow_dev, src, partial, out, s);
 }
 void launch_fold_round_lut_fix5(const DevCrt &t, const FoldRoundArgs &a, const int32_t *planesL, const int32_t *planesR, size_t n_planes,
                                 const u64 *lut_dev, Fq3Const r3, Fq3Const r4, u64 *xx_dev, u64 *yy_dev, u64 *mt_dev, u64 *Fout, size_t ldout, u32 K,
-                                const Fq3Const *mu_pow_dev, u64 *partial, u64 *out, hipStream_t s, const u64 *E, size_t ldE) {
+                                const Fq3Const *mu_pow_dev, u64 *partial, u64 *out, hipStream_t s, const u64 *E, size_t ldE, const uint8_t *codesL, const uint8_t *codesR) {
     const u32 nkd = 2 * K * 3;
     LF_LAUNCH(k_fold_r5tab, t.nu2p40, dim3((2 * 6561 + nkd * 324 + 255) / 256), dim3(256), s, t, lut_dev, r3, r4, mu_pow_dev, nkd, xx_dev, yy_dev, mt_dev);
     FoldSrc src = {};
     src.planesL = planesL; src.planesR = planesR; src.n_planes = n_planes; src.lut = lut_dev;
     src.out = Fout; src.ldo = ldout; src.r = r4; src.r_prev = r3; src.xx5 = xx_dev; src.yy5 = yy_dev; src.mt5 = mt_dev; src.E = E; src.ldE = ldE;
+    src.codesL = codesL; src.codesR = codesR; src.ldc = digit_codes_ld(n_planes);
     launch_fold_round_mode<7>(t, a, nullptr, 0, K, mu_pow_dev, src, partial, out, s);
 }
 void launch_fold_round_fix(const DevCrt &t, const FoldRoundArgs &a, const u64 *Fprev, size_t ldprev, Fq3Const r, u64 *Fout, size_t ldout, u32 K,
```
